# bliunlpr/Robust_e2e_gan

Hardware: AMD Instinct MI355X
Metric: joint_train utterances/sec (higher is better)
Workload: dtype f32; 1 GPU; config4: joint_train.py full GAN+ASR step, B=32 per GPU, T=800, F=257->80, L=40, V=4233, enhancer 2xBLSTM-256, VGG+3xBLSTMP-512, loc-attention decoder 300, D basic ndf64, Adadelta; global_batch=32, per_rank_batch=32, parallelism=dp1, utterance_lengths=560..800 frames (mean 680 of T=800)

## Files before the change

### include/re2e.h

```cpp
#ifndef RE2E_H
#define RE2E_H
#include <stddef.h>
#ifdef __cplusplus
extern "C" {
#endif

typedef struct ihipStream_t* re2e_stream_t;

#define RE2E_OK 0
#define RE2E_EINVAL (-1)
#define RE2E_EUNSUPPORTED (-2)
#define RE2E_EHIP (-3)

#define RE2E_ACT_NONE 0
#define RE2E_ACT_TANH 1
#define RE2E_ACT_RELU 2
#define RE2E_ACT_LRELU 3
#define RE2E_ACT_SIGMOID 4
#define RE2E_ACT_SIGMOID_MASK_MUL 5

#define RE2E_LOSS_L2 0
#define RE2E_LOSS_L1 1
#define RE2E_LOSS_SMOOTH_L1 2
#define RE2E_STREAM_DEFAULT 0
#define RE2E_STREAM_FILLER 1

#define RE2E_LOSS_BCE 3

#define RE2E_ABI_VERSION 322
int re2e_version(void);
const char* re2e_last_error(void);
int re2e_device_ok(void);
int re2e_warmup(void);
int re2e_stream_role(re2e_stream_t stream, int role);

size_t re2e_gemm_workspace_bytes(int transa, int transb, int M, int N, int K);
int re2e_gemm(int transa, int transb, int M, int N, int K, const float* A, long lda, const float* B, long ldb,
              float* C, long ldc, const float* bias, const float* bias2, int act, float beta, const float* mul,
              float* mask_out, const int* lens_dev, int T, void* workspace, size_t workspace_bytes,
              re2e_stream_t stream);
int re2e_gemm_plan(int transa, int transb, int M, int N, int K, int a16, int b16, int c16, int act, int rowmap, int filler, int cus, char* out,
                   size_t out_bytes);
int re2e_gemm_nt_rows(int Mv, int N, int K, const float* A, long lda, const float* B, long ldb, float* C, long ldc, const float* bias,
                      const float* bias2, int act, float beta, const int* rowmap, int ident_rows, int phys_rows, void* workspace,
                      size_t workspace_bytes, re2e_stream_t stream);
int re2e_gemm_tn_rows(int M, int N, int Kv, const float* A, long lda, const float* B, long ldb, float* C, long ldc, float beta,
                      const int* rowmap, int ident_rows, int phys_rows, void* workspace, size_t workspace_bytes, re2e_stream_t stream);
int re2e_fill_rows(float* C, long ldc, int N, const int* rows, int nrows, float value, const float* row_vec, int act, re2e_stream_t stream);

int re2e_conv_igemm(const float* in, int NI, int H, int W, int C, const float* wg, int Cout, int KH, int KW, int PH,
                    int PW, int SY, int SX, int DY, int DX, int OY0, int OX0, float* out, int OHF, int OWF, int osy,
                    int osx, int ooy, int oox, const float* bias, int act, float beta, re2e_stream_t stream);
int re2e_conv_igemm_masked(const float* in, int NI, int H, int W, int C, const float* wg, int Cout, int KH, int KW, int PH,
                           int PW, int SY, int SX, int DY, int DX, int OY0, int OX0, float* out, int OHF, int OWF, int osy,
                           int osx, int ooy, int oox, const float* relu_out, re2e_stream_t stream);
int re2e_conv3x3_relu_pool(const float* in, int NI, int H, int W, int C, const float* wg, int Cout, const float* bias, float* pooled,
                           unsigned char* idx_u8, re2e_stream_t stream);
size_t re2e_conv3x3_wino_workspace_bytes(int C, int Cout);
int re2e_conv3x3_wino(const float* in, int NI, int H, int W, int C, const float* w, int Cout, int dgrad, const float* bias, int relu,
                      const float* mask, float* out, float* pool_out, unsigned char* pool_idx, void* workspace, size_t workspace_bytes,
                      re2e_stream_t stream);

size_t re2e_conv3x3_wino_wgrad_workspace_bytes(int NI, int H, int W, int C, int Cout);
int re2e_conv3x3_wino_wgrad(const float* in, int NI, int H, int W, int C, const float* dout, int Cout, float* gw, float beta,
                            void* workspace, size_t workspace_bytes, re2e_stream_t stream);

int re2e_conv3x3_wino_rows(const float* in, int NI, int H, int W, int C, const float* w, int Cout, int dgrad, const float* bias, int relu,
                           const float* mask, float* out, float* pool_out, unsigned char* pool_idx, const int* row_lim, void* workspace,
                           size_t workspace_bytes, re2e_stream_t stream);
int re2e_conv3x3_wino_wgrad_rows(const float* in, int NI, int H, int W, int C, const float* dout, int Cout, float* gw, float beta,
                                 const int* row_lim, void* workspace, size_t workspace_bytes, re2e_stream_t stream);
int re2e_fill_image_rows(float* t, int N, int H, long row_floats, const int* lim, int div, int max_tail_rows, float value, re2e_stream_t stream);

size_t re2e_conv4x4_wino_workspace_bytes(int NI, int H, int W, int C, int Cout, int pad);
int re2e_conv4x4_wino(const float* in, int NI, int H, int W, int C, const float* w, int Cout, int pad, int dgrad, float* out,
                      void* workspace, size_t workspace_bytes, re2e_stream_t stream);
size_t re2e_conv4x4_wino_wgrad_workspace_bytes(int NI, int H, int W, int C, int Cout, int pad);
int re2e_conv4x4_wino_wgrad(const float* in, int NI, int H, int W, int C, const float* dout, int Cout, int pad, float* gw, float beta,
                            void* workspace, size_t workspace_bytes, re2e_stream_t stream);
size_t re2e_conv_wgrad_workspace_bytes(int NI, int PH, int PW, int C, int Cout, int KH, int KW);
int re2e_conv_wgrad(const float* in, int NI, int H, int W, int C, const float* dout, int Cout, int KH, int KW, int PH,
                    int PW, int SY, int SX, int OY0, int OX0, float* dW, float beta, void* workspace,
                    size_t workspace_bytes, re2e_stream_t stream);
int re2e_conv_dgrad_s2(const float* dz, int N, int OH, int OW, int Cout, const float* W, int Cin, int KH, int KW, int H,
                       int Wd, int pad, float* dx, float* wt_ws, re2e_stream_t stream);
int re2e_conv_weight_gather(const float* W, float* dst, int Cout, int Cin, int KH, int KW, int transpose, int TA,
                            int TB, int kh0, int kw0, int kstep, re2e_stream_t stream);

int re2e_transpose01(const float* in, float* out, int D0, int D1, int W, re2e_stream_t stream);
int re2e_act_fwd(const float* x, float* y, long n, int act, re2e_stream_t stream);
int re2e_act_bwd(const float* dy, const float* y, float* dz, long n, int act, re2e_stream_t stream);
size_t re2e_colsum_workspace_bytes(int M, int N);
int re2e_colsum(const float* A, int M, int N, long lda, float* out, float beta, void* workspace,
                size_t workspace_bytes, re2e_stream_t stream);
int re2e_act_bwd_colsum(const float* dy, const float* y, float* dz, int M, int N, int act, float* out, float beta,
                        void* workspace, size_t workspace_bytes, re2e_stream_t stream);
int re2e_mask_mul_bwd(const float* dout, const float* mix, const float* mask, float* dlin, long n,
                      re2e_stream_t stream);
int re2e_mask_mul_bwd_ld(const float* dout, const float* mix, const float* mask, float* dlin, long rows, int N, int ldd,
                         re2e_stream_t stream);
int re2e_mul(const float* a, const float* b, float* out, long n, re2e_stream_t stream);
int re2e_affine_cols(const float* x, const float* c0, const float* c1, float* out, long rows, int N,
                     re2e_stream_t stream);
int re2e_dropout(const float* x, float* y, long n, float p, unsigned long long seed, unsigned call, re2e_stream_t stream);
int re2e_axpby(float a, const float* x, float b, float* y, long n, re2e_stream_t stream);
int re2e_gather_rows(const float* src, const int* idx_dev, float* dst, int nrows, int W, re2e_stream_t stream);
int re2e_scatter_rows(const float* src, const int* idx_dev, float* dst, int nrows, int W, re2e_stream_t stream);
int re2e_mask_rows(const float* in, float* out, const int* lens_dev, int B, int T, int W, re2e_stream_t stream);

int re2e_pack_pad(const float* src_flat, const int* offsets_dev, const int* lens_dev, int B, int Tmax, int F,
                  float* dst, re2e_stream_t stream);

int re2e_kaldi_decode_pad(const unsigned char* blob, const long* rec_off_dev, const int* kind_dev, const int* lens_dev, int B,
                          int Tmax, int F, float* dst, float* dst_log, const float* cmvn, re2e_stream_t stream);

int re2e_fbank_fwd(const float* x, long rows, int F, int NF, const int* band_off, const int* band_len,
                   const float* band_w, int maxw, float* y_raw, float* y_norm, const float* cmvn, float* pw_out,
                   re2e_stream_t stream);
int re2e_fbank_bwd(const float* x, long rows, int F, int NF, const int* bin_off, const int* bin_len, const float* bin_w, int maxc,
                   const float* pw, const float* dy_raw, const float* dy_norm, const float* cmvn, float* dx, re2e_stream_t stream);
int re2e_logclamp_fwd(const float* z, const float* cmvn, long rows, int N, float* y, re2e_stream_t stream);
int re2e_logclamp_bwd(const float* z, const float* cmvn, long rows, int N, const float* dy, float* dz, re2e_stream_t stream);
int re2e_cmvn_stats(const float* y, const int* lens_dev, int B, int T, int NF, float* sum_out, float* sumsq_out,
                    re2e_stream_t stream);

size_t re2e_reduce_workspace_bytes(long n);
int re2e_loss_fwd(const float* a, const float* b, float target, long n, int kind, float* out, void* workspace,
                  size_t workspace_bytes, re2e_stream_t stream);
int re2e_loss_bwd(const float* a, const float* b, float target, long n, int kind, const float* gscale_dev,
                  float scale, float* da, float beta, re2e_stream_t stream);
int re2e_sumsq(const float* x, long n, float* out, void* workspace, size_t workspace_bytes, re2e_stream_t stream);

int re2e_maxpool2_fwd(const float* in, int NI, int H, int W, int C, float* out, unsigned char* idx_u8, int relu_in,
                      re2e_stream_t stream);
int re2e_maxpool2_bwd(const float* dout, const unsigned char* idx_u8, int NI, int H, int W, int C, float* din,
                      re2e_stream_t stream);
int re2e_vgg_pack_fwd(const float* in, const int* lens_dev, int NI, int T, int Fq, int C, float* out, int NI_total,
                      int n_off, re2e_stream_t stream);
int re2e_vgg_pack_bwd(const float* dout, const int* lens_dev, int NI, int T, int Fq, int C, float* din, int NI_total,
                      int n_off, re2e_stream_t stream);

size_t re2e_bn_workspace_bytes(long P, int C);
int re2e_bn_lrelu_fwd(const float* x, long P, int C, const float* gamma, const float* beta, float* running_mean,
                      float* running_var, float momentum, float eps, int train, float slope, float* y, float* save_mean,
                      float* save_invstd, void* workspace, size_t workspace_bytes, re2e_stream_t stream);
int re2e_bn_lrelu_bwd(const float* dy, const float* x, long P, int C, const float* gamma, const float* beta,
                      const float* save_mean, const float* save_invstd, float slope, float* dx, float* dgamma, float* dbeta,
                      float gbeta, void* workspace, size_t workspace_bytes, re2e_stream_t stream);
int re2e_bn_sync_partial(const float* x, long P, int C, const float* mean, int square, float* out, void* workspace, size_t workspace_bytes,
                         re2e_stream_t stream);
int re2e_bn_sync_finalize(const float* mean, const float* var, long Ptotal, int C, float momentum, float eps, float* running_mean,
                          float* running_var, float* save_mean, float* save_invstd, re2e_stream_t stream);
int re2e_bn_apply(const float* x, long P, int C, const float* save_mean, const float* save_invstd, const float* gamma, const float* beta,
                  float slope, float* y, re2e_stream_t stream);
int re2e_bn_sync_bwd_partial(const float* dy, const float* x, long P, int C, const float* gamma, const float* beta, const float* save_mean,
                             const float* save_invstd, float slope, float* out, void* workspace, size_t workspace_bytes, re2e_stream_t stream);
int re2e_bn_sync_bwd_apply(const float* dy, const float* x, long P, int C, const float* gamma, const float* beta, const float* save_mean,
                           const float* save_invstd, float slope, const float* sums, float* dx, re2e_stream_t stream);

size_t re2e_lstm_workspace_bytes(int B, int H);
int re2e_lstm_abort_count(void);
int re2e_debug_force_abort(int n);
int re2e_debug_occupy(int workgroups, int lds_bytes, int usec, re2e_stream_t stream);
int re2e_step_gate(int* base_dev, int ack, const float* extra_sumsq, float* stats_main, float* stats_d, const float* d_requires, float* hold_next,
                   float* delta_out, re2e_stream_t stream);
int re2e_lstm_seq_fwd(float* xg_f, float* xg_r, const float* whh_f, const float* whh_r, float* ybuf, float* cbuf,
                      const int* lens_dev, int T, int B, int H, void* workspace, size_t workspace_bytes,
                      re2e_stream_t stream);
int re2e_lstm_seq_bwd(float* g_f, float* g_r, const float* whh_f, const float* whh_r, const float* dy,
                      const float* ybuf, const float* cbuf, float* dc_state, const int* lens_dev, int T, int B, int H,
                      float* dbias, void* workspace, size_t workspace_bytes, re2e_stream_t stream);
int re2e_lstm_plan(int T, int B, int H, int backward, int cus, char* out, size_t out_bytes);

int re2e_lstm_cell_fwd(float* gates, const float* c_prev, float* c_out, float* h_out, int B, int H,
                       re2e_stream_t stream);
int re2e_lstm_cell_bwd(float* gates, const float* c_prev, const float* c_cur, const float* dh, const float* dh2,
                       const float* dc_in, float* dc_prev_out, int B, int H, re2e_stream_t stream);
int re2e_dec_gates_cell_fwd(const float* cx, const float* z_prev, const float* w_ctx, long ldw, const float* w_hh, float* gates,
                            const float* c_prev, float* c_out, float* h_out, int B, int E, int D, re2e_stream_t stream);
size_t re2e_dec_loop_workspace_bytes(int L1, int B, int T, int E, int D, int A, int C, int Fh);
int re2e_dec_loop_fwd(const float* pre, const float* enc, const int* hlens_dev, const float* w_decT, const float* w_att, const float* w_conv,
                      const float* gvec, const float* gvec_b, const float* w_ctx, long ldw, const float* w_hh, float* gates, float* z, float* c,
                      float* w, float* cx, float* conv, float* dpj, int L1, int B, int T, int E, int D, int A, int C, int Fh,
                      void* workspace, size_t workspace_bytes, re2e_stream_t stream);
size_t re2e_dec_loop_bwd_workspace_bytes(int L1, int B, int T, int E, int D, int A, int C, int Fh);
int re2e_dec_loop_bwd(const float* pre, const float* enc, const float* cx, const float* z, const float* c, const float* w, const float* conv,
                      const float* dpj, const float* dZ, const int* hlens_dev, const float* w_ctx, long ldw, const float* w_hh, const float* mlp_dec,
                      const float* w_att, const float* w_conv, const float* gvec, float* gates, float* d_cx_all, float* de_all, float* ddp,
                      float* d_pre, int L1, int B, int T, int E, int D, int A, int C, int Fh, void* workspace, size_t workspace_bytes,
                      re2e_stream_t stream);
int re2e_dec_loop_dwconv(const float* w, const int* hlens_dev, const void* workspace, size_t workspace_bytes, float* partials, int partial_floats,
                         int wconv_offset, int L1, int B, int T, int E, int D, int A, int C, int Fh, re2e_stream_t stream);
int re2e_gemm_skinny2(int M, int K, const float* A, long lda, const float* B1, long ldb1, int N1, float* C1, long ldc1,
                      const float* B2, long ldb2, int N2, float* C2, long ldc2, re2e_stream_t stream);
int re2e_embedding_fwd(const float* table, const int* ids_dev, int n, int D, float* out, long ldo,
                       re2e_stream_t stream);
int re2e_embedding_bwd(const float* dout, long ldo, const int* ids_dev, int n, int D, int V, float* dtable,
                       float beta, re2e_stream_t stream);
int re2e_argmax_rows(const float* x, int R, int V, long ldx, int* out_ids, re2e_stream_t stream);
int re2e_log_softmax_rows(const float* x, int R, int V, long ldx, float* out, re2e_stream_t stream);

int re2e_ce_fwd(const float* logits, const int* targets_dev, int R, int V, float scale, float* out, float* lse,
                void* workspace, size_t workspace_bytes, re2e_stream_t stream);
int re2e_ce_bwd(const float* logits, const int* targets_dev, const float* lse, const float* fwd_out, int R, int V,
                float scale, const float* gscale_dev, float* dlogits, re2e_stream_t stream);
int re2e_lsm_fwd(const float* logits, const float* dist, int R, int V, int nutt, float* out, void* workspace,
                 size_t workspace_bytes, re2e_stream_t stream);
int re2e_lsm_bwd(const float* logits, const float* dist, int R, int V, int nutt, const float* gscale, float* dlogits,
                 re2e_stream_t stream);

size_t re2e_ctc_workspace_bytes(int T, int B, int Lmax);
int re2e_ctc_fwd(const float* logits, int T, int B, int V, const int* hlens_dev, const int* labels_dev,
                 const int* label_off_dev, const int* label_len_dev, int Lmax, float* loss_out, float* nll_per_utt,
                 void* workspace, size_t workspace_bytes, re2e_stream_t stream);
int re2e_ctc_bwd(const float* logits, int T, int B, int V, const int* hlens_dev, const int* labels_dev,
                 const int* label_off_dev, const int* label_len_dev, int Lmax, const float* nll_per_utt,
                 const float* gscale_dev, float* dlogits, int ldd, const void* workspace, re2e_stream_t stream);

int re2e_ctc_prefix_score(const float* lpz, int T, int V, const float* att_lsm, int nh, const float* r_prev, const int* last_label_dev,
                          const int* out_len_dev, const float* prev_score_dev, int ctc_beam, float att_weight, float ctc_weight, int blank,
                          int eos, int* cand_out, float* local_out, float* ctc_score_out, float* r_new, re2e_stream_t stream);
int re2e_ctc_prefix_score_cands(const float* lpz, int T, int V, const float* att_lsm, int nh, const float* r_prev, const int* last_label_dev,
                                const int* out_len_dev, const float* prev_score_dev, const int* cand_dev, int ncand, float att_weight,
                                float ctc_weight, int blank, int eos, float* local_out, float* ctc_score_out, float* r_new, re2e_stream_t stream);

int re2e_attloc_fwd(const float* pre, const float* enc, const float* z, const float* att_prev, const int* hlens_dev,
                    const float* w_decT, const float* w_att, const float* w_conv, const float* gvec, const float* gvec_b,
                    int B, int T, int eprojs, int dunits, int adim, int chans, int filts, float* w_out, float* c_out,
                    long ldc_out, float* conv_out, float* dp_out, float* e_scratch, re2e_stream_t stream);
size_t re2e_attloc_partial_floats(int adim, int chans, int filts);
size_t re2e_attloc_workspace_bytes(int B, int T, int adim, int chans);
int re2e_attloc_bwd(const float* pre, const float* enc, const float* att_prev, const float* w_cur, const int* hlens_dev,
                    const float* w_att, const float* w_conv, const float* gvec, const float* conv_in, const float* dp_in,
                    const float* cx_in, const float* dc, long ld_dc, const float* dw_in, int B, int T, int eprojs, int adim,
                    int chans, int filts, float* de_out, float* d_att_prev, float* d_decproj, float* partials,
                    void* workspace, size_t workspace_bytes, re2e_stream_t stream);
int re2e_attloc_dpre(const float* pre, const float* conv_all, const float* dp_all, const float* de_all, const float* w_att,
                     const float* gvec, int L1, int B, int T, int adim, int chans, int filts, float* d_pre, float* partials,
                     void* workspace, size_t workspace_bytes, re2e_stream_t stream);
int re2e_attloc_denc(const float* w_all, const float* dc_all, int L1, int B, int T, int eprojs, float* d_enc, float beta,
                     re2e_stream_t stream);

int re2e_lm_lstm_cell(const float* x, long ldx, const int* ids_dev, int n_embed, int I, const float* w_ih, const float* w_hh,
                      const float* b_ih, const float* b_hh, const float* h_prev, const float* c_prev, int n, int H, float* h_out,
                      float* c_out, re2e_stream_t stream);
int re2e_lm_output(const float* h, const float* w, const float* b, int n, int V, int H, float* logits, re2e_stream_t stream);
int re2e_lm_log_softmax_combine(const float* logits, int n, int V, const float* att, float lm_weight, float* lsm, float* comb,
                                re2e_stream_t stream);
int re2e_lm_add_cands(float* local, const float* lm, const int* cand_dev, int n, int ncand, int V, float lm_weight, re2e_stream_t stream);

int re2e_clip_coef(const float* sumsq_dev, float max_norm, float* stats_dev, re2e_stream_t stream);
int re2e_adadelta_step(float* p, const float* g, float* sq_avg, float* acc_delta, long n, float rho, float eps,
                       float lr, const float* stats_dev, re2e_stream_t stream);
int re2e_adam_step(float* p, const float* g, float* m, float* v, long n, float lr, float beta1, float beta2,
                   float eps, int step, const float* stats_dev, re2e_stream_t stream);

#ifdef __cplusplus
}
#endif
#endif
```

### robust_e2e_gan_amd/csrc/lstm.hip

```cpp
#include <stdlib.h>

#include <atomic>

#include "common.h"

namespace {

#ifdef RE2E_EXPERIMENTS
__device__ unsigned long long* g_lstm_stamps = nullptr;
constexpr int kStampStep0 = 64;
#define LSTM_STAMP_DECL unsigned long long* const stamp_p = g_lstm_stamps
#define LSTM_STAMP(ph)                                                                                                              \
  do {                                                                                                                              \
    if (stamp_p && (threadIdx.x & 63) == 0 && s >= kStampStep0 && s < kStampStep0 + 16)                                             \
      stamp_p[((((long)blockIdx.z * gridDim.y + blockIdx.y) * gridDim.x + blockIdx.x) * 16 + (threadIdx.x >> 6)) * 192 + (s - kStampStep0) * 12 + (ph)] = \
          (ph) >= 10 ? __builtin_amdgcn_s_memrealtime() : __builtin_amdgcn_s_memtime();                                             \
  } while (0)
static void lstm_stamps_arm() {
  const char* v = getenv("RE2E_LSTM_STAMPS");
  unsigned long long* p = v ? (unsigned long long*)strtoull(v, nullptr, 16) : nullptr;
  (void)hipMemcpyToSymbol(HIP_SYMBOL(g_lstm_stamps), &p, sizeof(p));
}
#else
#define LSTM_STAMP_DECL
#define LSTM_STAMP(ph)
static void lstm_stamps_arm() {}
#endif

__device__ __forceinline__ void store_acc(float* red, const f32x16& acc, int lane) {
  int lr = lane & 31, lh = lane >> 5;
#pragma unroll
  for (int r = 0; r < 16; ++r) {
    int row = (r & 3) + 8 * (r >> 2) + 4 * lh;
    red[row * 33 + lr] = acc[r];
  }
}

__device__ __forceinline__ void mfma_chain(const f32x4* __restrict__ ap, const f32x4* __restrict__ bp, int QN, f32x16& acc,
                                           int bstride = 64, bool bvalid = true) {
  constexpr int CH = 8;
  const f32x4 zero = {0.f, 0.f, 0.f, 0.f};
  for (int q0 = 0; q0 < QN; q0 += CH) {
    f32x4 a[CH], b[CH];
#pragma unroll
    for (int u = 0; u < CH; ++u) {
      int q = q0 + u < QN ? q0 + u : QN - 1;
      a[u] = ap[(long)q * 64];
      b[u] = bvalid ? bp[(long)q * bstride] : zero;
    }
#pragma unroll
    for (int u = 0; u < CH; ++u) {
      if (q0 + u < QN) {
#pragma unroll
        for (int j = 0; j < 4; ++j) acc = __builtin_amdgcn_mfma_f32_32x32x2f32(a[u][j], b[u][j], acc, 0, 0, 0);
      }
    }
  }
}

__global__ void pack_w_fwd_kernel(const float* __restrict__ whh, float* __restrict__ wf, int H) {
  long tot = (long)4 * H * H;
  for (long e = (long)blockIdx.x * blockDim.x + threadIdx.x; e < tot; e += (long)gridDim.x * blockDim.x) {
    int i = (int)(e & 3); int lane = (int)((e >> 2) & 63); long r = e >> 8; int Q = (int)(r % (H / 8)); int x = (int)(r / (H / 8));
    int n = lane & 31, h = lane >> 5;
    wf[e] = whh[((long)((n >> 3) * H + 8 * x + (n & 7))) * H + 8 * Q + 4 * h + i];
  }
}
__global__ void pack_w_bwd_kernel(const float* __restrict__ whh, float* __restrict__ wb, int H, int UW) {
  const int njt = (H + 31) / 32, NQ = 4 * UW;
  long tot = (long)(H / (8 * UW)) * njt * NQ * 256;
  for (long e = (long)blockIdx.x * blockDim.x + threadIdx.x; e < tot; e += (long)gridDim.x * blockDim.x) {
    int i = (int)(e & 3); int lane = (int)((e >> 2) & 63); long r = e >> 8; int Q = (int)(r % NQ); r /= NQ; int jt = (int)(r % njt); int x = (int)(r / njt);
    int m = 8 * Q + 4 * (lane >> 5) + i;
    int j = 32 * jt + (lane & 31);
    wb[e] = j < H ? whh[((long)(((m >> 3) & 3) * H + 8 * UW * x + 8 * (m >> 5) + (m & 7))) * H + j] : 0.f;
  }
}

template <int WAVES>
__global__ __launch_bounds__(WAVES * 64) void lstm_fwd_step(float* xg_f, float* xg_r, const float* __restrict__ wfrag, float* ybuf,
                                                            float* cbuf, float* hfrag, const int* __restrict__ lens, int T, int B,
                                                            int H, int s) {
  extern __shared__ __attribute__((aligned(16))) float red[];
  constexpr int NTH = WAVES * 64;
  constexpr int ITER = (256 + NTH - 1) / NTH;
  const int dir = blockIdx.z, mt = blockIdx.y, x = blockIdx.x, MT = gridDim.y;
  const int t = dir ? T - 1 - s : s;
  float* xg = dir ? xg_r : xg_f;
  const int j0 = x * 8, b0 = mt * 32;
  const int tid = threadIdx.x, lane = tid & 63, wid = tid >> 6, lh = lane >> 5;
  const int QN = H / 8 / WAVES;
  const int prev_blk = dir ? t + 2 : t;
  const long H2 = 2L * H;
  const long hf_sz = (long)2 * MT * H * 32;
  const float* hf_rd = hfrag + ((s & 1) ^ 1) * hf_sz + (long)(dir * MT + mt) * H * 32;
  float* hf_wr = hfrag + (s & 1) * hf_sz + (long)(dir * MT + mt) * H * 32;
  float pre[ITER][4], cp[ITER];
  int ln[ITER];
#pragma unroll
  for (int it = 0; it < ITER; ++it) {
    int idx = tid + it * NTH;
    int bm = idx >> 3, jj = idx & 7, b = b0 + bm, j = j0 + jj;
    bool ok = idx < 256 && b < B;
    const float* gp = xg + ((long)t * B + (ok ? b : 0)) * 4 * H + j;
#pragma unroll
    for (int g = 0; g < 4; ++g) pre[it][g] = ok ? gp[g * H] : 0.f;
    cp[it] = ok ? cbuf[((long)prev_blk * B + b) * H2 + dir * H + j] : 0.f;
    ln[it] = ok ? lens[b] : 0;
  }
  const f32x4* wp = reinterpret_cast<const f32x4*>(wfrag) + ((long)(dir * (H / 8) + x) * (H / 8) + wid * QN) * 64 + lane;
  const f32x4* hp = reinterpret_cast<const f32x4*>(hf_rd) + ((long)(2 * wid * QN + lh)) * 32 + (lane & 31);
  f32x16 acc;
#pragma unroll
  for (int r = 0; r < 16; ++r) acc[r] = 0.f;
  if (s > 0) mfma_chain(hp, wp, QN, acc);
  store_acc(red + wid * (32 * 33), acc, lane);
  __syncthreads();
#pragma unroll
  for (int it = 0; it < ITER; ++it) {
    int idx = tid + it * NTH;
    int bm = idx >> 3, jj = idx & 7, b = b0 + bm, j = j0 + jj;
    if (idx >= 256 || b >= B) continue;
    float v[4];
#pragma unroll
    for (int g = 0; g < 4; ++g) {
      float a = 0.f;
      for (int w = 0; w < WAVES; ++w) a += red[w * (32 * 33) + bm * 33 + g * 8 + jj];
      v[g] = a + pre[it][g];
    }
    float gi = sigmoidf_(v[0]), gf = sigmoidf_(v[1]), gg = tanhf_(v[2]), go = sigmoidf_(v[3]);
    float c = gf * cp[it] + gi * gg;
    float h = go * tanhf_(c);
    if (t >= ln[it]) { c = 0.f; h = 0.f; }
    float* go_ = xg + ((long)t * B + b) * 4 * H + j;
    go_[0] = gi; go_[H] = gf; go_[2 * H] = gg; go_[3 * H] = go;
    cbuf[((long)(t + 1) * B + b) * H2 + dir * H + j] = c;
    ybuf[((long)(t + 1) * B + b) * H2 + dir * H + j] = h;
    hf_wr[((long)(j >> 2) * 32 + bm) * 4 + (j & 3)] = h;
  }
}

typedef unsigned long long u64;
typedef unsigned u32x4 __attribute__((ext_vector_type(4)));
typedef __attribute__((address_space(1))) u64 gu64;
__device__ unsigned g_persist_aborts = 0;
constexpr unsigned kSpinLimit = 1u << 24;

template <int WAVES, int QN, int UW>
__global__ __launch_bounds__(WAVES * 64) void lstm_fwd_persist(float* xg_f, float* xg_r, const float* __restrict__ wfrag, float* ybuf,
                                                               float* cbuf, u64* hx_, unsigned* err, const int* __restrict__ lens,
                                                               int T, int B, int H) {
  extern __shared__ __attribute__((aligned(16))) float red[];
  static_assert(WAVES >= 4 * UW, "256 threads per 8 units own the 32 x 8 cell updates");
  const int dir = blockIdx.z, mt = blockIdx.y, MT = gridDim.y, NX = gridDim.x * UW;
  const int tid = threadIdx.x, lane = tid & 63, wid = tid >> 6, lr = lane & 31, lh = lane >> 5;
  const int usub = (tid >> 8) < UW ? (tid >> 8) : 0;
  const int x = blockIdx.x * UW + usub;
  float* xg = dir ? xg_r : xg_f;
  const int j0 = x * 8, b0 = mt * 32;
  constexpr int kAbort = UW * WAVES * 32 * 33;
  if (tid == 0) red[kAbort] = 0.f;
  const long H2 = 2L * H;
  f32x4 w[UW][QN];
#pragma unroll
  for (int u = 0; u < UW; ++u) {
    const f32x4* wp = reinterpret_cast<const f32x4*>(wfrag) + ((long)(dir * NX + blockIdx.x * UW + u) * NX + wid * QN) * 64 + lane;
#pragma unroll
    for (int q = 0; q < QN; ++q) w[u][q] = wp[q * 64];
  }
  gu64* hx = (gu64*)hx_;
  const int par_sz = 2 * MT * NX * 256;
  const __amdgpu_buffer_rsrc_t hx_rs = __builtin_amdgcn_make_buffer_rsrc(hx_, 0, (int)(2 * par_sz * 8), 0x00020000);
  const int grp = (dir * MT + mt) * NX * 256;
  const int rd_off = grp + (wid * QN) * 256 + (lh * 32 + lr) * 4;
  const bool pw = tid < 256 * UW;
  const int bm = (tid >> 3) & 31, jj = tid & 7, b = b0 + bm, j = j0 + jj;
  const bool ok = pw && b < B;
  const int ln = ok ? lens[b] : 0;
  const int wr_off = grp + x * 256 + ((jj >> 2) * 32 + bm) * 4 + (jj & 3);
  float c = 0.f, pre[4] = {0.f, 0.f, 0.f, 0.f};
  if (ok) {
    const float* gp = xg + ((long)(dir ? T - 1 : 0) * B + b) * 4 * H + j;
#pragma unroll
    for (int g = 0; g < 4; ++g) pre[g] = gp[g * H];
  }
  LSTM_STAMP_DECL;
  __syncthreads();
  for (int s = 0; s < T; ++s) {
    const int t = dir ? T - 1 - s : s;
    LSTM_STAMP(0); LSTM_STAMP(10);
    f32x16 acc[UW];
#pragma unroll
    for (int u = 0; u < UW; ++u)
#pragma unroll
      for (int r = 0; r < 16; ++r) acc[u][r] = 0.f;
    if (s > 0) {
      const gu64* src = hx + ((s & 1) ^ 1) * par_sz + rd_off;
      float hv[QN][4];
      const unsigned rd_b = (unsigned)((((s & 1) ^ 1) * par_sz + rd_off) * 8);
      for (unsigned spins = 0;; ++spins) {
        asm volatile("" ::: "memory");
        bool good = true;
#pragma unroll
        for (int q = 0; q < QN; ++q) {
          const u32x4 lo = __builtin_amdgcn_raw_buffer_load_b128(hx_rs, rd_b + (unsigned)q * 2048u, 0, 16);
          const u32x4 hi = __builtin_amdgcn_raw_buffer_load_b128(hx_rs, rd_b + (unsigned)q * 2048u + 16u, 0, 16);
          hv[q][0] = __uint_as_float(lo[0]); hv[q][1] = __uint_as_float(lo[2]);
          hv[q][2] = __uint_as_float(hi[0]); hv[q][3] = __uint_as_float(hi[2]);
          good &= (lo[1] == (unsigned)s) & (lo[3] == (unsigned)s) & (hi[1] == (unsigned)s) & (hi[3] == (unsigned)s);
        }
        if (__all(good)) break;
        if (spins > kSpinLimit) { if (lane == 0) { red[kAbort] = 1.f; if (atomicExch(err, 1u) == 0u) atomicAdd(&g_persist_aborts, 1u); } break; }
        __builtin_amdgcn_s_sleep(1);
      }
      LSTM_STAMP(1);
#pragma unroll
      for (int q = 0; q < QN; ++q)
#pragma unroll
        for (int i = 0; i < 4; ++i)
#pragma unroll
          for (int u = 0; u < UW; ++u) acc[u] = __builtin_amdgcn_mfma_f32_32x32x2f32(hv[q][i], w[u][q][i], acc[u], 0, 0, 0);
    }
#pragma unroll
    for (int u = 0; u < UW; ++u) store_acc(red + (u * WAVES + wid) * (32 * 33), acc[u], lane);
    LSTM_STAMP(2);
    __syncthreads();
    LSTM_STAMP(3);
    if (red[kAbort] != 0.f) break;
    if (pw) {
      float v[4];
#pragma unroll
      for (int g = 0; g < 4; ++g) {
        float a = 0.f;
#pragma unroll
        for (int wv = 0; wv < WAVES; ++wv) a += red[(usub * WAVES + wv) * (32 * 33) + bm * 33 + g * 8 + jj];
        v[g] = a + pre[g];
      }
      float gi = sigmoidf_(v[0]), gf = sigmoidf_(v[1]), gg = tanhf_(v[2]), go = sigmoidf_(v[3]);
      float cn = gf * c + gi * gg;
      float h = go * tanhf_(cn);
      if (t >= ln) { cn = 0.f; h = 0.f; }
      c = cn;
      if (ok && s + 1 < T) {
        const float* gp = xg + ((long)(dir ? t - 1 : t + 1) * B + b) * 4 * H + j;
#pragma unroll
        for (int g = 0; g < 4; ++g) pre[g] = gp[g * H];
      }
      if (s + 1 < T)
        __hip_atomic_store(hx + (s & 1) * par_sz + wr_off, ((u64)(unsigned)(s + 1) << 32) | (u64)__float_as_uint(h), __ATOMIC_RELAXED,
                           __HIP_MEMORY_SCOPE_AGENT);
      LSTM_STAMP(4); LSTM_STAMP(11);
      if (ok) {
        float* go_ = xg + ((long)t * B + b) * 4 * H + j;
        go_[0] = gi; go_[H] = gf; go_[2 * H] = gg; go_[3 * H] = go;
        cbuf[((long)(t + 1) * B + b) * H2 + dir * H + j] = cn;
        ybuf[((long)(t + 1) * B + b) * H2 + dir * H + j] = h;
      }
    }
    LSTM_STAMP(5);
    __syncthreads();
    LSTM_STAMP(6);
  }
  if (red[kAbort] != 0.f && ok) {
    for (int t = 0; t < T; ++t) ybuf[((long)(t + 1) * B + b) * H2 + dir * H + j] = __uint_as_float(0x7fc00000u);
  }
}

__device__ __forceinline__ void store16u_sc1(unsigned* p, const u32x4& v) {
  asm volatile("global_store_dwordx4 %0, %1, off sc1\n\ts_nop 1" ::"v"(p), "v"(v) : "memory");
}
constexpr unsigned kTagBit = 0x40000000u, kNanPub = 0x3FC00000u;
__device__ __forceinline__ bool tags_are(const u32x4& v, unsigned want) {
  return (((v[0] & v[1] & v[2] & v[3]) ^ want) & kTagBit) == 0u && (((v[0] | v[1] | v[2] | v[3]) ^ want) & kTagBit) == 0u;
}

template <int TILES, int NJ, bool PERSIST>
__global__ __launch_bounds__(256) void lstm_fwd2(float* xg_f, float* xg_r, const float* __restrict__ whh_f, const float* __restrict__ whh_r,
                                                 float* ybuf, float* cbuf, unsigned* hx_, unsigned* err, const int* __restrict__ lens, int T,
                                                 int B, int H, int s_arg) {
  constexpr int KS = 4;
  extern __shared__ __attribute__((aligned(16))) float lds2[];
  f32x4* part = reinterpret_cast<f32x4*>(lds2);
  int* abortw = reinterpret_cast<int*>(lds2 + 2 * TILES * KS * 64 * 4);
  const int dir = blockIdx.z, mt = blockIdx.y, MT = gridDim.y, x = blockIdx.x;
  const int tid = threadIdx.x, lane = tid & 63, ks = tid >> 6, n = lane & 15, kk = lane >> 4;
  const int ft = ks < TILES ? ks : -1;
  float* xg = dir ? xg_r : xg_f;
  const float* whh = dir ? whh_r : whh_f;
  const long H2 = 2L * H;
  if (PERSIST && tid == 0) *abortw = 0;
  f32x4 w[TILES][NJ];
#pragma unroll
  for (int t = 0; t < TILES; ++t) {
    const long row = (long)(n & 3) * H + 4 * TILES * x + 4 * t + (n >> 2);
#pragma unroll
    for (int jj = 0; jj < NJ; ++jj) w[t][jj] = *reinterpret_cast<const f32x4*>(whh + row * H + 16 * (ks * NJ + jj) + 4 * kk);
  }
  const int par_w = 2 * MT * H * 16;
  const __amdgpu_buffer_rsrc_t hx_rs = __builtin_amdgcn_make_buffer_rsrc(hx_, 0, (int)(2 * par_w * 4), 0x00020000);
  const bool fin = ft >= 0;
  const int j = 4 * TILES * x + 4 * (fin ? ft : 0) + kk;
  const int s0 = PERSIST ? 0 : s_arg, s1 = PERSIST ? T : s_arg + 1;
  const int grp = (dir * MT + mt) * H * 16;
  const int b = 16 * mt + n;
  const unsigned rd_w = (unsigned)(grp + ((4 * ks * NJ + kk) * 16 + n) * 4);
  const unsigned poll_w = (unsigned)(grp + ((4 * ks * NJ + (lane < 4 * NJ ? lane : 0)) * 16) * 4);
  const bool ok = fin && b < B;
  const int ln = ok ? lens[b] : 0;
  const unsigned wr_w = (unsigned)(grp + ((TILES * x + (fin ? ft : 0)) * 16 + n) * 4);
  float c = 0.f, pre[4] = {0.f, 0.f, 0.f, 0.f};
  if (ok) {
    const int t0 = dir ? T - 1 - s0 : s0;
    const float* gp = xg + ((long)t0 * B + b) * 4 * H + j;
#pragma unroll
    for (int g = 0; g < 4; ++g) pre[g] = gp[g * H];
    if (!PERSIST) c = cbuf[((long)(dir ? t0 + 2 : t0) * B + b) * H2 + dir * H + j];
  }
  u32x4 ld[NJ];
#pragma unroll
  for (int jj = 0; jj < NJ; ++jj) ld[jj] = u32x4{0u, 0u, 0u, 0u};
  if (!PERSIST && s0 > 0) {
    const u32x4* src = reinterpret_cast<const u32x4*>(hx_ + ((s0 & 1) ^ 1) * par_w) + rd_w / 4;
#pragma unroll
    for (int jj = 0; jj < NJ; ++jj) ld[jj] = src[jj * 64];
  }
  LSTM_STAMP_DECL;
  if (PERSIST) __syncthreads();
  for (int s = s0; s < s1; ++s) {
    const int t = dir ? T - 1 - s : s;
    LSTM_STAMP(0); LSTM_STAMP(10);
    constexpr int NACC = TILES == 1 ? 2 : TILES;
    f32x4 acc[NACC];
#pragma unroll
    for (int tt = 0; tt < NACC; ++tt) acc[tt] = f32x4{0.f, 0.f, 0.f, 0.f};
    if (s > 0) {
      const unsigned want = PERSIST ? (unsigned)((((s - 1) >> 1) + 1) & 1) << 30 : 0u;
      const unsigned rd_b = (unsigned)((((s & 1) ^ 1) * par_w) * 4) + rd_w * 4u;
      const unsigned pl_b = (unsigned)((((s & 1) ^ 1) * par_w) * 4) + poll_w * 4u;
      auto wait_producers = [&]() {
        for (unsigned spins = 0;; ++spins) {
          asm volatile("" ::: "memory");
          const u32x4 pv = __builtin_amdgcn_raw_buffer_load_b128(hx_rs, pl_b, 0, 16);
          if (__all(tags_are(pv, want))) break;
          if (spins > kSpinLimit) { if (lane == 0) { *abortw = 1; if (atomicExch(err, 1u) == 0u) atomicAdd(&g_persist_aborts, 1u); } break; }
        }
        asm volatile("" ::: "memory");
      };
      if (PERSIST) {
        wait_producers();
#pragma unroll
        for (int jj = 0; jj < NJ; ++jj) ld[jj] = __builtin_amdgcn_raw_buffer_load_b128(hx_rs, rd_b + (unsigned)jj * 1024u, 0, 16);
        LSTM_STAMP(7);
      }
#pragma unroll
      for (int jj = 0; jj < NJ; ++jj) {
        u32x4 v = ld[jj];
        if (PERSIST) {
          if (!__all(tags_are(v, want))) {
            wait_producers();
#pragma unroll
            for (int j2 = jj; j2 < NJ; ++j2) ld[j2] = __builtin_amdgcn_raw_buffer_load_b128(hx_rs, rd_b + (unsigned)j2 * 1024u, 0, 16);
            v = ld[jj];
            for (unsigned spins = 0; !__all(tags_are(v, want)); ++spins) {
              asm volatile("" ::: "memory");
              v = __builtin_amdgcn_raw_buffer_load_b128(hx_rs, rd_b + (unsigned)jj * 1024u, 0, 16);
              if (spins > kSpinLimit) { if (lane == 0) { *abortw = 1; if (atomicExch(err, 1u) == 0u) atomicAdd(&g_persist_aborts, 1u); } break; }
            }
          }
        }
        float hv[4];
#pragma unroll
        for (int i = 0; i < 4; ++i) {
          unsigned uu = PERSIST ? (v[i] & ~kTagBit) : v[i];
          if (PERSIST) uu = uu == kNanPub ? 0x7fc00000u : uu;
          hv[i] = __uint_as_float(uu);
        }
#pragma unroll
        for (int i = 0; i < 4; ++i)
#pragma unroll
          for (int tt = 0; tt < TILES; ++tt) {
            const int a = TILES == 1 ? (i & 1) : tt;
            acc[a] = __builtin_amdgcn_mfma_f32_16x16x4f32(w[tt][jj][i], hv[i], acc[a], 0, 0, 0);
          }
      }
      if (TILES == 1) acc[0] += acc[1];
    }
    LSTM_STAMP(1);
    f32x4* pp = part + (s & 1) * (TILES * KS * 64);
#pragma unroll
    for (int tt = 0; tt < TILES; ++tt)
      if (tt != ft) pp[(tt * KS + ks) * 64 + lane] = acc[tt];
    LSTM_STAMP(2);
    __syncthreads();
    LSTM_STAMP(3);
    if (PERSIST && *abortw) break;
    float og[6] = {0.f, 0.f, 0.f, 0.f, 0.f, 0.f};
    if (fin) {
      f32x4 v = {0.f, 0.f, 0.f, 0.f};
      f32x4 mine = acc[0];
#pragma unroll
      for (int tt = 1; tt < TILES; ++tt) mine = ft == tt ? acc[tt] : mine;
#pragma unroll
      for (int k2 = 0; k2 < KS; ++k2) v += k2 == ks ? mine : pp[(ft * KS + k2) * 64 + lane];
      const float gi = sigmoidf_(v[0] + pre[0]), gf = sigmoidf_(v[1] + pre[1]), gg = tanhf_(v[2] + pre[2]), go = sigmoidf_(v[3] + pre[3]);
      float cn = __builtin_fmaf(gf, c, gi * gg);
      float h = go * tanhf_(cn);
      if (t >= ln) { cn = 0.f; h = 0.f; }
      c = cn;
      if (PERSIST && ok && s + 1 < T) {
        const float* gp = xg + ((long)(dir ? t - 1 : t + 1) * B + b) * 4 * H + j;
#pragma unroll
        for (int g = 0; g < 4; ++g) pre[g] = gp[g * H];
      }
      if (!PERSIST || s + 1 < T) {
        unsigned hb = __float_as_uint(h);
        if (PERSIST) hb = (h != h ? kNanPub : hb) | ((unsigned)(((s >> 1) + 1) & 1) << 30);
        u32x4 pv;
        pv[0] = hb;
        pv[1] = (unsigned)__builtin_amdgcn_ds_bpermute(((lane + 16) & 63) * 4, (int)hb);
        pv[2] = (unsigned)__builtin_amdgcn_ds_bpermute(((lane + 32) & 63) * 4, (int)hb);
        pv[3] = (unsigned)__builtin_amdgcn_ds_bpermute(((lane + 48) & 63) * 4, (int)hb);
        if (kk == 0) {
          if (PERSIST) store16u_sc1(hx_ + (s & 1) * par_w + wr_w, pv);
          else *reinterpret_cast<u32x4*>(hx_ + (s & 1) * par_w + wr_w) = pv;
        }
      }
      LSTM_STAMP(4); LSTM_STAMP(11);
      og[0] = gi; og[1] = gf; og[2] = gg; og[3] = go; og[4] = cn; og[5] = h;
    }
    LSTM_STAMP(5);
    if (ok) {
      float* go_ = xg + ((long)t * B + b) * 4 * H + j;
      go_[0] = og[0]; go_[H] = og[1]; go_[2 * H] = og[2]; go_[3 * H] = og[3];
      cbuf[((long)(t + 1) * B + b) * H2 + dir * H + j] = og[4];
      ybuf[((long)(t + 1) * B + b) * H2 + dir * H + j] = og[5];
    }
    LSTM_STAMP(6);
  }
  if (PERSIST && *abortw && ok) {
    for (int t = 0; t < T; ++t) ybuf[((long)(t + 1) * B + b) * H2 + dir * H + j] = __uint_as_float(0x7fc00000u);
  }
}

template <int JT>
__global__ __launch_bounds__(256) void lstm_bwd_step(float* g_f, float* g_r, const float* __restrict__ wb, const float* __restrict__ dy,
                                                     const float* __restrict__ cbuf, float* dc_state, float* slabs,
                                                     const int* __restrict__ lens, int T, int B, int H, int s) {
  __shared__ __attribute__((aligned(16))) float dgs[32 * 36];
  const int dir = blockIdx.z, mt = blockIdx.y, x = blockIdx.x, MT = gridDim.y, NX = gridDim.x;
  const int t = dir ? s : T - 1 - s;
  float* G = dir ? g_r : g_f;
  const int j0 = x * 8, b0 = mt * 32;
  const int tid = threadIdx.x, lane = tid & 63, wid = tid >> 6, lr = lane & 31, lh = lane >> 5;
  const int K4 = 4 * H;
  const long H2 = 2L * H;
  const int prev_blk = dir ? t + 2 : t;
  const long sl_sz = (long)2 * MT * NX * NX * 256;
  const float* sl_rd = slabs + ((s & 1) ^ 1) * sl_sz + (long)(dir * MT + mt) * NX * NX * 256;
  float* sl_wr = slabs + (s & 1) * sl_sz + (long)(dir * MT + mt) * NX * NX * 256;
  {
    const int bm = tid >> 3, jj = tid & 7, b = b0 + bm, j = j0 + jj;
    const bool ok = b < B;
    const long bb = ok ? b : 0;
    float dh = dy[((long)t * B + bb) * H2 + dir * H + j];
    const float* gp0 = G + ((long)t * B + bb) * K4 + j;
    const float gi = gp0[0], gf = gp0[H], gg = gp0[2 * H], go = gp0[3 * H];
    const float c = cbuf[((long)(t + 1) * B + bb) * H2 + dir * H + j];
    const float cp = cbuf[((long)prev_blk * B + bb) * H2 + dir * H + j];
    const float dc = dc_state[bb * H2 + dir * H + j];
    const int ln = lens[bb];
    if (s > 0) {
      const float* q = sl_rd + (long)x * NX * 256 + tid;
      float a0 = 0.f, a1 = 0.f, a2 = 0.f, a3 = 0.f;
      int xx = 0;
      for (; xx + 8 <= NX; xx += 8) {
        float v0 = q[(long)(xx + 0) * 256], v1 = q[(long)(xx + 1) * 256], v2 = q[(long)(xx + 2) * 256], v3 = q[(long)(xx + 3) * 256];
        float v4 = q[(long)(xx + 4) * 256], v5 = q[(long)(xx + 5) * 256], v6 = q[(long)(xx + 6) * 256], v7 = q[(long)(xx + 7) * 256];
        a0 += v0 + v4; a1 += v1 + v5; a2 += v2 + v6; a3 += v3 + v7;
      }
      for (; xx < NX; ++xx) a0 += q[(long)xx * 256];
      dh += (a0 + a1) + (a2 + a3);
    }
    float di = 0.f, df = 0.f, dg = 0.f, dout = 0.f, dcp = dc;
    if (ok && t < ln) {
      float tc = tanhf_(c);
      float dct = dh * go * (1.f - tc * tc) + dc;
      dout = dh * tc * go * (1.f - go);
      di = dct * gg * gi * (1.f - gi);
      df = dct * cp * gf * (1.f - gf);
      dg = dct * gi * (1.f - gg * gg);
      dcp = dct * gf;
    }
    if (ok) {
      float* gp = G + ((long)t * B + b) * K4 + j;
      gp[0] = di; gp[H] = df; gp[2 * H] = dg; gp[3 * H] = dout;
      dc_state[(long)b * H2 + dir * H + j] = dcp;
    }
    dgs[bm * 36 + jj] = di; dgs[bm * 36 + 8 + jj] = df; dgs[bm * 36 + 16 + jj] = dg; dgs[bm * 36 + 24 + jj] = dout;
  }
  __syncthreads();
  if (s == T - 1) return;
  f32x4 a4[4];
#pragma unroll
  for (int Q = 0; Q < 4; ++Q) a4[Q] = *reinterpret_cast<const f32x4*>(dgs + lr * 36 + 8 * Q + 4 * lh);
  const int njt = (H + 31) / 32;
  const f32x4* wp = reinterpret_cast<const f32x4*>(wb) + ((long)(dir * NX + x) * njt) * 256 + lane;
  for (int jt0 = wid * JT; jt0 < njt; jt0 += 4 * JT) {
    f32x4 b4[JT][4];
    f32x16 acc[JT];
#pragma unroll
    for (int u = 0; u < JT; ++u) {
      const int jt = jt0 + u < njt ? jt0 + u : njt - 1;
#pragma unroll
      for (int Q = 0; Q < 4; ++Q) b4[u][Q] = wp[(long)(jt * 4 + Q) * 64];
#pragma unroll
      for (int r = 0; r < 16; ++r) acc[u][r] = 0.f;
    }
#pragma unroll
    for (int Q = 0; Q < 4; ++Q)
#pragma unroll
      for (int i = 0; i < 4; ++i)
#pragma unroll
        for (int u = 0; u < JT; ++u) acc[u] = __builtin_amdgcn_mfma_f32_32x32x2f32(a4[Q][i], b4[u][Q][i], acc[u], 0, 0, 0);
#pragma unroll
    for (int u = 0; u < JT; ++u) {
      const int jt = jt0 + u;
      if (jt < njt && 32 * jt + lr < H) {
        float* dst = sl_wr + ((long)(4 * jt + (lr >> 3)) * NX + x) * 256 + (lr & 7);
#pragma unroll
        for (int r = 0; r < 16; ++r) {
          int row = (r & 3) + 8 * (r >> 2) + 4 * lh;
          dst[row * 8] = acc[u][r];
        }
      }
    }
  }
}

typedef __attribute__((address_space(1))) unsigned gu32;

__device__ __forceinline__ void store16_sc1(float* p, const f32x4& v) {
  asm volatile("global_store_dwordx4 %0, %1, off sc1\n\ts_nop 1" ::"v"(p), "v"(v) : "memory");
}

template <int TPW, int UW>
__global__ __launch_bounds__(256) void lstm_bwd_persist(float* g_f, float* g_r, const float* __restrict__ wb, const float* __restrict__ dy,
                                                        const float* __restrict__ cbuf, float* dc_state, float* xbuf, unsigned* flags_,
                                                        unsigned* err, const int* __restrict__ lens, int T, int B, int H) {
  constexpr int UN = 8 * UW;
  constexpr int KG = 32 * UW;
  constexpr int LDG = KG + 4;
  constexpr int BLK = 256 * UW;
  __shared__ __attribute__((aligned(16))) float dgs[32 * LDG];
  __shared__ __attribute__((aligned(16))) float psum[4 * 256];
  __shared__ int aborted;
  const int dir = blockIdx.z, mt = blockIdx.y, x = blockIdx.x, MT = gridDim.y, NX = gridDim.x;
  float* G = dir ? g_r : g_f;
  const int j0 = x * UN, b0 = mt * 32;
  const int tid = threadIdx.x, lane = tid & 63, wid = tid >> 6, lr = lane & 31, lh = lane >> 5;
  const int K4 = 4 * H;
  const long H2 = 2L * H;
  const int njt = (H + 31) / 32;
// ... 394 lines not shown
  float v = 0.f;
  if (c < H4)
    for (long r = rl; r < M; r += 4) v += G[r * H4 + c];
  red[rl][threadIdx.x & 63] = v;
  __syncthreads();
  if (rl == 0 && c < H4) out[(long)dir * H4 + c] = (red[0][threadIdx.x] + red[1][threadIdx.x]) + (red[2][threadIdx.x] + red[3][threadIdx.x]);
}

__global__ void zero_kernel(float* p, long n) {
  for (long i = (long)blockIdx.x * blockDim.x + threadIdx.x; i < n; i += (long)gridDim.x * blockDim.x) p[i] = 0.f;
}

int fwd_step_waves(int H) {
  if (const char* v = exp_env("RE2E_LSTM_WAVES_FWD")) {
    const int w = atoi(v);
    if (w >= 1 && w <= 16 && (w & (w - 1)) == 0 && H % (8 * w) == 0) return w;
  }
  for (int w = 16; w > 1; w >>= 1)
    if (H % (8 * w) == 0 && H / w >= 32) return w;
  return 1;
}

size_t fwd_ws_floats(int B, int H) { long MT = (B + 31) / 32; return (size_t)2 * 4 * H * H + (size_t)2 * 2 * MT * H * 32; }
size_t fwd_hx_bytes(int B, int H) { long MT = (B + 31) / 32; return 16 + (size_t)2 * 2 * MT * (H / 8) * 256 * 8; }
size_t bwd_ws_floats(int B, int H) {
  long MT = (B + 31) / 32, NX = H / 8, njt = (H + 31) / 32;
  return (size_t)2 * NX * njt * 1024 + (size_t)2 * 2 * MT * NX * NX * 256;
}
size_t bwd_flag_bytes(int B, int H) { long MT = (B + 15) / 16, NX = H / 8; return 16 + (size_t)2 * 2 * MT * NX * 128; }

int cu_count() {
  static const int n = [] { int dev = 0; hipDeviceProp_t p; return (hipGetDevice(&dev) == hipSuccess && hipGetDeviceProperties(&p, dev) == hipSuccess) ? p.multiProcessorCount : 1; }();
  return n;
}

enum SeqFamily { kFwd2Persist, kFwd2Step, kFwdPersist, kFwdStep, kBwd3, kBwdPersist, kBwdStep };
struct SeqPlan {
  SeqFamily family;
  int a, b;
  dim3 grid;
  size_t lds;
};
const struct { const char *name, *a, *b; } kFamilyText[] = {{"fwd2_persist", "tiles", "nj"}, {"fwd2_step", "tiles", "nj"}, {"fwd_persist", "waves", "qn"},
                                                            {"fwd_step", "waves", nullptr}, {"bwd3", "un", "tpw"},          {"bwd_persist", "tpw", "uw"},
                                                            {"bwd_step", "jt", nullptr}};

#define RE2E_FWD2_NJ(M, TL) M(TL, 1) M(TL, 2) M(TL, 4) M(TL, 5) M(TL, 8)
#define RE2E_FWD2_ALL(M) RE2E_FWD2_NJ(M, 1) RE2E_FWD2_NJ(M, 2) RE2E_FWD2_NJ(M, 4)
#define RE2E_FWD_PERSIST_ALL(M) M(8, 8) M(8, 5) M(8, 4) M(8, 3) M(4, 4) M(4, 2) M(4, 1)
#define RE2E_FWD_STEP_ALL(M) M(16, 0) M(8, 0) M(4, 0) M(2, 0) M(1, 0)
#define RE2E_BWD3_UN(M, U) M(U, 1) M(U, 2) M(U, 3) M(U, 4) M(U, 5) M(U, 6) M(U, 7) M(U, 8)
#define RE2E_BWD3_ALL(M) RE2E_BWD3_UN(M, 8) RE2E_BWD3_UN(M, 16)
#define RE2E_BWD_PERSIST_ALL(M) M(1, 1) M(1, 2) M(2, 1) M(2, 2) M(3, 1) M(3, 2) M(4, 1) M(4, 2)
#define RE2E_BWD_STEP_ALL(M) M(1, 0) M(2, 0)

bool is_built(SeqFamily family, int a, int b) {
#define RE2E_HAS(A, B) if (a == A && b == B) return true;
  switch (family) {
    case kFwd2Persist: case kFwd2Step: RE2E_FWD2_ALL(RE2E_HAS) break;
    case kFwdPersist: RE2E_FWD_PERSIST_ALL(RE2E_HAS) break;
    case kFwdStep: RE2E_FWD_STEP_ALL(RE2E_HAS) break;
    case kBwd3: RE2E_BWD3_ALL(RE2E_HAS) break;
    case kBwdPersist: RE2E_BWD_PERSIST_ALL(RE2E_HAS) break;
    case kBwdStep: RE2E_BWD_STEP_ALL(RE2E_HAS) break;
  }
#undef RE2E_HAS
  return false;
}

constexpr size_t kCuLds = 160 * 1024;
constexpr size_t kBwdStaticLds = 16 * 1024;
size_t own_cu_lds(long workgroups, int cus, size_t static_lds, size_t needed) {
  return workgroups <= cus / 2 ? kCuLds - static_lds : needed;
}

bool env_off(const char* name) {
  const char* v = getenv(name);
  return v && atoi(v) == 0;
}

bool plan_fwd(int T, int B, int H, bool weights_16B_aligned, int cus, SeqPlan& p) {
  if (H % 8 != 0) return false;
  const bool persist = !env_off("RE2E_LSTM_PERSIST") && T >= 2;
  if (!env_off("RE2E_LSTM_FWD2") && weights_16B_aligned && H % 64 == 0 && (B <= 16 || H >= 384)) {
    const long per = (long)cdiv(B, 16) * 2;
    int tiles = 0;
    for (int lim : {cus / 2, cus})
      for (int tl = 1; tl <= 4 && !tiles; tl *= 2)
        if ((long)(H / (4 * tl)) * per <= lim) tiles = tl;
    const bool resident = persist && tiles;
    if (!tiles) tiles = 4;
    if (is_built(kFwd2Persist, tiles, H / 64)) {
      p = {resident ? kFwd2Persist : kFwd2Step, tiles, H / 64, dim3(H / (4 * tiles), cdiv(B, 16), 2), (size_t)tiles * 8192 + 16};
      if (resident) p.lds = own_cu_lds((long)p.grid.x * p.grid.y * 2, cus, 0, p.lds);
      return true;
    }
  }
  const dim3 grid(H / 8, cdiv(B, 32), 2);
  if (persist && (long)grid.x * grid.y * 2 <= cus) {
#define RE2E_FIT(W, Q) if ((int)grid.x == W * Q) { p = {kFwdPersist, W, Q, grid, own_cu_lds((long)grid.x * grid.y * 2, cus, 0, (size_t)W * 32 * 33 * sizeof(float) + 16)}; return true; }
    RE2E_FWD_PERSIST_ALL(RE2E_FIT)
#undef RE2E_FIT
  }
  const int w = fwd_step_waves(H);
  p = {kFwdStep, w, 0, grid, (size_t)w * 32 * 33 * sizeof(float)};
  return is_built(kFwdStep, w, 0);
}

bool plan_bwd(int T, int B, int H, int cus, SeqPlan& p) {
  if (H % 8 != 0) return false;
  const bool persist = !env_off("RE2E_LSTM_PERSIST_BWD") && T >= 2;
  if (persist && !env_off("RE2E_LSTM_BWD3") && H % 64 == 0) {
    const long per = (long)cdiv(B, 16) * 2;
    const int ue = exp_env("RE2E_LSTM_BWD3_UN") ? atoi(exp_env("RE2E_LSTM_BWD3_UN")) : 0;
    int un = 0;
    if (ue == 8 || ue == 16) un = (long)(H / ue) * per <= cus ? ue : 0;
    else if ((long)(H / 8) * per <= cus / 4) un = 8;
    else if ((long)(H / 16) * per <= cus) un = 16;
    if (un && is_built(kBwd3, un, H / 64)) {
      p = {kBwd3, un, H / 64, dim3(H / un, cdiv(B, 16), 2), 0};
      p.lds = own_cu_lds((long)p.grid.x * p.grid.y * 2, cus, kBwdStaticLds, 0);
      return true;
    }
  }
  if (persist) {
    const char* wv = getenv("RE2E_LSTM_BWD_UW");
    const int uw = (wv ? atoi(wv) : (H >= 512 ? 2 : 1)) == 2 && H % 16 == 0 ? 2 : 1;
    const int tpw = ((H + 31) / 32 + 3) / 4;
    const dim3 grid(H / (8 * uw), cdiv(B, 32), 2);
    if ((long)grid.x * grid.y * 2 <= cus && grid.x <= 128 && is_built(kBwdPersist, tpw, uw)) {
      p = {kBwdPersist, tpw, uw, grid, own_cu_lds((long)grid.x * grid.y * 2, cus, kBwdStaticLds, 0)};
      return true;
    }
  }
  p = {kBwdStep, H / 32 >= 8 ? 2 : 1, 0, dim3(H / 8, cdiv(B, 32), 2), 0};
  return true;
}

template <auto Kernel>
void ensure_lds(size_t bytes) {
  static LdsLimit lim;
  lim.ensure(reinterpret_cast<const void*>(Kernel), bytes);
}

struct FwdArgs {
  float *xg_f, *xg_r;
  const float *whh_f, *whh_r;
  float *ybuf, *cbuf;
  const int* lens;
  int T, B, H;
  float *wfrag, *hfrag;
  void* hxmem;
  size_t hxbytes;
};
struct BwdArgs {
  float *g_f, *g_r;
  const float *wb, *dy, *cbuf;
  float *dc, *slabs;
  const int* lens;
  int T, B, H;
  void* flagmem;
  size_t flagbytes;
  float* dbp;
};

template <int W>
void launch_fwd_step(const SeqPlan& p, const FwdArgs& a, hipStream_t st) {
  ensure_lds<&lstm_fwd_step<W>>(p.lds);
  const long hn = (long)2 * 2 * p.grid.y * a.H * 32;
  hipLaunchKernelGGL(zero_kernel, dim3(cdiv(hn, 256) > 1024 ? 1024 : cdiv(hn, 256)), dim3(256), 0, st, a.hfrag, hn);
  for (int s = 0; s < a.T; ++s)
    hipLaunchKernelGGL((lstm_fwd_step<W>), p.grid, dim3(W * 64), p.lds, st, a.xg_f, a.xg_r, a.wfrag, a.ybuf, a.cbuf, a.hfrag, a.lens, a.T, a.B, a.H, s);
}
template <int W, int QN>
void launch_fwd_persist(const SeqPlan& p, const FwdArgs& a, hipStream_t st) {
  ensure_lds<&lstm_fwd_persist<W, QN, 1>>(p.lds);
  lstm_stamps_arm();
  (void)hipMemsetAsync(a.hxmem, 0, a.hxbytes, st);
  hipLaunchKernelGGL((lstm_fwd_persist<W, QN, 1>), p.grid, dim3(W * 64), p.lds, st, a.xg_f, a.xg_r, a.wfrag, a.ybuf, a.cbuf, (u64*)((char*)a.hxmem + 16),
                     (unsigned*)a.hxmem, a.lens, a.T, a.B, a.H);
}
template <int TILES, int NJ>
void launch_fwd2_persist(const SeqPlan& p, const FwdArgs& a, hipStream_t st) {
  ensure_lds<&lstm_fwd2<TILES, NJ, true>>(p.lds);
  lstm_stamps_arm();
  (void)hipMemsetAsync(a.hxmem, 0, a.hxbytes, st);
  hipLaunchKernelGGL((lstm_fwd2<TILES, NJ, true>), p.grid, dim3(256), p.lds, st, a.xg_f, a.xg_r, a.whh_f, a.whh_r, a.ybuf, a.cbuf,
                     (unsigned*)((char*)a.hxmem + 16), (unsigned*)a.hxmem, a.lens, a.T, a.B, a.H, 0);
}
template <int TILES, int NJ>
void launch_fwd2_step(const SeqPlan& p, const FwdArgs& a, hipStream_t st) {
  ensure_lds<&lstm_fwd2<TILES, NJ, false>>(p.lds);
  for (int s = 0; s < a.T; ++s)
    hipLaunchKernelGGL((lstm_fwd2<TILES, NJ, false>), p.grid, dim3(256), p.lds, st, a.xg_f, a.xg_r, a.whh_f, a.whh_r, a.ybuf, a.cbuf,
                       (unsigned*)((char*)a.hxmem + 16), (unsigned*)a.hxmem, a.lens, a.T, a.B, a.H, s);
}
template <int JT>
void launch_bwd_step(const SeqPlan& p, const BwdArgs& a, hipStream_t st) {
  for (int s = 0; s < a.T; ++s)
    hipLaunchKernelGGL((lstm_bwd_step<JT>), p.grid, dim3(256), 0, st, a.g_f, a.g_r, a.wb, a.dy, a.cbuf, a.dc, a.slabs, a.lens, a.T, a.B, a.H, s);
}
template <int TPW, int UW>
void launch_bwd_persist(const SeqPlan& p, const BwdArgs& a, hipStream_t st) {
  lstm_stamps_arm();
  (void)hipMemsetAsync(a.flagmem, 0, a.flagbytes, st);
  ensure_lds<&lstm_bwd_persist<TPW, UW>>(p.lds);
  hipLaunchKernelGGL((lstm_bwd_persist<TPW, UW>), p.grid, dim3(256), p.lds, st, a.g_f, a.g_r, a.wb, a.dy, a.cbuf, a.dc, a.slabs,
                     (unsigned*)((char*)a.flagmem + 16), (unsigned*)a.flagmem, a.lens, a.T, a.B, a.H);
}
template <int UN, int TPW>
void launch_bwd3(const SeqPlan& p, const BwdArgs& a, hipStream_t st) {
  lstm_stamps_arm();
  (void)hipMemsetAsync(a.flagmem, 0, a.flagbytes, st);
  ensure_lds<&lstm_bwd3<UN, TPW>>(p.lds);
  hipLaunchKernelGGL((lstm_bwd3<UN, TPW>), p.grid, dim3(256), p.lds, st, a.g_f, a.g_r, a.wb, a.dy, a.cbuf, a.dc, a.slabs,
                     (unsigned*)((char*)a.flagmem + 16), (unsigned*)a.flagmem, a.lens, a.T, a.B, a.H, a.dbp);
}

int run_fwd(const SeqPlan& p, const FwdArgs& args, hipStream_t st) {
  switch (p.family) {
#define RE2E_F2P(A, B) if (p.a == A && p.b == B) return launch_fwd2_persist<A, B>(p, args, st), RE2E_OK;
#define RE2E_F2S(A, B) if (p.a == A && p.b == B) return launch_fwd2_step<A, B>(p, args, st), RE2E_OK;
#define RE2E_FP(A, B) if (p.a == A && p.b == B) return launch_fwd_persist<A, B>(p, args, st), RE2E_OK;
#define RE2E_FS(A, B) if (p.a == A) return launch_fwd_step<A>(p, args, st), RE2E_OK;
    case kFwd2Persist: RE2E_FWD2_ALL(RE2E_F2P) break;
    case kFwd2Step: RE2E_FWD2_ALL(RE2E_F2S) break;
    case kFwdPersist: RE2E_FWD_PERSIST_ALL(RE2E_FP) break;
    case kFwdStep: RE2E_FWD_STEP_ALL(RE2E_FS) break;
    default: break;
#undef RE2E_F2P
#undef RE2E_F2S
#undef RE2E_FP
#undef RE2E_FS
  }
  re2e_set_error("re2e_lstm_seq_fwd: plan %s(%d, %d) is not in the instantiation tables", kFamilyText[p.family].name, p.a, p.b);
  return RE2E_EUNSUPPORTED;
}
int run_bwd(const SeqPlan& p, const BwdArgs& args, hipStream_t st) {
  switch (p.family) {
#define RE2E_B3(A, B) if (p.a == A && p.b == B) return launch_bwd3<A, B>(p, args, st), RE2E_OK;
#define RE2E_BP(A, B) if (p.a == A && p.b == B) return launch_bwd_persist<A, B>(p, args, st), RE2E_OK;
#define RE2E_BS(A, B) if (p.a == A) return launch_bwd_step<A>(p, args, st), RE2E_OK;
    case kBwd3: RE2E_BWD3_ALL(RE2E_B3) break;
    case kBwdPersist: RE2E_BWD_PERSIST_ALL(RE2E_BP) break;
    case kBwdStep: RE2E_BWD_STEP_ALL(RE2E_BS) break;
    default: break;
#undef RE2E_B3
#undef RE2E_BP
#undef RE2E_BS
  }
  re2e_set_error("re2e_lstm_seq_bwd: plan %s(%d, %d) is not in the instantiation tables", kFamilyText[p.family].name, p.a, p.b);
  return RE2E_EUNSUPPORTED;
}

}

namespace {
std::atomic<int> g_force_abort{0};
bool debug_hooks_enabled() {
  static const bool on = [] { const char* e = getenv("RE2E_DEBUG_HOOKS"); return e && atoi(e) == 1; }();
  return on;
}
__global__ void forced_abort_kernel(float* ybuf, long n) {
  for (long i = (long)blockIdx.x * blockDim.x + threadIdx.x; i < n; i += (long)gridDim.x * blockDim.x) ybuf[i] = __uint_as_float(0x7fc00000u);
  if (blockIdx.x == 0 && threadIdx.x == 0) atomicAdd(&g_persist_aborts, 1u);
}
bool forced_abort(hipStream_t st, float* ybuf, int T, int B, int H) {
  int left = g_force_abort.load(std::memory_order_relaxed);
  do {
    if (left <= 0) return false;
  } while (!g_force_abort.compare_exchange_weak(left, left - 1, std::memory_order_relaxed));
  const long n = (long)T * B * 2 * H;
  hipLaunchKernelGGL(forced_abort_kernel, dim3(1024), dim3(256), 0, st, ybuf + (long)B * 2 * H, n);
  return true;
}
__global__ __launch_bounds__(256) void occupy_kernel(unsigned long long ticks, float* sink) {
  extern __shared__ float occ_lds[];
  const unsigned long long t0 = __builtin_amdgcn_s_memrealtime();
  float x = 0.f;
  while (__builtin_amdgcn_s_memrealtime() - t0 < ticks) { occ_lds[threadIdx.x] = x; x += 1.f; __builtin_amdgcn_s_sleep(8); }
  if (x < 0.f) sink[0] = occ_lds[0];
}
}

extern "C" int re2e_debug_force_abort(int n) {
  RE2E_CHECK_ARG(n >= 0, "n must be >= 0");
  if (!debug_hooks_enabled()) { re2e_set_error("re2e_debug_force_abort: test hook, needs RE2E_DEBUG_HOOKS=1 in the environment"); return RE2E_EUNSUPPORTED; }
  g_force_abort.store(n, std::memory_order_relaxed);
  return RE2E_OK;
}

extern "C" int re2e_debug_occupy(int workgroups, int lds_bytes, int usec, hipStream_t stream) {
  RE2E_CHECK_ARG(workgroups > 0 && workgroups <= 4096 && lds_bytes >= 1024 && lds_bytes <= 160 * 1024 && usec > 0 && usec <= 1000000, "bad argument");
  if (!debug_hooks_enabled()) { re2e_set_error("re2e_debug_occupy: test hook, needs RE2E_DEBUG_HOOKS=1 in the environment"); return RE2E_EUNSUPPORTED; }
  static LdsLimit lim;
  lim.ensure(reinterpret_cast<const void*>(&occupy_kernel), (size_t)lds_bytes);
  hipLaunchKernelGGL(occupy_kernel, dim3(workgroups), dim3(256), (size_t)lds_bytes, stream, (unsigned long long)usec * 100ull, (float*)nullptr);
  RE2E_LAUNCH_CHECK();
  return RE2E_OK;
}

extern "C" int re2e_warmup(void) {
  const size_t fwd_own = kCuLds, bwd_own = kCuLds - kBwdStaticLds;
#define RE2E_WFP(W, Q) ensure_lds<&lstm_fwd_persist<W, Q, 1>>(fwd_own);
#define RE2E_WF2(TL, NJV) ensure_lds<&lstm_fwd2<TL, NJV, true>>(fwd_own);
#define RE2E_WBP(TP, U) ensure_lds<&lstm_bwd_persist<TP, U>>(bwd_own);
#define RE2E_WB3(U, TP) ensure_lds<&lstm_bwd3<U, TP>>(bwd_own);
  RE2E_FWD_PERSIST_ALL(RE2E_WFP) RE2E_FWD2_ALL(RE2E_WF2) RE2E_BWD_PERSIST_ALL(RE2E_WBP) RE2E_BWD3_ALL(RE2E_WB3)
#undef RE2E_WFP
#undef RE2E_WF2
#undef RE2E_WBP
#undef RE2E_WB3
  hipError_t e = hipGetLastError();
  if (e != hipSuccess) { re2e_set_error("re2e_warmup: %s", hipGetErrorString(e)); return RE2E_EHIP; }
  return RE2E_OK;
}

size_t bwd_dbp_bytes(int B, int H) { return (size_t)2 * ((B + 15) / 16) * 4 * H * sizeof(float); }
extern "C" size_t re2e_lstm_workspace_bytes(int B, int H) {
  size_t a = fwd_ws_floats(B, H) * sizeof(float) + fwd_hx_bytes(B, H), b = bwd_ws_floats(B, H) * sizeof(float) + bwd_flag_bytes(B, H) + bwd_dbp_bytes(B, H);
  return a > b ? a : b;
}

int re2e_dec_abort_count_();

const unsigned* re2e_dec_abort_counter_ptr_();
namespace {
__global__ void step_gate_kernel(const unsigned* dec_cnt, int* base, int ack, const float* extra_sumsq, float* stats_main, float* stats_d,
                                 const float* d_requires, float* hold_next, float* delta_out) {
  const int c = (int)(__hip_atomic_load(&g_persist_aborts, __ATOMIC_RELAXED, __HIP_MEMORY_SCOPE_AGENT) +
                      (dec_cnt ? __hip_atomic_load(dec_cnt, __ATOMIC_RELAXED, __HIP_MEMORY_SCOPE_AGENT) : 0u));
  if (ack) *base = c;
  const int delta = c - *base;
  if (delta_out) *delta_out = (float)delta;
  if (hold_next) *hold_next = delta == 0 ? 1.f : __uint_as_float(0x7fc00000u);
  bool ok = delta == 0;
  if (extra_sumsq) { const float e = *extra_sumsq; ok = ok && e == e && fabsf(e) < 3.0e38f; }
  if (stats_main && !ok) { stats_main[2] = 0.f; stats_main[5] = 0.f; stats_main[0] = __uint_as_float(0x7fc00000u); stats_main[3] = stats_main[0]; }
  if (stats_d && (delta != 0 || (d_requires && *d_requires == 0.f))) stats_d[2] = 0.f;
}
}

extern "C" int re2e_step_gate(int* base_dev, int ack, const float* extra_sumsq, float* stats_main, float* stats_d, const float* d_requires,
                              float* hold_next, float* delta_out, hipStream_t stream) {
  RE2E_CHECK_ARG(base_dev, "null base");
  hipLaunchKernelGGL(step_gate_kernel, dim3(1), dim3(1), 0, stream, re2e_dec_abort_counter_ptr_(), base_dev, ack, extra_sumsq, stats_main, stats_d,
                     d_requires, hold_next, delta_out);
  RE2E_LAUNCH_CHECK();
  return RE2E_OK;
}

extern "C" int re2e_lstm_abort_count(void) {
  unsigned n = 0;
  if (hipMemcpyFromSymbol(&n, HIP_SYMBOL(g_persist_aborts), sizeof(n)) != hipSuccess) return -1;
  const int d = re2e_dec_abort_count_();
  return d < 0 ? -1 : (int)n + d;
}

extern "C" int re2e_lstm_plan(int T, int B, int H, int backward, int cus, char* out, size_t out_bytes) {
  RE2E_CHECK_ARG(T > 0 && B > 0 && H > 0 && cus >= 0 && out && out_bytes > 0, "bad argument");
  if (cus == 0) cus = cu_count();
  SeqPlan p;
  if (!(backward ? plan_bwd(T, B, H, cus, p) : plan_fwd(T, B, H, true, cus, p))) {
    re2e_set_error("re2e_lstm_plan: no recurrence kernel is built for hidden size %d", H);
    return RE2E_EUNSUPPORTED;
  }
  const auto& f = kFamilyText[p.family];
  int n = snprintf(out, out_bytes, "family=%s %s=%d", f.name, f.a, p.a);
  if (f.b && n > 0 && (size_t)n < out_bytes) n += snprintf(out + n, out_bytes - n, " %s=%d", f.b, p.b);
  if (n > 0 && (size_t)n < out_bytes) n += snprintf(out + n, out_bytes - n, " grid=%ux%ux%u lds=%zu", p.grid.x, p.grid.y, p.grid.z, p.lds);
  RE2E_CHECK_ARG(n > 0 && (size_t)n < out_bytes, "out_bytes too small");
  return RE2E_OK;
}

extern "C" int re2e_lstm_seq_fwd(float* xg_f, float* xg_r, const float* whh_f, const float* whh_r, float* ybuf, float* cbuf,
                                 const int* lens_dev, int T, int B, int H, void* workspace, size_t workspace_bytes,
                                 hipStream_t stream) {
  RE2E_CHECK_ARG(xg_f && xg_r && whh_f && whh_r && ybuf && cbuf && lens_dev && workspace, "null arg");
  RE2E_CHECK_ARG(T > 0 && B > 0 && H > 0, "bad shape");
  if (H % 8 != 0) { re2e_set_error("re2e_lstm_seq_fwd: hidden size must be a multiple of 8 (got %d)", H); return RE2E_EUNSUPPORTED; }
  RE2E_CHECK_ARG(workspace_bytes >= fwd_ws_floats(B, H) * sizeof(float) + fwd_hx_bytes(B, H), "workspace too small");
  SeqPlan p;
  const bool aligned = ((reinterpret_cast<uintptr_t>(whh_f) | reinterpret_cast<uintptr_t>(whh_r)) & 15) == 0;
  if (!plan_fwd(T, B, H, aligned, cu_count(), p)) { re2e_set_error("re2e_lstm_seq_fwd: no kernel is built for hidden size %d", H); return RE2E_EUNSUPPORTED; }
  if (!env_off("RE2E_LSTM_PERSIST") && T >= 2 && forced_abort(stream, ybuf, T, B, H)) { RE2E_LAUNCH_CHECK(); return RE2E_OK; }
  const long wn = (long)4 * H * H;
  float* wfrag = (float*)workspace;
  const FwdArgs args = {xg_f, xg_r, whh_f, whh_r, ybuf, cbuf, lens_dev, T, B, H, wfrag, wfrag + 2 * wn,
                        (char*)workspace + fwd_ws_floats(B, H) * sizeof(float), fwd_hx_bytes(B, H)};
  if (p.family == kFwdPersist || p.family == kFwdStep) {
    hipLaunchKernelGGL(pack_w_fwd_kernel, dim3(cdiv(wn, 256) > 2048 ? 2048 : cdiv(wn, 256)), dim3(256), 0, stream, whh_f, wfrag, H);
    hipLaunchKernelGGL(pack_w_fwd_kernel, dim3(cdiv(wn, 256) > 2048 ? 2048 : cdiv(wn, 256)), dim3(256), 0, stream, whh_r, wfrag + wn, H);
  }
  if (const int rc = run_fwd(p, args, stream)) return rc;
  RE2E_LAUNCH_CHECK();
  return RE2E_OK;
}

extern "C" int re2e_lstm_seq_bwd(float* g_f, float* g_r, const float* whh_f, const float* whh_r, const float* dy, const float* ybuf,
                                 const float* cbuf, float* dc_state, const int* lens_dev, int T, int B, int H, float* dbias, void* workspace,
                                 size_t workspace_bytes, hipStream_t stream) {
  (void)ybuf;
  RE2E_CHECK_ARG(g_f && g_r && whh_f && whh_r && dy && cbuf && dc_state && lens_dev && workspace, "null arg");
  RE2E_CHECK_ARG(T > 0 && B > 0 && H > 0, "bad shape");
  if (H % 8 != 0) { re2e_set_error("re2e_lstm_seq_bwd: hidden size must be a multiple of 8 (got %d)", H); return RE2E_EUNSUPPORTED; }
  RE2E_CHECK_ARG(workspace_bytes >= bwd_ws_floats(B, H) * sizeof(float) + bwd_flag_bytes(B, H) + (dbias ? bwd_dbp_bytes(B, H) : 0), "workspace too small");
  SeqPlan p;
  if (!plan_bwd(T, B, H, cu_count(), p)) { re2e_set_error("re2e_lstm_seq_bwd: no kernel is built for hidden size %d", H); return RE2E_EUNSUPPORTED; }
  const long wn = (long)(H / 8) * ((H + 31) / 32) * 1024;
  float* wb = (float*)workspace;
  char* flagmem = (char*)workspace + bwd_ws_floats(B, H) * sizeof(float);
  const BwdArgs args = {g_f, g_r, wb, dy, cbuf, dc_state, wb + 2 * wn, lens_dev, T, B, H, flagmem, bwd_flag_bytes(B, H),
                        dbias && p.family == kBwd3 ? (float*)(flagmem + bwd_flag_bytes(B, H)) : nullptr};
  const dim3 pack_grid(cdiv(wn, 256) > 2048 ? 2048 : cdiv(wn, 256));
  if (p.family == kBwd3) {
    const int un = p.a;
    hipLaunchKernelGGL(pack_w_bwd3_kernel, pack_grid, dim3(256), 0, stream, whh_f, wb, H, un);
    hipLaunchKernelGGL(pack_w_bwd3_kernel, pack_grid, dim3(256), 0, stream, whh_r, wb + wn, H, un);
  } else {
    const int uw = p.family == kBwdPersist ? p.b : 1;
    hipLaunchKernelGGL(pack_w_bwd_kernel, pack_grid, dim3(256), 0, stream, whh_f, wb, H, uw);
    hipLaunchKernelGGL(pack_w_bwd_kernel, pack_grid, dim3(256), 0, stream, whh_r, wb + wn, H, uw);
  }
  const long nz = (long)B * 2 * H;
  hipLaunchKernelGGL(zero_kernel, dim3(cdiv(nz, 256)), dim3(256), 0, stream, dc_state, nz);
  if (const int rc = run_bwd(p, args, stream)) return rc;
  if (dbias && p.family == kBwd3)
    hipLaunchKernelGGL(lstm_dbias_reduce_kernel, dim3(cdiv(4 * H, 256), 2), dim3(256), 0, stream, args.dbp, cdiv(B, 16), 4 * H, dbias);
  else if (dbias)
    hipLaunchKernelGGL(gates_colsum_kernel, dim3(cdiv(4 * H, 64), 2), dim3(256), 0, stream, g_f, g_r, (long)T * B, 4 * H, dbias);
  RE2E_LAUNCH_CHECK();
  return RE2E_OK;
}

__global__ void lstm_cell_fwd_kernel(float* gates, const float* __restrict__ c_prev, float* c_out, float* h_out, int B, int H) {
  int i = blockIdx.x * blockDim.x + threadIdx.x;
  if (i >= B * H) return;
  int b = i / H, j = i % H;
  float* g = gates + (long)b * 4 * H + j;
  float gi = sigmoidf_(g[0]), gf = sigmoidf_(g[H]), gg = tanhf_(g[2 * H]), go = sigmoidf_(g[3 * H]);
  float c = gf * c_prev[i] + gi * gg;
  g[0] = gi; g[H] = gf; g[2 * H] = gg; g[3 * H] = go;
  c_out[i] = c;
  h_out[i] = go * tanhf_(c);
}
__global__ __launch_bounds__(512) void dec_gates_cell_kernel(const float* __restrict__ cx, const float* __restrict__ zp, const float* __restrict__ w_ctx,
                                                             long ldw, const float* __restrict__ w_hh, float* gates,
                                                             const float* __restrict__ c_prev, float* c_out, float* h_out, int B, int E, int D) {
  __shared__ float red[8][32][33];
  const int tid = threadIdx.x, lane = tid & 63, wid = tid >> 6, lr = lane & 31, lh = lane >> 5;
  const int u0 = blockIdx.x * 8, b0 = blockIdx.y * 32;
  const int g = lr >> 3, u = u0 + (lr & 7);
  const bool cok = u < D, rok = b0 + lr < B;
  const long wrow = (long)g * D + (cok ? u : 0);
  const int brow = rok ? b0 + lr : 0;
  f32x16 acc;
#pragma unroll
  for (int r = 0; r < 16; ++r) acc[r] = 0.f;
  const f32x4 zero = {0.f, 0.f, 0.f, 0.f};
#pragma unroll
  for (int seg = 0; seg < 2; ++seg) {
    const int K = seg ? D : E;
    const float* ap = (seg ? zp + (long)brow * D : cx + (long)brow * E);
    const float* bp = (seg ? w_hh + wrow * D : w_ctx + wrow * ldw);
    const int kq = (K + 7) / 8;
    for (int qb = wid * 4; qb < kq; qb += 32) {
      f32x4 av[4], bv[4];
#pragma unroll
      for (int t = 0; t < 4; ++t) {
        const int k = 8 * (qb + t) + 4 * lh;
        const bool kok = qb + t < kq && k + 3 < K;
        av[t] = (kok && rok) ? *reinterpret_cast<const f32x4*>(ap + k) : zero;
        bv[t] = (kok && cok) ? *reinterpret_cast<const f32x4*>(bp + k) : zero;
      }
#pragma unroll
      for (int t = 0; t < 4; ++t)
#pragma unroll
        for (int j = 0; j < 4; ++j) acc = __builtin_amdgcn_mfma_f32_32x32x2f32(av[t][j], bv[t][j], acc, 0, 0, 0);
    }
  }
#pragma unroll
  for (int r = 0; r < 16; ++r) red[wid][(r & 3) + 8 * (r >> 2) + 4 * lh][lr] = acc[r];
  __syncthreads();
  if (tid < 256) {
    const int bm = tid >> 3, jj = tid & 7, b = b0 + bm, uu = u0 + jj;
    if (b < B && uu < D) {
      float* gp = gates + (long)b * 4 * D + uu;
      float v[4];
#pragma unroll
      for (int q = 0; q < 4; ++q) {
        float a = 0.f;
#pragma unroll
        for (int w = 0; w < 8; ++w) a += red[w][bm][q * 8 + jj];
        v[q] = a + gp[(long)q * D];
      }
      const float gi = sigmoidf_(v[0]), gf = sigmoidf_(v[1]), gg = tanhf_(v[2]), go = sigmoidf_(v[3]);
      const float c = gf * c_prev[(long)b * D + uu] + gi * gg;
      gp[0] = gi; gp[D] = gf; gp[2L * D] = gg; gp[3L * D] = go;
      c_out[(long)b * D + uu] = c;
      h_out[(long)b * D + uu] = go * tanhf_(c);
    }
  }
}
extern "C" int re2e_dec_gates_cell_fwd(const float* cx, const float* z_prev, const float* w_ctx, long ldw, const float* w_hh, float* gates,
                                       const float* c_prev, float* c_out, float* h_out, int B, int E, int D, hipStream_t stream) {
  RE2E_CHECK_ARG(cx && z_prev && w_ctx && w_hh && gates && c_prev && c_out && h_out, "null operand");
  RE2E_CHECK_ARG(B > 0 && E > 0 && D > 0, "bad shape");
  if (E % 4 || D % 4 || ldw % 4 || ((reinterpret_cast<uintptr_t>(cx) | reinterpret_cast<uintptr_t>(z_prev) | reinterpret_cast<uintptr_t>(w_ctx) |
                                      reinterpret_cast<uintptr_t>(w_hh)) & 15)) {
    re2e_set_error("re2e_dec_gates_cell_fwd: E, D, ldw must be multiples of 4 and the operands 16-byte aligned");
    return RE2E_EUNSUPPORTED;
  }
  hipLaunchKernelGGL(dec_gates_cell_kernel, dim3(cdiv(D, 8), cdiv(B, 32)), dim3(512), 0, stream, cx, z_prev, w_ctx, ldw, w_hh, gates, c_prev, c_out,
                     h_out, B, E, D);
  RE2E_LAUNCH_CHECK();
  return RE2E_OK;
}

extern "C" int re2e_lstm_cell_fwd(float* gates, const float* c_prev, float* c_out, float* h_out, int B, int H, hipStream_t stream) {
  RE2E_CHECK_ARG(gates && c_prev && c_out && h_out && B > 0 && H > 0, "bad args");
  hipLaunchKernelGGL(lstm_cell_fwd_kernel, dim3(cdiv((long)B * H, 256)), dim3(256), 0, stream, gates, c_prev, c_out, h_out, B, H);
  RE2E_LAUNCH_CHECK();
  return RE2E_OK;
}
__global__ void lstm_cell_bwd_kernel(float* gates, const float* __restrict__ c_prev, const float* __restrict__ c_cur,
                                     const float* __restrict__ dh, const float* __restrict__ dh2, const float* __restrict__ dc_in,
                                     float* dc_prev_out, int B, int H) {
  int i = blockIdx.x * blockDim.x + threadIdx.x;
  if (i >= B * H) return;
  int b = i / H, j = i % H;
  float* g = gates + (long)b * 4 * H + j;
  float gi = g[0], gf = g[H], gg = g[2 * H], go = g[3 * H];
  float tc = tanhf_(c_cur[i]);
  float d = dh[i] + (dh2 ? dh2[i] : 0.f);
  float dct = d * go * (1.f - tc * tc) + (dc_in ? dc_in[i] : 0.f);
  g[0] = dct * gg * gi * (1.f - gi);
  g[H] = dct * c_prev[i] * gf * (1.f - gf);
  g[2 * H] = dct * gi * (1.f - gg * gg);
  g[3 * H] = d * tc * go * (1.f - go);
  dc_prev_out[i] = dct * gf;
}
extern "C" int re2e_lstm_cell_bwd(float* gates, const float* c_prev, const float* c_cur, const float* dh, const float* dh2,
                                  const float* dc_in, float* dc_prev_out, int B, int H, hipStream_t stream) {
  RE2E_CHECK_ARG(gates && c_prev && c_cur && dh && dc_prev_out && B > 0 && H > 0, "bad args");
  hipLaunchKernelGGL(lstm_cell_bwd_kernel, dim3(cdiv((long)B * H, 256)), dim3(256), 0, stream, gates, c_prev, c_cur, dh, dh2, dc_in,
                     dc_prev_out, B, H);
  RE2E_LAUNCH_CHECK();
  return RE2E_OK;
}
// ... 1 lines not shown
```

### robust_e2e_gan_amd/flops.py

```python
import contextlib

from . import lib

ROW_HINTS = {}


def note_rows(ptr, values):
    if lib.FLOP_METER is not None:
        ROW_HINTS[int(ptr)] = tuple(int(v) for v in values)


def _rows(ptr, n, H, patch=8):
    lim = ROW_HINTS.get(int(ptr)) if ptr is not None else None
    if lim is None:
        return n * H
    return sum(min(H, (min(l, H) + patch - 1) // patch * patch) for l in lim[:n])


def _ptr(p):
    return getattr(p, 'value', p)


def _wino33(a, rows=None):
    NI, H, W, C, Cout = a[1], a[2], a[3], a[4], a[6]
    return 2.0 * 4 * C * Cout * (NI * H if rows is None else rows) * W


def _wino44(NI, H, W, C, Cout, pad):
    OH, OW = H + 2 * pad - 3, W + 2 * pad - 3
    return 2.0 * 25 * C * Cout * NI * ((OH + 1) // 2) * ((OW + 1) // 2)


EXECUTED = {
    're2e_gemm': lambda *a: 2.0 * a[2] * a[3] * a[4],
    're2e_gemm_nt_rows': lambda *a: 2.0 * a[0] * a[1] * a[2],
    're2e_gemm_tn_rows': lambda *a: 2.0 * a[0] * a[1] * a[2],
    're2e_gemm_skinny2': lambda *a: 2.0 * a[0] * a[1] * (a[6] + a[11]),
    're2e_conv_igemm': lambda *a: 2.0 * a[1] * a[9] * a[10] * a[6] * a[7] * a[8] * a[4],
    're2e_conv_igemm_masked': lambda *a: 2.0 * a[1] * a[9] * a[10] * a[6] * a[7] * a[8] * a[4],
    're2e_conv3x3_relu_pool': lambda *a: 2.0 * 9 * a[1] * a[2] * a[3] * a[4] * a[6],
    're2e_conv3x3_wino': lambda *a: _wino33(a),
    're2e_conv3x3_wino_wgrad': lambda *a: _wino33(a),
    're2e_conv3x3_wino_rows': lambda *a: _wino33(a, _rows(_ptr(a[14]), a[1], a[2])),
    're2e_conv3x3_wino_wgrad_rows': lambda *a: _wino33(a, _rows(_ptr(a[9]), a[1], a[2])),
    're2e_conv4x4_wino': lambda *a: _wino44(a[1], a[2], a[3], a[4], a[6], a[7]),
    're2e_conv4x4_wino_wgrad': lambda *a: _wino44(a[1], a[2], a[3], a[4], a[6], a[7]),
    're2e_conv_wgrad': lambda *a: 2.0 * a[1] * a[9] * a[10] * a[6] * a[7] * a[8] * a[4],
    're2e_conv_dgrad_s2': lambda *a: 2.0 * a[1] * a[9] * a[10] * a[6] * a[4] * (a[7] * a[8] / 4.0),
    're2e_lstm_seq_fwd': lambda *a: 2.0 * 2 * a[7] * a[8] * a[9] * 4 * a[9],
    're2e_lstm_seq_bwd': lambda *a: 2.0 * 2 * a[9] * a[10] * a[11] * 4 * a[11],
    're2e_fbank_fwd': lambda *a: 2.0 * a[1] * a[2] * a[3],
    're2e_fbank_bwd': lambda *a: 2.0 * a[1] * a[2] * a[3],
}


@contextlib.contextmanager
def meter():
    prev, lib.FLOP_METER = lib.FLOP_METER, {}
    try:
        yield lib.FLOP_METER
    finally:
        lib.FLOP_METER = prev
        ROW_HINTS.clear()


DIRECT_OVER_EXECUTED = {'re2e_conv3x3_wino': 2.25, 're2e_conv3x3_wino_rows': 2.25, 're2e_conv3x3_wino_wgrad': 2.25, 're2e_conv3x3_wino_wgrad_rows': 2.25,
                        're2e_conv4x4_wino': 64.0 / 25.0, 're2e_conv4x4_wino_wgrad': 64.0 / 25.0}
DIRECT = '(direct-form equivalent of all of the above)'


def count(name, args):
    fn = EXECUTED.get(name)
    if fn is not None:
        m = lib.FLOP_METER
        f = float(fn(*args))
        m[name] = m.get(name, 0.0) + f
        m[DIRECT] = m.get(DIRECT, 0.0) + f * DIRECT_OVER_EXECUTED.get(name, 1.0)


def totals(m):
    return sum(v for k, v in m.items() if k != DIRECT), m.get(DIRECT, 0.0)
```

### robust_e2e_gan_amd/joint_train.py

```python
import collections
import copy
import logging
import math
import os
import time

import numpy as np
import torch

from . import lib, ops
from . import dist as rdist
from .dist import GradSync
from .model.e2e_common import set_requires_grad
from .model.gan_model import CORAL, GANLoss, replay_running_stats
from .optim import FlatOptimizer

_LOSS_KIND = {'L2': lib.LOSS_L2, 'L1': lib.LOSS_L1, 'smooth_L1': lib.LOSS_SMOOTH_L1}

_Forward = collections.namedtuple('_Forward', 'enhance_out enhance_feat clean_feat clean_branch d_real')
_DFake = collections.namedtuple('_DFake', 'd_fake gan_loss stats bn_layers')


class stepwise_kernels(object):
    _KEYS = ('RE2E_LSTM_PERSIST', 'RE2E_LSTM_PERSIST_BWD')

    def __enter__(self):
        self.saved = {k: os.environ.get(k) for k in self._KEYS}
        for k in self._KEYS:
            os.environ[k] = '0'
        self.dec, ops.DECODER_PERSIST = ops.DECODER_PERSIST, False
        return self

    def __exit__(self, *exc):
        ops.DECODER_PERSIST = self.dec
        for k, v in self.saved.items():
            if v is None:
                os.environ.pop(k, None)
            else:
                os.environ[k] = v
        return False


def compute_cmvn_epoch(opt, train_loader, enhance_model, feat_model):
    enhance_model.eval()
    feat_model.eval()
    enhance_cmvn = None
    with torch.no_grad():
        for data in train_loader:
            mix_inputs, mix_log_inputs, input_sizes = data[4], data[5], data[8]
            enhance_out = enhance_model(mix_inputs, mix_log_inputs, input_sizes)
            enhance_cmvn = feat_model.compute_cmvn(enhance_out, input_sizes)
            if enhance_cmvn is not None:
                if getattr(opt, 'exp_path', None) and rdist.rank() == 0:
                    os.makedirs(opt.exp_path, exist_ok=True)
                    np.save(os.path.join(opt.exp_path, 'enhance_cmvn.npy'), enhance_cmvn)
                break
    enhance_model.train()
    feat_model.train()
    if rdist.any_rank(1 if enhance_cmvn is None else 0):
        raise RuntimeError('train_loader exhausted before cmvn_num utterances were accumulated'
                           + ('' if enhance_cmvn is None else ' (on another rank)'))
    return rdist.broadcast_(torch.FloatTensor(enhance_cmvn), 0)


def build_optimizers(opt, enhance_model, asr_model, gan_model=None):
    def mk(m):
        ps = [p for p in m.parameters() if p.requires_grad]
        if opt.opt_type == 'adadelta':
            return FlatOptimizer(ps, 'adadelta', rho=0.95, eps=opt.eps)
        return FlatOptimizer(ps, 'adam', lr=opt.lr, betas=(opt.beta1, 0.999), eps=1e-8)
    return mk(enhance_model), mk(asr_model), (mk(gan_model) if gan_model is not None else None)


class JointTrainer(object):
    def __init__(self, opt, enhance_model, feat_model, asr_model, gan_model=None):
        self.opt = opt
        self.enhance_model, self.feat_model, self.asr_model, self.gan_model = enhance_model, feat_model, asr_model, gan_model
        self.isGAN = bool(getattr(opt, 'isGAN', False)) and gan_model is not None
        if self.isGAN and getattr(opt, 'netD_type', 'basic') == 'pixel':
            raise lib.Re2eError('the joint loop cannot drive netD_type pixel: upstream reads an undefined mix_feat for it '
                                '(joint_train.py:178) and applies the 80-wide CMVN to the 160-wide concatenation')
        self.enhance_optimizer, self.asr_optimizer, self.gan_optimizer = build_optimizers(opt, enhance_model, asr_model,
                                                                                          gan_model if self.isGAN else None)
        self.criterionGAN = GANLoss(use_lsgan=not opt.no_lsgan) if self.isGAN else None
        self.asr_model.dec.return_acc_tensor = True
        self._gate = None
        self._step_no = 0
        if any(float(getattr(opt, k, 0.0) or 0.0) > 0.0 for k in ('dropout_rate', 'enhance_dropout_rate')):
            ops.dropout_seed(self._dropout_stream_seed(int(getattr(opt, 'seed', 1234))))
        self.overlap_dstep = os.environ.get('RE2E_NO_OVERLAP', '0') != '1'
        self.marks = [] if os.environ.get('RE2E_TIMELINE') else None
        self.main_stream = self.side_stream = self.wgrad_stream = None
        if torch.cuda.is_available():
            self.main_stream, self.side_stream, self.wgrad_stream = lib.step_streams(next(enhance_model.parameters()).device)

    def step(self, data, sche_samp_rate, enhance_cmvn):
        overlap = self.overlap_dstep
        with ops.routing(wgrad=self.wgrad_stream if overlap else None, aux=self.side_stream if overlap else None, marks=self.marks, multi=overlap,
                         sync_bn=bool(getattr(self.opt, 'sync_bn', False)) and rdist.world_size() > 1):
            if not (overlap and self.main_stream is not None):
                return self._step(data, sche_samp_rate, enhance_cmvn)
            caller = torch.cuda.current_stream()
            self.main_stream.wait_stream(caller)
            with torch.cuda.stream(self.main_stream):
                out = self._step(data, sche_samp_rate, enhance_cmvn)
            caller.wait_stream(self.main_stream)
            return out

    def _mark(self, label):
        if self.marks is not None:
            ev = torch.cuda.Event(enable_timing=True)
            ev.record()
            self.marks.append((label, time.perf_counter(), ev))

    def _mark_on(self, stream, label):
        if self.marks is not None:
            with torch.cuda.stream(stream):
                self._mark(label)

    def timeline(self):
        torch.cuda.synchronize()
        (l0, h0, e0), rows = self.marks[0], []
        for label, h, e in self.marks:
            rows.append((label, (h - h0) * 1e3, e0.elapsed_time(e)))
        self.marks = []
        return rows

    def _step(self, data, sche_samp_rate, enhance_cmvn):
        opt = self.opt
        self._mark('start')
        clean_inputs, mix_inputs, mix_log_inputs, targets, input_sizes, target_sizes = data[2], data[4], data[5], data[7], data[8], data[9]
        hold = self._hold_factor()
        fwd = self._enhancer_forward(clean_inputs, mix_inputs, mix_log_inputs, input_sizes, enhance_cmvn, hold)
        enhance_loss = opt.enhance_loss_lambda * ops.mean_loss(fwd.enhance_feat, fwd.clean_feat, 0.0, _LOSS_KIND[opt.enhance_loss_type])
        d_fwd = self._gstep_d_forward(fwd.enhance_feat, enhance_cmvn) if self.isGAN else None
        self._mark('fbank + G-step D fwd enqueued (side)')
        loss, out, asr_meters = self._asr_forward_and_loss(fwd, d_fwd, enhance_loss, targets, input_sizes, target_sizes, sche_samp_rate,
                                                           enhance_cmvn, hold)
        self.enhance_optimizer.zero_grad()
        self.asr_optimizer.zero_grad()
        sync = GradSync()
        armed = fwd.clean_branch is None
        if armed:
            sync.arm(fwd.enhance_feat, self.asr_optimizer, issue_stream=ops.WGRAD_STREAM, also_wait=[ops.AUX_STREAM])
        if self.isGAN and self.overlap_dstep:
            loss_D, armed = self._backward_two_phase(loss, fwd, d_fwd, enhance_cmvn, hold, sync, armed)
        else:
            loss_D = self._backward_single(loss, fwd)
        grad_norm, loss_D, aborts = self._update(fwd, d_fwd, loss_D, enhance_cmvn, hold, sync, armed)
        if self.isGAN:
            out['train/loss_D'] = loss_D.detach()
        out.update(asr_meters)
        out.update({'grad_norm': grad_norm.clone(),
                    'aborts': aborts.clone()})
        self.last = dict(enhance_out=fwd.enhance_out, enhance_feat=fwd.enhance_feat)
        self._mark('optimizers')
        return out

    def _enhancer_forward(self, clean_inputs, mix_inputs, mix_log_inputs, input_sizes, enhance_cmvn, hold):
        if not (self.overlap_dstep and getattr(self.asr_model, 'etype', '').startswith('vgg')):
            enhance_out = self.enhance_model(mix_inputs, mix_log_inputs, input_sizes)
            enhance_feat = self.feat_model(enhance_out)
            with torch.no_grad():
                clean_feat = self.feat_model(clean_inputs)
            return _Forward(enhance_out, enhance_feat, clean_feat, None, None)
        main, side = torch.cuda.current_stream(), self.side_stream
        side.wait_stream(main)
        with torch.cuda.stream(side):
            with torch.no_grad():
                clean_feat = self.feat_model(clean_inputs)
            ev_cf = torch.cuda.Event()
            ev_cf.record()
            clean_branch = self.asr_model.encode_clean(clean_feat, enhance_cmvn, input_sizes)
        self._mark('clean branch enqueued (side)')
        enhance_out = self.enhance_model(mix_inputs, mix_log_inputs, input_sizes)
        self._mark('enhancer fwd')
        d_real = None
        if self.isGAN:
            with torch.cuda.stream(side):
                d_real = self._d_real(clean_feat, enhance_cmvn, hold)
        ops.mark_grad(enhance_out, 'enhance_out (fbank bwd done)')
        enhance_feat = self.feat_model(enhance_out)
        ops.mark_grad(enhance_feat, 'enhance_feat (VGG, D, L1 bwd done)')
        main.wait_event(ev_cf)
        clean_feat.record_stream(main)
        return _Forward(enhance_out, enhance_feat, clean_feat, clean_branch, d_real)

    def _gstep_d_forward(self, enhance_feat, enhance_cmvn):
        set_requires_grad([self.gan_model], True)
        stats = []

        def forward():
            with ops.bn_stats(stats):
                d = self.gan_model(enhance_feat, enhance_cmvn)
            return d, self.opt.gan_loss_lambda * self.criterionGAN(d, True)
        if self.overlap_dstep:
            self.side_stream.wait_stream(torch.cuda.current_stream())
            with torch.cuda.stream(self.side_stream):
                enhance_feat.record_stream(self.side_stream)
                d_fake, gan_loss = forward()
                ops.mark_grad(d_fake, 'd_fake (side: G-step D bwd starts)')
        else:
            d_fake, gan_loss = forward()
        return _DFake(d_fake, gan_loss, stats, list(self.gan_model._bn_layers_last))

    def _asr_forward_and_loss(self, fwd, d_fwd, enhance_loss, targets, input_sizes, target_sizes, sche_samp_rate, enhance_cmvn, hold):
        opt = self.opt
        loss_ctc, loss_att, acc, _, _ = self.asr_model(
            fwd.clean_feat, fwd.enhance_feat, targets, input_sizes, target_sizes, sche_samp_rate, enhance_cmvn, clean_branch=fwd.clean_branch,
            context_loss=lambda cc, mc: opt.coral_loss_lambda * CORAL(cc, mc))
        self._mark('ASR fwd')
        coral_loss = self.asr_model.last_context_loss
        asr_loss = opt.mtlalpha * loss_ctc.view(()) + (1 - opt.mtlalpha) * loss_att
        loss = asr_loss + enhance_loss + coral_loss
        out = {}
        if d_fwd is not None:
            if self.overlap_dstep:
                torch.cuda.current_stream().wait_stream(self.side_stream)
            loss = loss + d_fwd.gan_loss
            out['train/gan_loss'] = opt.gan_loss_lambda * d_fwd.gan_loss.detach()
        out['train/loss'] = loss.detach()
        asr_meters = {'train/loss_ctc': loss_ctc.detach().view(()), 'train/acc': acc, 'train/loss_att': loss_att.detach(),
                      'train/enhance_loss': enhance_loss.detach(), 'train/coral_loss': coral_loss.detach()}
        return loss * hold, out, asr_meters

    def _take_clean_cut(self, clean_branch):
        cut = getattr(self.asr_model, 'clean_cut', None) if clean_branch is not None else None
        self.asr_model.clean_cut = None
        return cut

    def _clean_conv_backward(self, cut, grad, after):
        side = self.side_stream
        side.wait_event(after)
        with torch.cuda.stream(side):
            grad.record_stream(side)
            torch.autograd.backward([cut[0]], [grad])

    def _backward_single(self, loss, fwd):
        cut = self._take_clean_cut(fwd.clean_branch)
        with ops.frozen_params(self.gan_model if self.isGAN else ()):
            loss.backward(retain_graph=self.isGAN)
        if cut is not None and cut[1].grad is not None:
            self._clean_conv_backward(cut, cut[1].grad, torch.cuda.current_stream().record_event())
            cut[1].grad = None
        if self.overlap_dstep:
            torch.cuda.current_stream().wait_stream(self.side_stream)
        return None

    def _backward_two_phase(self, loss, fwd, d_fwd, enhance_cmvn, hold, sync, armed):
        main, side = torch.cuda.current_stream(), self.side_stream
        ev_fwd = torch.cuda.Event()
# ... 437 lines not shown
```

### robust_e2e_gan_amd/lib.py

```python
import atexit
import ctypes
import os
from ctypes import c_char_p, c_float, c_int, c_long, c_size_t, c_uint, c_ulonglong, c_void_p

import torch

_HERE = os.path.dirname(os.path.abspath(__file__))
LIB_PATH = os.environ.get('RE2E_LIB') or os.path.join(_HERE, 'libre2e_hip.so')
ABI_VERSION = 322

ACT_NONE, ACT_TANH, ACT_RELU, ACT_LRELU, ACT_SIGMOID, ACT_SIGMOID_MASK_MUL = range(6)
LOSS_L2, LOSS_L1, LOSS_SMOOTH_L1, LOSS_BCE = range(4)
EUNSUPPORTED = -2
STREAM_DEFAULT, STREAM_FILLER = 0, 1

P, I, L, F, Z = c_void_p, c_int, c_long, c_float, c_size_t

SIGNATURES = {
    're2e_version': (I, []),
    're2e_warmup': (I, []),
    're2e_last_error': (c_char_p, []),
    're2e_device_ok': (I, []),
    're2e_stream_role': (I, [P, I]),
    're2e_gemm_workspace_bytes': (Z, [I, I, I, I, I]),
    're2e_gemm': (I, [I, I, I, I, I, P, L, P, L, P, L, P, P, I, F, P, P, P, I, P, Z, P]),
    're2e_gemm_plan': (I, [I, I, I, I, I, I, I, I, I, I, I, I, P, Z]),
    're2e_gemm_nt_rows': (I, [I, I, I, P, L, P, L, P, L, P, P, I, F, P, I, I, P, Z, P]),
    're2e_gemm_tn_rows': (I, [I, I, I, P, L, P, L, P, L, F, P, I, I, P, Z, P]),
    're2e_fill_rows': (I, [P, L, I, P, I, F, P, I, P]),
    're2e_conv_igemm': (I, [P, I, I, I, I, P, I, I, I, I, I, I, I, I, I, I, I, P, I, I, I, I, I, I, P, I, F, P]),
    're2e_conv3x3_relu_pool': (I, [P, I, I, I, I, P, I, P, P, P, P]),
    're2e_conv_igemm_masked': (I, [P, I, I, I, I, P, I, I, I, I, I, I, I, I, I, I, I, P, I, I, I, I, I, I, P, P]),
    're2e_conv3x3_wino_workspace_bytes': (Z, [I, I]),
    're2e_conv3x3_wino': (I, [P, I, I, I, I, P, I, I, P, I, P, P, P, P, P, Z, P]),
    're2e_conv3x3_wino_wgrad_workspace_bytes': (Z, [I, I, I, I, I]),
    're2e_conv3x3_wino_wgrad': (I, [P, I, I, I, I, P, I, P, F, P, Z, P]),
    're2e_conv3x3_wino_rows': (I, [P, I, I, I, I, P, I, I, P, I, P, P, P, P, P, P, Z, P]),
    're2e_conv3x3_wino_wgrad_rows': (I, [P, I, I, I, I, P, I, P, F, P, P, Z, P]),
    're2e_fill_image_rows': (I, [P, I, I, L, P, I, I, F, P]),
    're2e_conv4x4_wino_workspace_bytes': (Z, [I, I, I, I, I, I]),
    're2e_conv4x4_wino': (I, [P, I, I, I, I, P, I, I, I, P, P, Z, P]),
    're2e_conv4x4_wino_wgrad_workspace_bytes': (Z, [I, I, I, I, I, I]),
    're2e_conv4x4_wino_wgrad': (I, [P, I, I, I, I, P, I, I, P, F, P, Z, P]),
    're2e_conv_wgrad_workspace_bytes': (Z, [I, I, I, I, I, I, I]),
    're2e_conv_wgrad': (I, [P, I, I, I, I, P, I, I, I, I, I, I, I, I, I, P, F, P, Z, P]),
    're2e_conv_dgrad_s2': (I, [P, I, I, I, I, P, I, I, I, I, I, I, P, P, P]),
    're2e_conv_weight_gather': (I, [P, P, I, I, I, I, I, I, I, I, I, I, P]),
    're2e_transpose01': (I, [P, P, I, I, I, P]),
    're2e_act_fwd': (I, [P, P, L, I, P]),
    're2e_act_bwd': (I, [P, P, P, L, I, P]),
    're2e_act_bwd_colsum': (I, [P, P, P, I, I, I, P, F, P, Z, P]),
    're2e_colsum_workspace_bytes': (Z, [I, I]),
    're2e_colsum': (I, [P, I, I, L, P, F, P, Z, P]),
    're2e_mask_mul_bwd': (I, [P, P, P, P, L, P]),
    're2e_mask_mul_bwd_ld': (I, [P, P, P, P, L, I, I, P]),
    're2e_mul': (I, [P, P, P, L, P]),
    're2e_affine_cols': (I, [P, P, P, P, L, I, P]),
    're2e_dropout': (I, [P, P, L, F, c_ulonglong, c_uint, P]),
    're2e_axpby': (I, [F, P, F, P, L, P]),
    're2e_gather_rows': (I, [P, P, P, I, I, P]),
    're2e_scatter_rows': (I, [P, P, P, I, I, P]),
    're2e_mask_rows': (I, [P, P, P, I, I, I, P]),
    're2e_pack_pad': (I, [P, P, P, I, I, I, P, P]),
    're2e_kaldi_decode_pad': (I, [P, P, P, P, I, I, I, P, P, P, P]),
    're2e_fbank_fwd': (I, [P, L, I, I, P, P, P, I, P, P, P, P, P]),
    're2e_fbank_bwd': (I, [P, L, I, I, P, P, P, I, P, P, P, P, P, P]),
    're2e_logclamp_fwd': (I, [P, P, L, I, P, P]),
    're2e_logclamp_bwd': (I, [P, P, L, I, P, P, P]),
    're2e_cmvn_stats': (I, [P, P, I, I, I, P, P, P]),
    're2e_reduce_workspace_bytes': (Z, [L]),
    're2e_loss_fwd': (I, [P, P, F, L, I, P, P, Z, P]),
    're2e_loss_bwd': (I, [P, P, F, L, I, P, F, P, F, P]),
    're2e_sumsq': (I, [P, L, P, P, Z, P]),
    're2e_maxpool2_fwd': (I, [P, I, I, I, I, P, P, I, P]),
    're2e_maxpool2_bwd': (I, [P, P, I, I, I, I, P, P]),
    're2e_vgg_pack_fwd': (I, [P, P, I, I, I, I, P, I, I, P]),
    're2e_vgg_pack_bwd': (I, [P, P, I, I, I, I, P, I, I, P]),
    're2e_bn_workspace_bytes': (Z, [L, I]),
    're2e_bn_lrelu_fwd': (I, [P, L, I, P, P, P, P, F, F, I, F, P, P, P, P, Z, P]),
    're2e_bn_lrelu_bwd': (I, [P, P, L, I, P, P, P, P, F, P, P, P, F, P, Z, P]),
    're2e_bn_sync_partial': (I, [P, L, I, P, I, P, P, Z, P]),
    're2e_bn_sync_finalize': (I, [P, P, L, I, F, F, P, P, P, P, P]),
    're2e_bn_apply': (I, [P, L, I, P, P, P, P, F, P, P]),
    're2e_bn_sync_bwd_partial': (I, [P, P, L, I, P, P, P, P, F, P, P, Z, P]),
    're2e_bn_sync_bwd_apply': (I, [P, P, L, I, P, P, P, P, F, P, P, P]),
    're2e_lstm_workspace_bytes': (Z, [I, I]),
    're2e_lstm_abort_count': (I, []),
    're2e_debug_force_abort': (I, [I]),
    're2e_debug_occupy': (I, [I, I, I, P]),
    're2e_step_gate': (I, [P, I, P, P, P, P, P, P, P]),
    're2e_lstm_seq_fwd': (I, [P, P, P, P, P, P, P, I, I, I, P, Z, P]),
    're2e_lstm_seq_bwd': (I, [P, P, P, P, P, P, P, P, P, I, I, I, P, P, Z, P]),
    're2e_lstm_plan': (I, [I, I, I, I, I, P, Z]),
    're2e_lstm_cell_fwd': (I, [P, P, P, P, I, I, P]),
    're2e_lstm_cell_bwd': (I, [P, P, P, P, P, P, P, I, I, P]),
    're2e_dec_gates_cell_fwd': (I, [P, P, P, L, P, P, P, P, P, I, I, I, P]),
    're2e_gemm_skinny2': (I, [I, I, P, L, P, L, I, P, L, P, L, I, P, L, P]),
    're2e_dec_loop_workspace_bytes': (Z, [I, I, I, I, I, I, I, I]),
    're2e_dec_loop_bwd_workspace_bytes': (Z, [I, I, I, I, I, I, I, I]),
    're2e_dec_loop_bwd': (I, [P, P, P, P, P, P, P, P, P, P, P, L, P, P, P, P, P, P, P, P, P, P, I, I, I, I, I, I, I, I, P, Z, P]),
    're2e_dec_loop_dwconv': (I, [P, P, P, Z, P, I, I, I, I, I, I, I, I, I, I, P]),
    're2e_dec_loop_fwd': (I, [P, P, P, P, P, P, P, P, P, L, P, P, P, P, P, P, P, P, I, I, I, I, I, I, I, I, P, Z, P]),
    're2e_embedding_fwd': (I, [P, P, I, I, P, L, P]),
    're2e_embedding_bwd': (I, [P, L, P, I, I, I, P, F, P]),
    're2e_lsm_fwd': (I, [P, P, I, I, I, P, P, Z, P]),
    're2e_lsm_bwd': (I, [P, P, I, I, I, P, P, P]),
    're2e_log_softmax_rows': (I, [P, I, I, L, P, P]),
    're2e_argmax_rows': (I, [P, I, I, L, P, P]),
    're2e_ce_fwd': (I, [P, P, I, I, F, P, P, P, Z, P]),
    're2e_ce_bwd': (I, [P, P, P, P, I, I, F, P, P, P]),
    're2e_ctc_workspace_bytes': (Z, [I, I, I]),
    're2e_ctc_fwd': (I, [P, I, I, I, P, P, P, P, I, P, P, P, Z, P]),
    're2e_ctc_bwd': (I, [P, I, I, I, P, P, P, P, I, P, P, P, I, P, P]),
    're2e_ctc_prefix_score': (I, [P, I, I, P, I, P, P, P, P, I, F, F, I, I, P, P, P, P, P]),
    're2e_ctc_prefix_score_cands': (I, [P, I, I, P, I, P, P, P, P, P, I, F, F, I, I, P, P, P, P]),
    're2e_attloc_fwd': (I, [P, P, P, P, P, P, P, P, P, P, I, I, I, I, I, I, I, P, P, L, P, P, P, P]),
    're2e_attloc_partial_floats': (Z, [I, I, I]),
    're2e_attloc_workspace_bytes': (Z, [I, I, I, I]),
    're2e_attloc_bwd': (I, [P, P, P, P, P, P, P, P, P, P, P, P, L, P, I, I, I, I, I, I, P, P, P, P, P, Z, P]),
    're2e_attloc_dpre': (I, [P, P, P, P, P, P, I, I, I, I, I, I, P, P, P, Z, P]),
    're2e_attloc_denc': (I, [P, P, I, I, I, I, P, F, P]),
    're2e_lm_lstm_cell': (I, [P, L, P, I, I, P, P, P, P, P, P, I, I, P, P, P]),
    're2e_lm_output': (I, [P, P, P, I, I, I, P, P]),
    're2e_lm_log_softmax_combine': (I, [P, I, I, P, F, P, P, P]),
    're2e_lm_add_cands': (I, [P, P, P, I, I, I, F, P]),
    're2e_clip_coef': (I, [P, F, P, P]),
    're2e_adadelta_step': (I, [P, P, P, P, L, F, F, F, P, P]),
    're2e_adam_step': (I, [P, P, P, P, L, F, F, F, F, I, P, P]),
}

def exp_env(name, default=None):
    return os.environ.get(name, default) if os.environ.get('RE2E_EXPERIMENTS') == '1' else default


_lib = None


class Re2eError(RuntimeError):
    pass


def load():
    global _lib
    if _lib is not None:
        return _lib
    if not os.path.exists(LIB_PATH):
        raise Re2eError('%s not found: build it with `python -c "import __graft_entry__ as g; g.build()"` '
                        '(hipcc --offload-arch=gfx950); there is no CPU fallback' % LIB_PATH)
    lib = ctypes.CDLL(LIB_PATH)
    lib.re2e_version.restype = ctypes.c_int
    got = lib.re2e_version()
    if got != ABI_VERSION:
        raise Re2eError('%s was built for ABI version %d, this binding is written for %d (include/re2e.h RE2E_ABI_VERSION): rebuild it '
                        'with `python -c "import __graft_entry__ as g; g.build()"`' % (LIB_PATH, got, ABI_VERSION))
    for name, (res, args) in SIGNATURES.items():
        fn = getattr(lib, name)
        fn.restype = res
        fn.argtypes = args
    _lib = lib
    try:
        if torch.cuda.is_available():
            lib.re2e_warmup()
    except Exception:
        pass
    return lib


def ptr(t):
    if t is None:
        return None
    if not t.is_cuda:
        raise Re2eError('expected a CUDA tensor, got device %s' % t.device)
    if not t.is_contiguous():
        raise Re2eError('expected a contiguous tensor')
    return t.data_ptr()


_raw_stream = getattr(torch._C, '_cuda_getCurrentRawStream', None)
_cur_device = getattr(torch._C, '_cuda_getDevice', None)


def stream():
    if _raw_stream is not None and _cur_device is not None:
        return _raw_stream(_cur_device())
    return torch.cuda.current_stream().cuda_stream


FLOP_METER = None


def call(name, *args):
    lib = load()
    rc = getattr(lib, name)(*args, stream())
    if rc != 0:
        raise Re2eError('%s failed (%d): %s' % (name, rc, lib.re2e_last_error().decode()))
    if FLOP_METER is not None:
        from . import flops
        flops.count(name, args)


def call_supported(name, *args):
    lib = load()
    rc = getattr(lib, name)(*args, stream())
    if rc == EUNSUPPORTED:
        return False
    if rc != 0:
        raise Re2eError('%s failed (%d): %s' % (name, rc, lib.re2e_last_error().decode()))
    if FLOP_METER is not None:
        from . import flops
        flops.count(name, args)
    return True


def set_stream_role(torch_stream, filler=True):
    lib = load()
    rc = lib.re2e_stream_role(c_void_p(torch_stream.cuda_stream), STREAM_FILLER if filler else STREAM_DEFAULT)
    if rc != 0:
        raise Re2eError('re2e_stream_role failed (%d): %s' % (rc, lib.re2e_last_error().decode()))


def query(name, *args):
    return getattr(load(), name)(*args)


def lstm_plan(T, B, H, backward=False, cus=0):
    buf = ctypes.create_string_buffer(160)
    lib = load()
    rc = lib.re2e_lstm_plan(T, B, H, int(backward), cus, buf, len(buf))
    if rc != 0:
        raise Re2eError('re2e_lstm_plan failed (%d): %s' % (rc, lib.re2e_last_error().decode()))
    return dict(kv.split('=') for kv in buf.value.decode().split())


def gemm_plan(transa, transb, M, N, K, act=ACT_NONE, aligned=(True, True, True), rowmap=False, filler=False, cus=0):
    buf = ctypes.create_string_buffer(256)
    lib = load()
    rc = lib.re2e_gemm_plan(int(transa), int(transb), M, N, K, int(aligned[0]), int(aligned[1]), int(aligned[2]), act, int(rowmap), int(filler), cus,
                            buf, len(buf))
    if rc != 0:
        raise Re2eError('re2e_gemm_plan failed (%d): %s' % (rc, lib.re2e_last_error().decode()))
    return dict(kv.split('=') for kv in buf.value.decode().split())


_STEP_STREAMS = {}


def step_streams(device=None, main_priority=-1):
    idx = torch.cuda.current_device() if device is None else (torch.device(device).index if torch.device(device).index is not None else torch.cuda.current_device())
    key = (idx, int(main_priority))
    got = _STEP_STREAMS.get(key)
    if got is None:
        with torch.cuda.device(idx):
            main = torch.cuda.Stream(priority=int(main_priority))
            side, wgrad = torch.cuda.Stream(), torch.cuda.Stream()
        set_stream_role(side, True)
        set_stream_role(wgrad, True)
        got = _STEP_STREAMS[key] = (main, side, wgrad)
    return got


_ws_cache = {}


def workspace(nbytes, device, tag='ws'):
    nbytes = max(int(nbytes), 16)
    key = (str(device), stream() if torch.cuda.is_available() else 0, tag)
    buf = _ws_cache.get(key)
    if buf is None or buf.numel() * 4 < nbytes:
        buf = torch.empty((nbytes + 3) // 4 + 1024, dtype=torch.float32, device=device)
        _ws_cache[key] = buf
    return buf


_hip = None


_masked_streams = []


def _destroy_masked_streams():
    try:
        _hip.hipStreamSynchronize.argtypes = [c_void_p]
        _hip.hipStreamDestroy.argtypes = [c_void_p]
        for h in _masked_streams:
            _hip.hipStreamSynchronize(c_void_p(h))
            _hip.hipStreamDestroy(c_void_p(h))
    except Exception:
        pass
    del _masked_streams[:]


def cu_masked_stream(enabled_cus, total_cus=256, device=None, first=0):
    global _hip
    try:
        if _hip is None:
            _hip = ctypes.CDLL('libamdhip64.so')
            _hip.hipExtStreamCreateWithCUMask.restype = c_int
            _hip.hipExtStreamCreateWithCUMask.argtypes = [ctypes.POINTER(c_void_p), ctypes.c_uint32, ctypes.POINTER(ctypes.c_uint32)]
        words = (total_cus + 31) // 32
        mask = (ctypes.c_uint32 * words)()
        for i in range(first, min(first + enabled_cus, total_cus)):
            mask[i // 32] |= (1 << (i % 32))
        st = c_void_p()
        rc = _hip.hipExtStreamCreateWithCUMask(ctypes.byref(st), words, mask)
        if rc != 0 or not st.value:
            return None
        if not _masked_streams and 'rocprof' in os.environ.get('LD_PRELOAD', ''):
            atexit.register(_destroy_masked_streams)
        _masked_streams.append(st.value)
        return torch.cuda.ExternalStream(st.value, device=device)
    except Exception:
        return None
```

### robust_e2e_gan_amd/ops.py

```python
import contextlib
import os
import time
import torch

from . import lib
from .lib import call, ptr, query, workspace

ACT = {None: lib.ACT_NONE, 'tanh': lib.ACT_TANH, 'relu': lib.ACT_RELU, 'lrelu': lib.ACT_LRELU, 'sigmoid': lib.ACT_SIGMOID}


def _f32(t):
    if t.dtype != torch.float32:
        t = t.float()
    return t if t.is_contiguous() else t.contiguous()


def _need_gpu(t):
    if not t.is_cuda:
        raise lib.Re2eError('robust_e2e_gan_amd ops run on the GPU only (no CPU fallback); got a %s tensor' % t.device)


def empty(shape, like):
    return torch.empty(shape, dtype=torch.float32, device=like.device)


def zeros(shape, like):
    return torch.zeros(shape, dtype=torch.float32, device=like.device)


def gemm(A, B, C, M, N, K, transa=False, transb=False, lda=None, ldb=None, ldc=None, bias=None, bias2=None,
         act=lib.ACT_NONE, beta=0.0, mul=None, mask_out=None, lens=None, T=0, dev=None):
    lda = lda if lda is not None else (M if transa else K)
    ldb = ldb if ldb is not None else (K if transb else N)
    ldc = ldc if ldc is not None else N
    wsb = query('re2e_gemm_workspace_bytes', int(transa), int(transb), M, N, K)
    ws = workspace(wsb, dev if dev is not None else A.device, 'gemm') if wsb else None
    _p = lambda t: t if isinstance(t, int) else t.data_ptr()
    call('re2e_gemm', int(transa), int(transb), M, N, K, _p(A), lda, _p(B), ldb, _p(C), ldc,
         ptr(bias), ptr(bias2), act, float(beta), ptr(mul), ptr(mask_out), ptr(lens), T, ptr(ws), wsb)
    return C


NT_INPUT_GRAD = lib.exp_env('RE2E_NO_NT_INPUT_GRAD') is None
INLINE_LAST_WGRAD = lib.exp_env('RE2E_NO_INLINE_LAST_WGRAD') is None
FUSED_DBIAS = lib.exp_env('RE2E_NO_FUSED_DBIAS') is None


def gemm_input_grad(dz, W, dx, M, K, N, beta=0.0):
    if NT_INPUT_GRAD and M >= 2048 and K % 4 == 0 and N % 4 == 0 and W.is_contiguous():
        wt = empty((K, N), dz)
        call('re2e_conv_weight_gather', W.data_ptr(), wt.data_ptr(), N, K, 1, 1, 1, 1, 1, 0, 0, 1)
        return gemm(dz, wt, dx, M, K, N, transb=True, beta=beta)
    return gemm(dz, W, dx, M, K, N, beta=beta)


ROW_MAPS = lib.exp_env('RE2E_NO_ROW_MAPS') is None
TN_ROW_MAPS = lib.exp_env('RE2E_NO_TN_ROW_MAPS') is None
ROW_IDENT = lib.exp_env('RE2E_NO_ROW_IDENT') is None
ROW_MAPS_MIN_K = 384
ROW_MAPS_MIN_PAD = 0.04


class RowMaps(object):
    __slots__ = ('valid', 'invalid', 'nv', 'ni', 'rows', 'ident')

    def __init__(self, valid, invalid, nv, ni, rows, ident):
        self.valid, self.invalid, self.nv, self.ni, self.rows, self.ident = valid, invalid, nv, ni, rows, ident


_ROW_MAPS = {}


def row_maps(lens_d, T, B):
    if not ROW_MAPS or lens_d is None:
        return None
    from .model import e2e_common as ec
    lens = ec.host_lens_of(lens_d)
    if lens is None or len(lens) != B:
        return None
    key = (lens, T, B, str(lens_d.device))
    hit = _ROW_MAPS.get(key)
    if hit is None:
        import numpy as np
        ln = np.minimum(np.asarray(lens, np.int64), T)
        ok = (np.arange(T, dtype=np.int64)[:, None] < ln[None, :]).reshape(-1)
        idx = np.arange(T * B, dtype=np.int32)
        v_ = idx[ok]
        neq = np.nonzero(v_ != idx[:v_.size])[0]
        hit = (v_, idx[~ok], int(neq[0]) if neq.size else int(v_.size))
        while len(_ROW_MAPS) >= 64:
            _ROW_MAPS.pop(next(iter(_ROW_MAPS)))
        _ROW_MAPS[key] = hit
    v, iv, ident = hit
    if v.size < 256 or iv.size < ROW_MAPS_MIN_PAD * T * B:
        return None
    dev = lens_d.device
    return RowMaps(ec.dev_cached(('rows_v',) + key, lambda: v, dev), ec.dev_cached(('rows_i',) + key, lambda: iv, dev), int(v.size), int(iv.size), T * B,
                   ident if ROW_IDENT else 0)


def gemm_rows(A, B, C, N, K, maps, lda=None, ldb=None, ldc=None, bias=None, bias2=None, act=lib.ACT_NONE, beta=0.0, fill=False):
    if fill and bias2 is not None:
        raise lib.Re2eError('gemm_rows(fill=True) takes one bias')
    lda = lda if lda is not None else K
    ldb = ldb if ldb is not None else K
    ldc = ldc if ldc is not None else N
    if K < ROW_MAPS_MIN_K and not fill:
        return gemm(A, B, C, maps.rows, N, K, transb=True, lda=lda, ldb=ldb, ldc=ldc, bias=bias, bias2=bias2, act=act, beta=beta)
    wsb = query('re2e_gemm_workspace_bytes', 0, 1, maps.nv, N, K)
    ws = workspace(wsb, A.device, 'gemm') if wsb else None
    _p = lambda t: t if isinstance(t, int) else t.data_ptr()
    if lib.call_supported('re2e_gemm_nt_rows', maps.nv, N, K, _p(A), lda, _p(B), ldb, _p(C), ldc, ptr(bias), ptr(bias2), act, float(beta),
                          maps.valid.data_ptr(), maps.ident, maps.rows, ptr(ws), wsb):
        if fill and N % 4 == 0 and ldc % 4 == 0:
            call('re2e_fill_rows', _p(C), ldc, N, maps.invalid.data_ptr(), maps.ni, 0.0, ptr(bias), act if bias is not None else lib.ACT_NONE)
        return C
    return gemm(A, B, C, maps.rows, N, K, transb=True, lda=lda, ldb=ldb, ldc=ldc, bias=bias, bias2=bias2, act=act, beta=beta)


def gemm_input_grad_rows(dz, W, dx, K, N, maps, beta=0.0, fill=False):
    if K % 4 == 0 and N % 4 == 0 and W.is_contiguous():
        wt = empty((K, N), dz)
        call('re2e_conv_weight_gather', W.data_ptr(), wt.data_ptr(), N, K, 1, 1, 1, 1, 1, 0, 0, 1)
        return gemm_rows(dz, wt, dx, K, N, maps, beta=beta, fill=fill)
    return gemm_input_grad(dz, W, dx, maps.rows, K, N, beta=beta)


def gemm_tn_rows(A, B, C, M, N, maps, beta=0.0, lda=None, ldb=None, ldc=None):
    lda = lda if lda is not None else M
    ldb = ldb if ldb is not None else N
    ldc = ldc if ldc is not None else N
    wsb = query('re2e_gemm_workspace_bytes', 1, 0, M, N, maps.nv)
    ws = workspace(wsb, A.device if not isinstance(A, int) else C.device, 'gemm') if wsb else None
    _p = lambda t: t if isinstance(t, int) else t.data_ptr()
    if TN_ROW_MAPS and lib.call_supported('re2e_gemm_tn_rows', M, N, maps.nv, _p(A), lda, _p(B), ldb, _p(C), ldc, float(beta), maps.valid.data_ptr(), maps.ident,
                          maps.rows, ptr(ws), wsb):
        return C
    wsb = query('re2e_gemm_workspace_bytes', 1, 0, M, N, maps.rows)
    ws = workspace(wsb, C.device, 'gemm') if wsb else None
    call('re2e_gemm', 1, 0, M, N, maps.rows, _p(A), lda, _p(B), ldb, _p(C), ldc, None, None, lib.ACT_NONE, float(beta), None, None, None, 0, ptr(ws), wsb)
    return C


def colsum_into(A2d, M, N, out, beta, lda=None):
    wsb = query('re2e_colsum_workspace_bytes', M, N)
    ws = workspace(wsb, A2d.device, 'colsum')
    call('re2e_colsum', A2d.data_ptr(), M, N, lda if lda is not None else N, out.data_ptr(), float(beta), ws.data_ptr(), wsb)


MULTI_STREAM = False
WGRAD_STREAM = None
AUX_STREAM = None
FROZEN_PARAMS = frozenset()
MARKS = None
SYNC_BN = False
BN_DEFER_RUNNING = False
BN_STATS_SINK = None


@contextlib.contextmanager
def _ambient(**values):
    g = globals()
    prev = {k: g[k] for k in values}
    g.update(values)
    try:
        yield
    finally:
        g.update(prev)


def routing(wgrad=None, aux=None, marks=None, sync_bn=False, multi=None):
    multi = (wgrad is not None or aux is not None) if multi is None else bool(multi)
    return _ambient(MULTI_STREAM=multi, WGRAD_STREAM=wgrad, AUX_STREAM=aux, MARKS=marks, SYNC_BN=bool(sync_bn))


def inline_weight_grads():
    return _ambient(WGRAD_STREAM=None)


def frozen_params(module_or_params):
    ps = module_or_params.parameters() if hasattr(module_or_params, 'parameters') else module_or_params
    return _ambient(FROZEN_PARAMS=frozenset(id(p) for p in ps))


def bn_stats(sink, defer=False):
    return _ambient(BN_STATS_SINK=sink, BN_DEFER_RUNNING=bool(defer))


def mark_grad(t, label):
    if MARKS is not None and isinstance(t, torch.Tensor) and t.requires_grad:
        marks = MARKS

        def hook(g):
            ev = torch.cuda.Event(enable_timing=True)
            ev.record()
            marks.append(('  grad of ' + label, time.perf_counter(), ev))
        t.register_hook(hook)
    return t


def mark(label):
    if MARKS is not None:
        ev = torch.cuda.Event(enable_timing=True)
        ev.record()
        MARKS.append(('  ' + label, time.perf_counter(), ev))


def _wants(ctx, i, p):
    return ctx.needs_input_grad[i] and (p is None or id(p) not in FROZEN_PARAMS)


class param_grads(object):
    __slots__ = ('ts', 'ctx', 'inline')

    def __init__(self, *tensors, inline=False):
        self.ts = tensors
        self.ctx = None
        self.inline = inline

    def __enter__(self):
        ws = WGRAD_STREAM
        if not MULTI_STREAM or ws is None or self.inline:
            return self
        cur = torch.cuda.current_stream()
        if cur == ws:
            return self
        ev = torch.cuda.Event()
        ev.record(cur)
        ws.wait_event(ev)
        for t in self.ts:
            if isinstance(t, torch.Tensor):
                t.record_stream(ws)
            elif t is not None:
                for name in t.__slots__:
                    v = getattr(t, name)
                    if isinstance(v, torch.Tensor):
                        v.record_stream(ws)
        self.ctx = torch.cuda.stream(ws)
        self.ctx.__enter__()
        return self

    def __exit__(self, *exc):
        if self.ctx is not None:
            self.ctx.__exit__(*exc)
            self.ctx = None
        return False


class accumulate(object):
    __slots__ = ('p',)

    def __init__(self, p):
        self.p = p

    def __enter__(self):
        p = self.p
        if MULTI_STREAM:
            ev = getattr(p, '_re2e_ev', None)
            if ev is not None:
                torch.cuda.current_stream().wait_event(ev)
        if p.grad is None:
            p.grad = torch.empty_like(p)
            return p.grad, 0.0
        return p.grad, 1.0

    def __exit__(self, *exc):
        if MULTI_STREAM:
            ev = torch.cuda.Event()
            ev.record()
            self.p._re2e_ev = ev
        return False


def act_bwd(dy, y, act):
    if act == lib.ACT_NONE:
        return dy
    dz = torch.empty_like(dy)
    call('re2e_act_bwd', dy.data_ptr(), y.data_ptr(), dz.data_ptr(), dy.numel(), act)
    return dz


def act_bwd_bias(dy2, y, act, b, b_needs_grad=None):
    if b_needs_grad is None:
        b_needs_grad = b is not None and b.requires_grad
    if act == lib.ACT_NONE or b is None or not b_needs_grad:
        return act_bwd(dy2, y, act), False
    M, N = dy2.shape
    dz = torch.empty_like(dy2)
    wsb = query('re2e_colsum_workspace_bytes', M, N)
    ws = workspace(wsb, dy2.device, 'colsum')
    with accumulate(b) as (gb, beta):
        call('re2e_act_bwd_colsum', dy2.data_ptr(), y.data_ptr(), dz.data_ptr(), M, N, act, gb.data_ptr(), float(beta), ws.data_ptr(), wsb)
    return dz, True


_PADDED_GRADS = {}


def _linear_backward_padded(ctx, dy, x2, W, b, M, K, N, Np, need_w, need_b):
    dzp = dy.as_strided((M, Np), (Np, 1))
    dx = None
    if ctx.needs_input_grad[0]:
        wt = zeros((K, Np), dzp)
        wt[:, :N].copy_(W.t())
        dx = empty((M, K), x2)
        gemm(dzp, wt, dx, M, K, Np, transb=True)
        dx = dx.view(ctx.xshape)
    with param_grads(dzp, x2):
        if need_w:
            tmp = empty((Np, K), x2)
            gemm(dzp, x2, tmp, Np, K, M, transa=True)
            with accumulate(W) as (gw, beta):
                if beta:
                    gw.add_(tmp[:N])
                else:
                    gw.copy_(tmp[:N])
        if b is not None and need_b:
            with accumulate(b) as (gb, beta):
                colsum_into(dzp, M, N, gb, beta, lda=Np)
    return dx, None, None, None, None


class LinearFn(torch.autograd.Function):
    @staticmethod
    def forward(ctx, x, W, b, act, maps=None):
        _need_gpu(x)
# ... 687 lines not shown
def sync_bn_flags():
    return list(_SYNC_BN_RAGGED.values())


def check_sync_bn(counts=None):
    if counts is None:
        counts = [float(c.item()) for c in _SYNC_BN_RAGGED.values()]
    n = int(sum(counts))
    if n:
        for c in _SYNC_BN_RAGGED.values():
            c.zero_()
        raise lib.Re2eError('synchronised BatchNorm needs the same number of rows on every rank (%d BatchNorm calls saw ranks with different '
                            'row counts; their statistics were poisoned with NaN and no update was applied): shard equal utterance '
                            'counts of equal padded length, or leave opt.sync_bn off' % n)


class BnLreluFn(torch.autograd.Function):

    @staticmethod
    def forward(ctx, x, gamma, beta, rm, rv, train, momentum, eps, slope=0.2):
        _need_gpu(x)
        x = _f32(x)
        C = x.shape[-1]
        Pn = x.numel() // C
        y = empty(x.shape, x)
        sm, si = empty((C,), x), empty((C,), x)
        wsb = query('re2e_bn_workspace_bytes', Pn, C)
        ws = workspace(wsb, x.device, 'bn')
        defer = BN_DEFER_RUNNING and BN_STATS_SINK is not None and train
        world = _sync_world() if train else 1
        ctx.ptot = Pn
        if world > 1:
            from . import dist as rdist
            acc = empty((C,), x)
            call('re2e_bn_sync_partial', x.data_ptr(), Pn, C, None, 0, acc.data_ptr(), ws.data_ptr(), wsb)
            rdist.allreduce_sum_(acc)
            ptot = Pn * world
            mean = (acc / float(ptot) + _sync_rows_poison(Pn, x.device)).contiguous()
            var = empty((C,), x)
            call('re2e_bn_sync_partial', x.data_ptr(), Pn, C, mean.data_ptr(), 1, var.data_ptr(), ws.data_ptr(), wsb)
            rdist.allreduce_sum_(var)
            var = (var / float(ptot)).contiguous()
            call('re2e_bn_sync_finalize', mean.data_ptr(), var.data_ptr(), ptot, C, 0.0 if defer else float(momentum), float(eps), rm.data_ptr(),
                 rv.data_ptr(), sm.data_ptr(), si.data_ptr())
            call('re2e_bn_apply', x.data_ptr(), Pn, C, sm.data_ptr(), si.data_ptr(), gamma.data_ptr(), beta.data_ptr(), float(slope), y.data_ptr())
            ctx.ptot = ptot
        else:
            call('re2e_bn_lrelu_fwd', x.data_ptr(), Pn, C, gamma.data_ptr(), beta.data_ptr(), rm.data_ptr(), rv.data_ptr(),
                 0.0 if defer else float(momentum), float(eps), int(train), float(slope), y.data_ptr(), sm.data_ptr(), si.data_ptr(), ws.data_ptr(), wsb)
        ctx.gamma, ctx.beta, ctx.train, ctx.slope = gamma, beta, train, float(slope)
        ctx.save_for_backward(x, sm, si)
        if BN_STATS_SINK is not None and train:
            BN_STATS_SINK.append((rm, rv, sm, si, ctx.ptot, float(momentum), float(eps)))
        return y

    @staticmethod
    def backward(ctx, dy):
        x, sm, si = ctx.saved_tensors
        if not ctx.train:
            raise lib.Re2eError('BatchNorm backward is implemented for train mode only')
        gamma, beta = ctx.gamma, ctx.beta
        C = x.shape[-1]
        Pn = x.numel() // C
        dy = _f32(dy)
        dx = empty(x.shape, x)
        wsb = query('re2e_bn_workspace_bytes', Pn, C)
        ws = workspace(wsb, x.device, 'bn')
        if ctx.ptot != Pn:
            from . import dist as rdist
            sums = empty((2 * C,), x)
            call('re2e_bn_sync_bwd_partial', dy.data_ptr(), x.data_ptr(), Pn, C, gamma.data_ptr(), beta.data_ptr(), sm.data_ptr(), si.data_ptr(),
                 ctx.slope, sums.data_ptr(), ws.data_ptr(), wsb)
            if _wants(ctx, 1, gamma):
                with accumulate(gamma) as (dg, gbeta), accumulate(beta) as (db, _):
                    if gbeta:
                        dg.add_(sums[C:]); db.add_(sums[:C])
                    else:
                        dg.copy_(sums[C:]); db.copy_(sums[:C])
            tot = sums.clone()
            rdist.allreduce_sum_(tot)
            tot.mul_(float(Pn) / float(ctx.ptot))
            call('re2e_bn_sync_bwd_apply', dy.data_ptr(), x.data_ptr(), Pn, C, gamma.data_ptr(), beta.data_ptr(), sm.data_ptr(), si.data_ptr(),
                 ctx.slope, tot.data_ptr(), dx.data_ptr())
            return dx, None, None, None, None, None, None, None, None
        if _wants(ctx, 1, gamma):
            with accumulate(gamma) as (dg, gbeta), accumulate(beta) as (db, _):
                call('re2e_bn_lrelu_bwd', dy.data_ptr(), x.data_ptr(), Pn, C, gamma.data_ptr(), beta.data_ptr(), sm.data_ptr(), si.data_ptr(),
                     ctx.slope, dx.data_ptr(), dg.data_ptr(), db.data_ptr(), gbeta, ws.data_ptr(), wsb)
        else:
            call('re2e_bn_lrelu_bwd', dy.data_ptr(), x.data_ptr(), Pn, C, gamma.data_ptr(), beta.data_ptr(), sm.data_ptr(), si.data_ptr(),
                 ctx.slope, dx.data_ptr(), None, None, 0.0, ws.data_ptr(), wsb)
        return dx, None, None, None, None, None, None, None, None


class InstanceNormLreluFn(torch.autograd.Function):

    @staticmethod
    def forward(ctx, x, eps, slope):
        _need_gpu(x)
        x = _f32(x).contiguous()
        N, C = x.shape[0], x.shape[-1]
        Pn = x.numel() // (N * C)
        y = empty(x.shape, x)
        sm, si = empty((N, C), x), empty((N, C), x)
        ones, zero = torch.ones(C, device=x.device), torch.zeros(C, device=x.device)
        rm, rv = torch.zeros(C, device=x.device), torch.ones(C, device=x.device)
        wsb = query('re2e_bn_workspace_bytes', Pn, C)
        ws = workspace(wsb, x.device, 'bn')
        st = Pn * C * 4
        for n in range(N):
            call('re2e_bn_lrelu_fwd', x.data_ptr() + n * st, Pn, C, ones.data_ptr(), zero.data_ptr(), rm.data_ptr(), rv.data_ptr(), 0.0, float(eps), 1,
                 float(slope), y.data_ptr() + n * st, sm[n].data_ptr(), si[n].data_ptr(), ws.data_ptr(), wsb)
        ctx.save_for_backward(x, sm, si, ones, zero)
        ctx.slope = float(slope)
        return y

    @staticmethod
    def backward(ctx, dy):
        x, sm, si, ones, zero = ctx.saved_tensors
        N, C = x.shape[0], x.shape[-1]
        Pn = x.numel() // (N * C)
        dy = _f32(dy).contiguous()
        dx = empty(x.shape, x)
        wsb = query('re2e_bn_workspace_bytes', Pn, C)
        ws = workspace(wsb, x.device, 'bn')
        st = Pn * C * 4
        for n in range(N):
            call('re2e_bn_lrelu_bwd', dy.data_ptr() + n * st, x.data_ptr() + n * st, Pn, C, ones.data_ptr(), zero.data_ptr(), sm[n].data_ptr(),
                 si[n].data_ptr(), ctx.slope, dx.data_ptr() + n * st, None, None, 0.0, ws.data_ptr(), wsb)
        return dx, None, None


def instance_norm_lrelu(x, eps=1e-5, slope=0.2):
    return InstanceNormLreluFn.apply(x, eps, slope)


def bn_lrelu(x, gamma, beta, rm, rv, train=True, momentum=0.1, eps=1e-5, slope=0.2):
    return BnLreluFn.apply(x, gamma, beta, rm, rv, train, momentum, eps, slope)


class BiLstmFn(torch.autograd.Function):

    @staticmethod
    def forward(ctx, x, lens_dev, *w):
        _need_gpu(x)
        x = _f32(x)
        T, B, I = x.shape
        H = w[1].shape[1]
        x2 = x.view(T * B, I)
        maps = row_maps(lens_dev, T, B)
        ctx.maps = maps
        xg = [empty((T * B, 4 * H), x), empty((T * B, 4 * H), x)]
        Ip = (I + 3) & ~3
        if Ip != I and T * B >= 1024 and lib.exp_env('RE2E_NO_PAD_INPUT') != '1':
            x2p = zeros((T * B, Ip), x)
            x2p[:, :I].copy_(x2)
            for d in range(2):
                wp = zeros((4 * H, Ip), x)
                wp[:, :I].copy_(w[4 * d].detach())
                if maps is not None:
                    gemm_rows(x2p, wp, xg[d], 4 * H, Ip, maps, bias=w[4 * d + 2], bias2=w[4 * d + 3])
                else:
                    gemm(x2p, wp, xg[d], T * B, 4 * H, Ip, transb=True, bias=w[4 * d + 2], bias2=w[4 * d + 3])
            x2 = x2p
        else:
            for d in range(2):
                if maps is not None and w[4 * d].is_contiguous():
                    gemm_rows(x2, w[4 * d], xg[d], 4 * H, I, maps, bias=w[4 * d + 2], bias2=w[4 * d + 3])
                else:
                    gemm(x2, w[4 * d], xg[d], T * B, 4 * H, I, transb=True, bias=w[4 * d + 2], bias2=w[4 * d + 3])
        ybuf = empty((T + 2, B, 2 * H), x)
        cbuf = empty((T + 2, B, 2 * H), x)
        for buf in (ybuf, cbuf):
            buf[0].zero_()
            buf[T + 1].zero_()
        wsb = query('re2e_lstm_workspace_bytes', B, H)
        ws = workspace(wsb, x.device, 'lstm')
        call('re2e_lstm_seq_fwd', xg[0].data_ptr(), xg[1].data_ptr(), w[1].data_ptr(), w[5].data_ptr(), ybuf.data_ptr(), cbuf.data_ptr(),
             lens_dev.data_ptr(), T, B, H, ws.data_ptr(), wsb)
        ctx.w, ctx.lens = w, lens_dev
        ctx.save_for_backward(x2, xg[0], xg[1], ybuf, cbuf)
        ctx.dims = (T, B, I, H)
        return ybuf[1:T + 1]

    @staticmethod
    def backward(ctx, dy):
        x2, g_f, g_r, ybuf, cbuf = ctx.saved_tensors
        w = ctx.w
        T, B, I, H = ctx.dims
        dy = _f32(dy)
        dc = empty((B, 2 * H), dy)
        wsb = query('re2e_lstm_workspace_bytes', B, H)
        ws = workspace(wsb, dy.device, 'lstm')
        dbias = empty((2, 4 * H), dy) if any(ctx.needs_input_grad[4 + 4 * d] or ctx.needs_input_grad[5 + 4 * d] for d in range(2)) else None
        if dbias is not None and not FUSED_DBIAS:
            dbias = None
        call('re2e_lstm_seq_bwd', g_f.data_ptr(), g_r.data_ptr(), w[1].data_ptr(), w[5].data_ptr(), dy.data_ptr(), ybuf.data_ptr(),
             cbuf.data_ptr(), dc.data_ptr(), ctx.lens.data_ptr(), T, B, H, ptr(dbias), ws.data_ptr(), wsb)
        dG = (g_f, g_r)
        M = T * B
        dx = None
        if ctx.needs_input_grad[0]:
            dx = empty((M, I), dy)
            if ctx.maps is not None and I % 4 == 0:
                gemm_input_grad_rows(dG[0], w[0], dx, I, 4 * H, ctx.maps, fill=True)
                gemm_input_grad_rows(dG[1], w[4], dx, I, 4 * H, ctx.maps, beta=1.0)
            else:
                gemm_input_grad(dG[0], w[0], dx, M, I, 4 * H)
                gemm_input_grad(dG[1], w[4], dx, M, I, 4 * H, beta=1.0)
            dx = dx.view(T, B, I)
        yflat = ybuf.view((T + 2) * B, 2 * H)
        last = INLINE_LAST_WGRAD and not ctx.needs_input_grad[0]
        needs = ctx.needs_input_grad

        def weight_grads(inline):
            with param_grads(g_f, g_r, x2, ybuf, dbias, ctx.maps, inline=inline):
                for d in range(2):
                    w_ih, w_hh, b_ih, b_hh = w[4 * d:4 * d + 4]
                    n_ih, n_hh, n_bi, n_bh = needs[2 + 4 * d:6 + 4 * d]
                    mp = ctx.maps
                    if n_ih and x2.shape[1] != I:
                        tmp = empty((4 * H, x2.shape[1]), dy)
                        if mp is not None:
                            gemm_tn_rows(dG[d], x2, tmp, 4 * H, x2.shape[1], mp)
                        else:
                            gemm(dG[d], x2, tmp, 4 * H, x2.shape[1], M, transa=True)
                        with accumulate(w_ih) as (gw, beta):
                            if beta == 0.0:
                                gw.copy_(tmp[:, :I])
                            else:
                                gw.add_(tmp[:, :I])
                    elif n_ih:
                        with accumulate(w_ih) as (gw, beta):
                            if mp is not None:
                                gemm_tn_rows(dG[d], x2, gw, 4 * H, I, mp, beta=beta)
                            else:
                                gemm(dG[d], x2, gw, 4 * H, I, M, transa=True, beta=beta)
                    if n_hh:
                        hprev = yflat[(0 if d == 0 else 2 * B):, d * H:]
                        with accumulate(w_hh) as (gw, beta):
                            if mp is not None:
                                gemm_tn_rows(dG[d], hprev.data_ptr(), gw, 4 * H, H, mp, beta=beta, lda=4 * H, ldb=2 * H)
                            else:
                                call_gemm_strided(dG[d], hprev, gw, 4 * H, H, M, lda=4 * H, ldb=2 * H, beta=beta)
                    csum = dbias[d] if dbias is not None else None
                    if csum is None and (n_bi or n_bh):
                        csum = empty((4 * H,), dy)
                        colsum_into(dG[d], M, 4 * H, csum, 0.0)
                    for b_, need in ((b_ih, n_bi), (b_hh, n_bh)):
                        if need:
                            with accumulate(b_) as (gb, beta):
                                if beta == 0.0:
                                    gb.copy_(csum)
                                else:
                                    gb.add_(csum)

        weight_grads(last)
        return (dx, None) + (None,) * len(w)


def call_gemm_strided(A, Bview, C, M, N, K, lda, ldb, beta):
    wsb = query('re2e_gemm_workspace_bytes', 1, 0, M, N, K)
    ws = workspace(wsb, A.device, 'gemm') if wsb else None
    call('re2e_gemm', 1, 0, M, N, K, A.data_ptr(), lda, Bview.data_ptr(), ldb, C.data_ptr(), N, None, None, lib.ACT_NONE, float(beta),
         None, None, None, 0, ptr(ws), wsb)


def bilstm(x_tm, lens_dev, weights):
    return BiLstmFn.apply(x_tm, lens_dev, *weights)


class CtcFn(torch.autograd.Function):

    @staticmethod
    def forward(ctx, logits, hlens_dev, labels_dev, loff_dev, llen_dev, Lmax):
        _need_gpu(logits)
        logits = _f32(logits)
        T, B, V = logits.shape
        wsb = query('re2e_ctc_workspace_bytes', T, B, Lmax)
        ws = torch.empty(wsb // 4 + 4, dtype=torch.float32, device=logits.device)
        loss = empty((1,), logits)
        nll = empty((B,), logits)
        call('re2e_ctc_fwd', logits.data_ptr(), T, B, V, hlens_dev.data_ptr(), labels_dev.data_ptr(), loff_dev.data_ptr(), llen_dev.data_ptr(),
             Lmax, loss.data_ptr(), nll.data_ptr(), ws.data_ptr(), wsb)
        ctx.save_for_backward(logits, ws, nll)
        ctx.meta = (hlens_dev, labels_dev, loff_dev, llen_dev, Lmax)
        return loss

    @staticmethod
    def backward(ctx, g):
        logits, ws, nll = ctx.saved_tensors
        hlens_dev, labels_dev, loff_dev, llen_dev, Lmax = ctx.meta
        T, B, V = logits.shape
        g = _f32(g).reshape(1)
        Vp = (V + 15) // 16 * 16 if (V % 4 and T * B >= 2048) else V
        d = empty((T, B, Vp), logits)
        call('re2e_ctc_bwd', logits.data_ptr(), T, B, V, hlens_dev.data_ptr(), labels_dev.data_ptr(), loff_dev.data_ptr(), llen_dev.data_ptr(),
             Lmax, nll.data_ptr(), g.data_ptr(), d.data_ptr(), Vp, ws.data_ptr())
        if Vp != V:
            if len(_PADDED_GRADS) > 8:
                _PADDED_GRADS.clear()
            _PADDED_GRADS[d.data_ptr()] = (T * B, V, Vp)
            d = d[..., :V]
        return d, None, None, None, None, None


ctc_loss = CtcFn.apply


class GatherRowsFn(torch.autograd.Function):
    @staticmethod
    def forward(ctx, src2d, idx_dev):
        src2d = _f32(src2d)
        n, W = idx_dev.numel(), src2d.shape[1]
        out = empty((n, W), src2d)
        call('re2e_gather_rows', src2d.data_ptr(), idx_dev.data_ptr(), out.data_ptr(), n, W)
        ctx.idx, ctx.shape = idx_dev, src2d.shape
        return out

    @staticmethod
    def backward(ctx, dy):
        dy = _f32(dy)
        dx = zeros(ctx.shape, dy)
        call('re2e_scatter_rows', dy.data_ptr(), ctx.idx.data_ptr(), dx.data_ptr(), ctx.idx.numel(), ctx.shape[1])
        return dx, None


gather_rows = GatherRowsFn.apply


class CoralFn(torch.autograd.Function):

# ... 404 lines not shown
```

### robust_e2e_gan_amd/trainers.py

```python
import contextlib
import os

import torch

from . import lib, ops
from .dist import GradSync
from .joint_train import _LOSS_KIND
from .model.e2e_common import set_requires_grad
from .model.gan_model import GANLoss
from .optim import FlatOptimizer


def make_optimizer(opt, module):
    ps = [p for p in module.parameters() if p.requires_grad]
    if opt.opt_type == 'adadelta':
        return FlatOptimizer(ps, 'adadelta', rho=0.95, eps=opt.eps)
    return FlatOptimizer(ps, 'adam', lr=opt.lr, betas=(opt.beta1, 0.999), eps=1e-8)


def _update(optimizer, max_norm):
    GradSync().finish([optimizer])
    gn = optimizer.clip_grad_norm(max_norm)
    optimizer.step()
    return gn


class StepStreams(object):

    def __init__(self):
        self.on = torch.cuda.is_available() and os.environ.get('RE2E_NO_OVERLAP', '0') != '1'
        self.main = self.side = self.wgrad = None
        if self.on:
            self.main, self.side, self.wgrad = lib.step_streams()

    @contextlib.contextmanager
    def step(self):
        if not self.on:
            yield None
            return
        caller = torch.cuda.current_stream()
        self.main.wait_stream(caller)
        try:
            with ops.routing(wgrad=self.wgrad, aux=self.side, multi=True), torch.cuda.stream(self.main):
                yield self
                torch.cuda.current_stream().wait_stream(self.wgrad)
                torch.cuda.current_stream().wait_stream(self.side)
        finally:
            caller.wait_stream(self.main)

    def join(self):
        torch.cuda.current_stream().wait_stream(self.wgrad)


class EnhanceBaseTrainer(object):

    def __init__(self, opt, enhance_model):
        self.opt, self.enhance_model = opt, enhance_model
        self.enhance_optimizer = make_optimizer(opt, enhance_model)
        self.streams = StepStreams()

    def step(self, data):
        clean_inputs, mix_inputs, mix_log_inputs, cos_angles, input_sizes = data[2], data[4], data[5], data[6], data[8]
        with self.streams.step() as st:
            loss, enhance_out = self.enhance_model(mix_inputs, mix_log_inputs, input_sizes, clean_inputs, cos_angles)
            self.enhance_optimizer.zero_grad()
            loss.backward()
            if st is not None:
                st.join()
            gn = _update(self.enhance_optimizer, self.opt.grad_clip)
        self.last = dict(enhance_out=enhance_out)
        return {'train/loss': loss.detach(), 'grad_norm': gn}


class EnhanceFbankTrainer(object):

    def __init__(self, opt, enhance_model, feat_model):
        self.opt, self.enhance_model, self.feat_model = opt, enhance_model, feat_model
        self.enhance_optimizer = make_optimizer(opt, enhance_model)
        self.streams = StepStreams()

    def step(self, data):
        clean_inputs, mix_inputs, mix_log_inputs, input_sizes = data[2], data[4], data[5], data[8]
        with self.streams.step() as st:
            enhance_out = self.enhance_model(mix_inputs, mix_log_inputs, input_sizes)
            enhance_feat = self.feat_model(enhance_out)
            with torch.no_grad():
                clean_feat = self.feat_model(clean_inputs)
            loss = ops.mean_loss(enhance_feat, clean_feat, 0.0, _LOSS_KIND[self.opt.enhance_loss_type])
            self.enhance_optimizer.zero_grad()
            loss.backward()
            if st is not None:
                st.join()
            gn = _update(self.enhance_optimizer, self.opt.grad_clip)
        self.last = dict(enhance_out=enhance_out, enhance_feat=enhance_feat)
        return {'train/loss': loss.detach(), 'grad_norm': gn}


class EnhanceGanTrainer(object):

    def __init__(self, opt, enhance_model, feat_model, gan_model):
        self.opt, self.enhance_model, self.feat_model, self.gan_model = opt, enhance_model, feat_model, gan_model
        self.enhance_optimizer = make_optimizer(opt, enhance_model)
        self.gan_optimizer = make_optimizer(opt, gan_model)
        self.criterionGAN = GANLoss(use_lsgan=not opt.no_lsgan)
        self.streams = StepStreams()

    def step(self, data, enhance_cmvn):
        with self.streams.step() as st:
            return self._step_streams(data, enhance_cmvn, st) if st is not None else self._step_plain(data, enhance_cmvn)

    def _step_plain(self, data, enhance_cmvn):
        opt = self.opt
        clean_inputs, mix_inputs, mix_log_inputs, cos_angles, input_sizes = data[2], data[4], data[5], data[6], data[8]
        enhance_loss, enhance_out = self.enhance_model(mix_inputs, mix_log_inputs, input_sizes, clean_inputs, cos_angles)
        enhance_feat = self.feat_model(enhance_out, enhance_cmvn)
        with torch.no_grad():
            clean_feat = self.feat_model(clean_inputs, enhance_cmvn)
        set_requires_grad([self.gan_model], False)
        gan_loss = self.criterionGAN(self.gan_model(enhance_feat), True)
        self.enhance_optimizer.zero_grad()
        loss = enhance_loss + opt.gan_loss_lambda * gan_loss
        loss.backward()
        gn = _update(self.enhance_optimizer, opt.grad_clip)
        set_requires_grad([self.gan_model], True)
        self.gan_optimizer.zero_grad()
        loss_D = (self.criterionGAN(self.gan_model(clean_feat.detach()), True)
                  + self.criterionGAN(self.gan_model(enhance_feat.detach()), False)) * 0.5
        loss_D.backward()
        gnD = _update(self.gan_optimizer, opt.grad_clip)
        self.last = dict(enhance_out=enhance_out, enhance_feat=enhance_feat)
        return {'train/loss': loss.detach(), 'train/gan_loss': gan_loss.detach(), 'train/enhance_loss': enhance_loss.detach(),
                'train/loss_D': loss_D.detach(), 'grad_norm': gn, 'grad_norm_D': gnD}

    def _step_streams(self, data, enhance_cmvn, st):
        opt = self.opt
        clean_inputs, mix_inputs, mix_log_inputs, cos_angles, input_sizes = data[2], data[4], data[5], data[6], data[8]
        main, side = torch.cuda.current_stream(), st.side
        enhance_loss, enhance_out = self.enhance_model(mix_inputs, mix_log_inputs, input_sizes, clean_inputs, cos_angles)
        enhance_feat = self.feat_model(enhance_out, enhance_cmvn)
        with torch.no_grad():
            clean_feat = self.feat_model(clean_inputs, enhance_cmvn)
        set_requires_grad([self.gan_model], False)
        gan_loss = self.criterionGAN(self.gan_model(enhance_feat), True)
        self.enhance_optimizer.zero_grad()
        loss = enhance_loss + opt.gan_loss_lambda * gan_loss
        (g_eo,) = torch.autograd.grad(loss, [enhance_out])
        set_requires_grad([self.gan_model], True)
        ev = torch.cuda.Event()
        ev.record(main)
        side.wait_event(ev)
        with torch.cuda.stream(side):
            fake, real = enhance_feat.detach(), clean_feat.detach()
            fake.record_stream(side)
            real.record_stream(side)
            self.gan_optimizer.zero_grad()
            loss_D = (self.criterionGAN(self.gan_model(real), True) + self.criterionGAN(self.gan_model(fake), False)) * 0.5
            loss_D.backward()
            st.join()
            gnD = _update(self.gan_optimizer, opt.grad_clip)
            for t_ in (loss_D, gnD):
                t_.record_stream(main)
        enhance_out.backward(g_eo)
        st.join()
        gn = _update(self.enhance_optimizer, opt.grad_clip)
        main.wait_stream(side)
        self.last = dict(enhance_out=enhance_out, enhance_feat=enhance_feat)
        return {'train/loss': loss.detach(), 'train/gan_loss': gan_loss.detach(), 'train/enhance_loss': enhance_loss.detach(),
                'train/loss_D': loss_D.detach(), 'grad_norm': gn, 'grad_norm_D': gnD}


class AsrTrainer(object):

    def __init__(self, opt, asr_model):
        self.opt, self.asr_model = opt, asr_model
        self.optimizer = make_optimizer(opt, asr_model)
        self.asr_model.dec.return_acc_tensor = True
        self.streams = StepStreams()

    def step(self, data, sche_samp_rate=0.0):
        fbank_features, targets, input_sizes, target_sizes = data[2], data[3], data[4], data[5]
        with self.streams.step() as st:
            loss_ctc, loss_att, acc = self.asr_model(fbank_features, targets, input_sizes, target_sizes, sche_samp_rate)[:3]
            loss = self.opt.mtlalpha * loss_ctc.view(()) + (1 - self.opt.mtlalpha) * loss_att
            self.optimizer.zero_grad()
            loss.backward()
            if st is not None:
                st.join()
            gn = _update(self.optimizer, self.opt.grad_clip)
        return {'train/loss': loss.detach(), 'train/loss_ctc': loss_ctc.detach().view(()), 'train/acc': acc, 'train/loss_att': loss_att.detach(),
                'grad_norm': gn}
```

Measured before the change: 687.4 utterances/s.

## Pipeline BiLSTM input projection with recurrent scan across time segments on feed stream

Adds a bilstm_fwd_pipe entry point that splits the time axis into segments. It computes each segment's input-projection GEMM on a separate high-priority feed stream while the persistent recurrent LSTM kernel processes earlier segments. To support this, the LSTM kernels gain a step range and can resume mid-sequence from h and c already written to ybuf and cbuf. The segment count comes from a cost model that is gated behind an experiment env flag, so by default the plan is a single segment and no overlap happens. The trade-off is extra kernel launches and event syncs when it is enabled, plus a reworked projection path when it is not.

Result: no change. 682.1 utterances/s (-0.8%).

```diff
diff --git a/include/re2e.h b/include/re2e.h
--- a/include/re2e.h
+++ b/include/re2e.h
@@ -27,7 +27,7 @@
 
 #define RE2E_LOSS_BCE 3
 
-#define RE2E_ABI_VERSION 322
+#define RE2E_ABI_VERSION 323
 int re2e_version(void);
 const char* re2e_last_error(void);
 int re2e_device_ok(void);
@@ -167,6 +167,16 @@
 int re2e_lstm_seq_fwd(float* xg_f, float* xg_r, const float* whh_f, const float* whh_r, float* ybuf, float* cbuf,
                       const int* lens_dev, int T, int B, int H, void* workspace, size_t workspace_bytes,
                       re2e_stream_t stream);
+int re2e_lstm_seq_fwd_range(float* xg_f, float* xg_r, const float* whh_f, const float* whh_r, float* ybuf, float* cbuf,
+                            const int* lens_dev, int T, int B, int H, int s_begin, int s_end, void* workspace, size_t workspace_bytes,
+                            re2e_stream_t stream);
+int re2e_bilstm_fwd_pipe(const float* x, long ldx, int K, const float* wih_f, const float* wih_r, long ldw, const float* bih_f, const float* bhh_f,
+                         const float* bih_r, const float* bhh_r, float* xg_f, float* xg_r, const float* whh_f, const float* whh_r, float* ybuf,
+                         float* cbuf, const int* lens_dev, int T, int B, int H, const int* valid_dev, int nvalid, int ident,
+                         const int* t_off_host, int segments, void* lstm_ws, size_t lstm_ws_bytes, void* gemm_ws, size_t gemm_ws_bytes,
+                         re2e_stream_t feed, re2e_stream_t stream);
+size_t re2e_bilstm_pipe_workspace_bytes(int T, int B, int H, int K, const int* t_off_host, int segments, int have_feed);
+int re2e_bilstm_pipe_plan(int T, int B, int H, long rows, int N, int K, int cus, int segments, int have_feed, char* out, size_t out_bytes);
 int re2e_lstm_seq_bwd(float* g_f, float* g_r, const float* whh_f, const float* whh_r, const float* dy,
                       const float* ybuf, const float* cbuf, float* dc_state, const int* lens_dev, int T, int B, int H,
                       float* dbias, void* workspace, size_t workspace_bytes, re2e_stream_t stream);
diff --git a/robust_e2e_gan_amd/csrc/bilstm_pipe.hip b/robust_e2e_gan_amd/csrc/bilstm_pipe.hip
--- /dev/null
+++ b/robust_e2e_gan_amd/csrc/bilstm_pipe.hip
@@ -0,0 +1,182 @@
+#include <mutex>
+
+#include "common.h"
+
+int re2e_lstm_fwd_resident_(int T, int B, int H, int cus);
+
+namespace {
+
+constexpr int kMaxSeg = 64;
+constexpr int kRowMapsMinK = 384;
+
+hipEvent_t next_event() {
+  constexpr int kPool = 256;
+  static std::mutex mu;
+  static hipEvent_t pool[16][kPool];
+  static unsigned made[16] = {0}, next[16] = {0};
+  int dev = 0;
+  if (hipGetDevice(&dev) != hipSuccess || dev < 0 || dev >= 16) return nullptr;
+  std::lock_guard<std::mutex> g(mu);
+  const unsigned i = next[dev]++ % kPool;
+  if (i >= made[dev]) {
+    if (hipEventCreateWithFlags(&pool[dev][i], hipEventDisableTiming) != hipSuccess) { --next[dev]; return nullptr; }
+    made[dev] = i + 1;
+  }
+  return pool[dev][i];
+}
+
+bool order_after(hipStream_t waiter, hipStream_t from) {
+  hipEvent_t e = next_event();
+  return e && hipEventRecord(e, from) == hipSuccess && hipStreamWaitEvent(waiter, e, 0) == hipSuccess;
+}
+
+constexpr double kSegUs = 6.0;
+constexpr double kMinGainUs = 30.0;
+double chain_step_us(int H) { return H >= 384 ? 5.2 : 3.2; }
+int min_segment_steps(int H) { return (int)(kSegUs / (0.02 * chain_step_us(H)) + 0.999); }
+
+struct PipePlan { int K; int s[kMaxSeg + 1]; int min_len; };
+
+bool rule_on() { const char* v = exp_env("RE2E_LSTM_PIPE_RULE"); return v && atoi(v) == 1; }
+bool pipe_off() { const char* v = getenv("RE2E_LSTM_PIPE"); return v && atoi(v) == 0; }
+
+PipePlan plan_pipe(int T, int B, int H, long rows, int N, int Kd, int cus, int segments, bool have_feed) {
+  PipePlan p;
+  p.min_len = min_segment_steps(H);
+  int K = 1;
+  const bool resident = re2e_lstm_fwd_resident_(T, B, H, cus) != 0;
+  if (segments > 0) K = segments;
+  else if (resident && have_feed && !pipe_off() && rule_on()) {
+    const double prod_us = 2.0 * 2.0 * (double)rows * N * Kd / 100e6;
+    const int kmax = T / p.min_len < kMaxSeg ? T / p.min_len : kMaxSeg;
+    double best = 0.0;
+    for (int k = 2; k <= kmax; ++k) {
+      const double gain = prod_us * (1.0 - 1.0 / k) - (k - 1) * kSegUs;
+      if (gain > best + 1e-9 && gain >= kMinGainUs) { best = gain; K = k; }
+    }
+  }
+  if (!have_feed || K > T) K = have_feed ? T : 1;
+  if (K > kMaxSeg) K = kMaxSeg;
+  if (K < 1) K = 1;
+  p.K = K;
+  for (int k = 0; k <= K; ++k) p.s[k] = (int)((long)k * T / K);
+  return p;
+}
+
+struct Layer {
+  const float* x; long ldx; int Kd;
+  const float* wih[2]; long ldw;
+  const float* bih[2]; const float* bhh[2];
+  float* xg[2];
+  int T, B, H;
+  const int* valid; int nvalid, ident; const int* t_off;
+};
+
+size_t project_ws(const Layer& L, int t0, int t1) {
+  const int N = 4 * L.H;
+  size_t need = re2e_gemm_workspace_bytes(0, 1, (t1 - t0) * L.B, N, L.Kd);
+  if (L.valid && L.Kd >= kRowMapsMinK) {
+    const int r0 = L.t_off[t0], r1 = L.t_off[t1];
+    if (r1 > r0) { const size_t b = re2e_gemm_workspace_bytes(0, 1, r1 - r0, N, L.Kd); if (b > need) need = b; }
+  }
+  return need;
+}
+
+int project(const Layer& L, int d, int t0, int t1, void* ws, size_t wsb, hipStream_t st) {
+  const int N = 4 * L.H;
+  long row0 = (long)t0 * L.B;
+  int M = (t1 - t0) * L.B;
+  if (L.valid && L.Kd >= kRowMapsMinK) {
+    const int r0 = L.t_off[t0], r1 = L.t_off[t1];
+    if (r1 == r0) return RE2E_OK;
+    if (r1 <= L.ident) { row0 = r0; M = r1 - r0; }
+    else {
+      const int rc = re2e_gemm_nt_rows(r1 - r0, N, L.Kd, L.x, L.ldx, L.wih[d], L.ldw, L.xg[d], N, L.bih[d], L.bhh[d], RE2E_ACT_NONE, 0.f, L.valid + r0,
+                                       r0 == 0 ? (L.ident < r1 ? L.ident : r1) : 0, L.T * L.B, ws, wsb, st);
+      if (rc != RE2E_EUNSUPPORTED) return rc;
+    }
+  }
+  return re2e_gemm(0, 1, M, N, L.Kd, L.x + row0 * L.ldx, L.ldx, L.wih[d], L.ldw, L.xg[d] + row0 * N, N, L.bih[d], L.bhh[d], RE2E_ACT_NONE, 0.f, nullptr, nullptr,
+                   nullptr, 0, ws, wsb, st);
+}
+
+size_t align256(size_t b) { return (b + 255) & ~(size_t)255; }
+
+}
+
+extern "C" int re2e_bilstm_pipe_plan(int T, int B, int H, long rows, int N, int K, int cus, int segments, int have_feed, char* out, size_t out_bytes) {
+  RE2E_CHECK_ARG(T > 0 && B > 0 && H > 0 && rows > 0 && N > 0 && K > 0 && cus >= 0 && segments >= 0 && out && out_bytes > 0, "bad argument");
+  if (H % 8 != 0) { re2e_set_error("re2e_bilstm_pipe_plan: hidden size must be a multiple of 8 (got %d)", H); return RE2E_EUNSUPPORTED; }
+  if (cus == 0) cus = re2e_cu_count();
+  const PipePlan p = plan_pipe(T, B, H, rows, N, K, cus, segments, have_feed != 0);
+  int n = snprintf(out, out_bytes, "segments=%d min_len=%d bounds=", p.K, p.min_len);
+  for (int k = 0; k <= p.K && n > 0 && (size_t)n < out_bytes; ++k) n += snprintf(out + n, out_bytes - n, k ? ",%d" : "%d", p.s[k]);
+  RE2E_CHECK_ARG(n > 0 && (size_t)n < out_bytes, "out_bytes too small");
+  return RE2E_OK;
+}
+
+extern "C" size_t re2e_bilstm_pipe_workspace_bytes(int T, int B, int H, int K, const int* t_off_host, int segments, int have_feed) {
+  if (T <= 0 || B <= 0 || H <= 0 || H % 8 || K <= 0) return 0;
+  const PipePlan p = plan_pipe(T, B, H, (long)T * B, 4 * H, K, re2e_cu_count(), segments, have_feed != 0);
+  Layer L;
+  memset(&L, 0, sizeof(L));
+  L.Kd = K; L.T = T; L.B = B; L.H = H; L.t_off = t_off_host; L.valid = t_off_host ? reinterpret_cast<const int*>(1) : nullptr;
+  size_t need = 0;
+  for (int k = 0; k < p.K; ++k)
+    for (int d = 0; d < 2; ++d) {
+      const size_t b = d ? project_ws(L, T - p.s[k + 1], T - p.s[k]) : project_ws(L, p.s[k], p.s[k + 1]);
+      if (b > need) need = b;
+    }
+  return 2 * align256(need);
+}
+
+extern "C" int re2e_bilstm_fwd_pipe(const float* x, long ldx, int K, const float* wih_f, const float* wih_r, long ldw, const float* bih_f, const float* bhh_f,
+                                    const float* bih_r, const float* bhh_r, float* xg_f, float* xg_r, const float* whh_f, const float* whh_r, float* ybuf,
+                                    float* cbuf, const int* lens_dev, int T, int B, int H, const int* valid_dev, int nvalid, int ident,
+                                    const int* t_off_host, int segments, void* lstm_ws, size_t lstm_ws_bytes, void* gemm_ws, size_t gemm_ws_bytes,
+                                    hipStream_t feed, hipStream_t stream) {
+  RE2E_CHECK_ARG(x && wih_f && wih_r && xg_f && xg_r && whh_f && whh_r && ybuf && cbuf && lens_dev && lstm_ws, "null arg");
+  RE2E_CHECK_ARG(T > 0 && B > 0 && H > 0 && K > 0 && ldx >= K && ldw >= K && segments >= 0, "bad shape");
+  RE2E_CHECK_ARG(!valid_dev || (t_off_host && nvalid > 0 && ident >= 0 && ident <= nvalid && t_off_host[0] == 0 && t_off_host[T] == nvalid), "bad row map");
+  RE2E_CHECK_ARG(feed != stream || feed == nullptr, "feed must be another stream than the caller's (or null)");
+  if (H % 8 != 0) { re2e_set_error("re2e_bilstm_fwd_pipe: hidden size must be a multiple of 8 (got %d)", H); return RE2E_EUNSUPPORTED; }
+  const bool have_feed = feed != nullptr;
+  const PipePlan p = plan_pipe(T, B, H, (long)T * B, 4 * H, K, re2e_cu_count(), segments, have_feed);
+  Layer L = {x, ldx, K, {wih_f, wih_r}, ldw, {bih_f, bih_r}, {bhh_f, bhh_r}, {xg_f, xg_r}, T, B, H, valid_dev, nvalid, ident, t_off_host};
+  size_t need = 0;
+  for (int k = 0; k < p.K; ++k)
+    for (int d = 0; d < 2; ++d) {
+      const size_t b = d ? project_ws(L, T - p.s[k + 1], T - p.s[k]) : project_ws(L, p.s[k], p.s[k + 1]);
+      if (b > need) need = b;
+    }
+  need = align256(need);
+  RE2E_CHECK_ARG(need == 0 || (gemm_ws && gemm_ws_bytes >= 2 * need), "product workspace too small (re2e_bilstm_pipe_workspace_bytes)");
+  void* ws_main = gemm_ws;
+  void* ws_feed = gemm_ws ? (char*)gemm_ws + need : nullptr;
+  for (int d = 0; d < 2; ++d)
+    if (const int rc = d ? project(L, 1, T - p.s[1], T, ws_main, need, stream) : project(L, 0, 0, p.s[1], ws_main, need, stream)) return rc;
+  hipEvent_t ready[kMaxSeg + 1] = {nullptr};
+  if (p.K > 1) {
+    if (!order_after(feed, stream)) { re2e_set_error("re2e_bilstm_fwd_pipe: no event to be had"); return RE2E_EHIP; }
+    for (int k = 1; k < p.K; ++k) {
+      for (int d = 0; d < 2; ++d)
+        if (const int rc = d ? project(L, 1, T - p.s[k + 1], T - p.s[k], ws_feed, need, feed) : project(L, 0, p.s[k], p.s[k + 1], ws_feed, need, feed)) {
+          (void)order_after(stream, feed);
+          return rc;
+        }
+      ready[k] = next_event();
+      if (!ready[k] || hipEventRecord(ready[k], feed) != hipSuccess) {
+        (void)hipStreamSynchronize(feed);
+        re2e_set_error("re2e_bilstm_fwd_pipe: no event to be had");
+        return RE2E_EHIP;
+      }
+    }
+  }
+  int rc = RE2E_OK;
+  for (int k = 0; k < p.K && rc == RE2E_OK; ++k) {
+    if (k > 0 && hipStreamWaitEvent(stream, ready[k], 0) != hipSuccess) { re2e_set_error("re2e_bilstm_fwd_pipe: hipStreamWaitEvent failed"); rc = RE2E_EHIP; break; }
+    rc = re2e_lstm_seq_fwd_range(xg_f, xg_r, whh_f, whh_r, ybuf, cbuf, lens_dev, T, B, H, p.s[k], p.s[k + 1], lstm_ws, lstm_ws_bytes, stream);
+  }
+  if (rc != RE2E_OK && p.K > 1) (void)order_after(stream, feed);
+  return rc;
+}
diff --git a/robust_e2e_gan_amd/csrc/lstm.hip b/robust_e2e_gan_amd/csrc/lstm.hip
--- a/robust_e2e_gan_amd/csrc/lstm.hip
+++ b/robust_e2e_gan_amd/csrc/lstm.hip
@@ -149,7 +149,7 @@
 template <int WAVES, int QN, int UW>
 __global__ __launch_bounds__(WAVES * 64) void lstm_fwd_persist(float* xg_f, float* xg_r, const float* __restrict__ wfrag, float* ybuf,
                                                                float* cbuf, u64* hx_, unsigned* err, const int* __restrict__ lens,
-                                                               int T, int B, int H) {
+                                                               int T, int B, int H, int s_begin, int s_end) {
   extern __shared__ __attribute__((aligned(16))) float red[];
   static_assert(WAVES >= 4 * UW, "256 threads per 8 units own the 32 x 8 cell updates");
   const int dir = blockIdx.z, mt = blockIdx.y, MT = gridDim.y, NX = gridDim.x * UW;
@@ -159,7 +159,7 @@
   float* xg = dir ? xg_r : xg_f;
   const int j0 = x * 8, b0 = mt * 32;
   constexpr int kAbort = UW * WAVES * 32 * 33;
-  if (tid == 0) red[kAbort] = 0.f;
+  if (tid == 0) red[kAbort] = (s_begin > 0 && *err != 0u) ? 1.f : 0.f;
   const long H2 = 2L * H;
   f32x4 w[UW][QN];
 #pragma unroll
@@ -180,13 +180,15 @@
   const int wr_off = grp + x * 256 + ((jj >> 2) * 32 + bm) * 4 + (jj & 3);
   float c = 0.f, pre[4] = {0.f, 0.f, 0.f, 0.f};
   if (ok) {
-    const float* gp = xg + ((long)(dir ? T - 1 : 0) * B + b) * 4 * H + j;
+    const int t0 = dir ? T - 1 - s_begin : s_begin;
+    const float* gp = xg + ((long)t0 * B + b) * 4 * H + j;
 #pragma unroll
     for (int g = 0; g < 4; ++g) pre[g] = gp[g * H];
+    if (s_begin > 0) c = cbuf[((long)(dir ? t0 + 2 : t0) * B + b) * H2 + dir * H + j];
   }
   LSTM_STAMP_DECL;
   __syncthreads();
-  for (int s = 0; s < T; ++s) {
+  for (int s = s_begin; s < s_end; ++s) {
     const int t = dir ? T - 1 - s : s;
     LSTM_STAMP(0); LSTM_STAMP(10);
     f32x16 acc[UW];
@@ -195,23 +197,31 @@
 #pragma unroll
       for (int r = 0; r < 16; ++r) acc[u][r] = 0.f;
     if (s > 0) {
-      const gu64* src = hx + ((s & 1) ^ 1) * par_sz + rd_off;
       float hv[QN][4];
-      const unsigned rd_b = (unsigned)((((s & 1) ^ 1) * par_sz + rd_off) * 8);
-      for (unsigned spins = 0;; ++spins) {
-        asm volatile("" ::: "memory");
-        bool good = true;
+      if (s == s_begin) {
+        const f32x4* hp = reinterpret_cast<const f32x4*>(ybuf + ((long)(dir ? t + 2 : t) * B + (b0 + lr < B ? b0 + lr : 0)) * H2 + dir * H + 8 * wid * QN + 4 * lh);
 #pragma unroll
         for (int q = 0; q < QN; ++q) {
-          const u32x4 lo = __builtin_amdgcn_raw_buffer_load_b128(hx_rs, rd_b + (unsigned)q * 2048u, 0, 16);
-          const u32x4 hi = __builtin_amdgcn_raw_buffer_load_b128(hx_rs, rd_b + (unsigned)q * 2048u + 16u, 0, 16);
-          hv[q][0] = __uint_as_float(lo[0]); hv[q][1] = __uint_as_float(lo[2]);
-          hv[q][2] = __uint_as_float(hi[0]); hv[q][3] = __uint_as_float(hi[2]);
-          good &= (lo[1] == (unsigned)s) & (lo[3] == (unsigned)s) & (hi[1] == (unsigned)s) & (hi[3] == (unsigned)s);
+          const f32x4 v = b0 + lr < B ? hp[2 * q] : f32x4{0.f, 0.f, 0.f, 0.f};
+          hv[q][0] = v[0]; hv[q][1] = v[1]; hv[q][2] = v[2]; hv[q][3] = v[3];
         }
-        if (__all(good)) break;
-        if (spins > kSpinLimit) { if (lane == 0) { red[kAbort] = 1.f; if (atomicExch(err, 1u) == 0u) atomicAdd(&g_persist_aborts, 1u); } break; }
-        __builtin_amdgcn_s_sleep(1);
+      } else {
+        const unsigned rd_b = (unsigned)((((s & 1) ^ 1) * par_sz + rd_off) * 8);
+        for (unsigned spins = 0;; ++spins) {
+          asm volatile("" ::: "memory");
+          bool good = true;
+#pragma unroll
+          for (int q = 0; q < QN; ++q) {
+            const u32x4 lo = __builtin_amdgcn_raw_buffer_load_b128(hx_rs, rd_b + (unsigned)q * 2048u, 0, 16);
+            const u32x4 hi = __builtin_amdgcn_raw_buffer_load_b128(hx_rs, rd_b + (unsigned)q * 2048u + 16u, 0, 16);
+            hv[q][0] = __uint_as_float(lo[0]); hv[q][1] = __uint_as_float(lo[2]);
+            hv[q][2] = __uint_as_float(hi[0]); hv[q][3] = __uint_as_float(hi[2]);
+            good &= (lo[1] == (unsigned)s) & (lo[3] == (unsigned)s) & (hi[1] == (unsigned)s) & (hi[3] == (unsigned)s);
+          }
+          if (__all(good)) break;
+          if (spins > kSpinLimit) { if (lane == 0) { red[kAbort] = 1.f; if (atomicExch(err, 1u) == 0u) atomicAdd(&g_persist_aborts, 1u); } break; }
+          __builtin_amdgcn_s_sleep(1);
+        }
       }
       LSTM_STAMP(1);
 #pragma unroll
@@ -241,7 +251,7 @@
       float h = go * tanhf_(cn);
       if (t >= ln) { cn = 0.f; h = 0.f; }
       c = cn;
-      if (ok && s + 1 < T) {
+      if (ok && s + 1 < s_end) {
         const float* gp = xg + ((long)(dir ? t - 1 : t + 1) * B + b) * 4 * H + j;
 #pragma unroll
         for (int g = 0; g < 4; ++g) pre[g] = gp[g * H];
@@ -277,7 +287,7 @@
 template <int TILES, int NJ, bool PERSIST>
 __global__ __launch_bounds__(256) void lstm_fwd2(float* xg_f, float* xg_r, const float* __restrict__ whh_f, const float* __restrict__ whh_r,
                                                  float* ybuf, float* cbuf, unsigned* hx_, unsigned* err, const int* __restrict__ lens, int T,
-                                                 int B, int H, int s_arg) {
+                                                 int B, int H, int s_arg, int s_end) {
   constexpr int KS = 4;
   extern __shared__ __attribute__((aligned(16))) float lds2[];
   f32x4* part = reinterpret_cast<f32x4*>(lds2);
@@ -288,7 +298,7 @@
   float* xg = dir ? xg_r : xg_f;
   const float* whh = dir ? whh_r : whh_f;
   const long H2 = 2L * H;
-  if (PERSIST && tid == 0) *abortw = 0;
+  if (PERSIST && tid == 0) *abortw = (s_arg > 0 && *err != 0u) ? 1 : 0;
   f32x4 w[TILES][NJ];
 #pragma unroll
   for (int t = 0; t < TILES; ++t) {
@@ -300,7 +310,7 @@
   const __amdgpu_buffer_rsrc_t hx_rs = __builtin_amdgcn_make_buffer_rsrc(hx_, 0, (int)(2 * par_w * 4), 0x00020000);
   const bool fin = ft >= 0;
   const int j = 4 * TILES * x + 4 * (fin ? ft : 0) + kk;
-  const int s0 = PERSIST ? 0 : s_arg, s1 = PERSIST ? T : s_arg + 1;
+  const int s0 = s_arg, s1 = PERSIST ? s_end : s_arg + 1;
   const int grp = (dir * MT + mt) * H * 16;
   const int b = 16 * mt + n;
   const unsigned rd_w = (unsigned)(grp + ((4 * ks * NJ + kk) * 16 + n) * 4);
@@ -314,7 +324,7 @@
     const float* gp = xg + ((long)t0 * B + b) * 4 * H + j;
 #pragma unroll
     for (int g = 0; g < 4; ++g) pre[g] = gp[g * H];
-    if (!PERSIST) c = cbuf[((long)(dir ? t0 + 2 : t0) * B + b) * H2 + dir * H + j];
+    if (!PERSIST || s0 > 0) c = cbuf[((long)(dir ? t0 + 2 : t0) * B + b) * H2 + dir * H + j];
   }
   u32x4 ld[NJ];
 #pragma unroll
@@ -324,9 +334,15 @@
 #pragma unroll
     for (int jj = 0; jj < NJ; ++jj) ld[jj] = src[jj * 64];
   }
+  if (PERSIST && s0 > 0 && b < B) {
+    const u32x4* src = reinterpret_cast<const u32x4*>(ybuf + ((long)(dir ? T + 1 - s0 : s0) * B + b) * H2 + dir * H + 16 * ks * NJ + 4 * kk);
+#pragma unroll
+    for (int jj = 0; jj < NJ; ++jj) ld[jj] = src[jj * 4];
+  }
   LSTM_STAMP_DECL;
   if (PERSIST) __syncthreads();
   for (int s = s0; s < s1; ++s) {
+    const bool hand = PERSIST && s > s0;
     const int t = dir ? T - 1 - s : s;
     LSTM_STAMP(0); LSTM_STAMP(10);
     constexpr int NACC = TILES == 1 ? 2 : TILES;
@@ -346,7 +362,7 @@
         }
         asm volatile("" ::: "memory");
       };
-      if (PERSIST) {
+      if (hand) {
         wait_producers();
 #pragma unroll
         for (int jj = 0; jj < NJ; ++jj) ld[jj] = __builtin_amdgcn_raw_buffer_load_b128(hx_rs, rd_b + (unsigned)jj * 1024u, 0, 16);
@@ -355,7 +371,7 @@
 #pragma unroll
       for (int jj = 0; jj < NJ; ++jj) {
         u32x4 v = ld[jj];
-        if (PERSIST) {
+        if (hand) {
           if (!__all(tags_are(v, want))) {
             wait_producers();
 #pragma unroll
@@ -371,8 +387,8 @@
         float hv[4];
 #pragma unroll
         for (int i = 0; i < 4; ++i) {
-          unsigned uu = PERSIST ? (v[i] & ~kTagBit) : v[i];
-          if (PERSIST) uu = uu == kNanPub ? 0x7fc00000u : uu;
+          unsigned uu = hand ? (v[i] & ~kTagBit) : v[i];
+          if (hand) uu = uu == kNanPub ? 0x7fc00000u : uu;
           hv[i] = __uint_as_float(uu);
         }
 #pragma unroll
@@ -407,7 +423,7 @@
       float h = go * tanhf_(cn);
       if (t >= ln) { cn = 0.f; h = 0.f; }
       c = cn;
-      if (PERSIST && ok && s + 1 < T) {
+      if (PERSIST && ok && s + 1 < s1) {
         const float* gp = xg + ((long)(dir ? t - 1 : t + 1) * B + b) * 4 * H + j;
 #pragma unroll
         for (int g = 0; g < 4; ++g) pre[g] = gp[g * H];
@@ -1108,6 +1124,7 @@
   float *wfrag, *hfrag;
   void* hxmem;
   size_t hxbytes;
+  int s0, s1;
 };
 struct BwdArgs {
   float *g_f, *g_r;
@@ -1124,32 +1141,32 @@
 void launch_fwd_step(const SeqPlan& p, const FwdArgs& a, hipStream_t st) {
   ensure_lds<&lstm_fwd_step<W>>(p.lds);
   const long hn = (long)2 * 2 * p.grid.y * a.H * 32;
-  hipLaunchKernelGGL(zero_kernel, dim3(cdiv(hn, 256) > 1024 ? 1024 : cdiv(hn, 256)), dim3(256), 0, st, a.hfrag, hn);
-  for (int s = 0; s < a.T; ++s)
+  if (a.s0 == 0) hipLaunchKernelGGL(zero_kernel, dim3(cdiv(hn, 256) > 1024 ? 1024 : cdiv(hn, 256)), dim3(256), 0, st, a.hfrag, hn);
+  for (int s = a.s0; s < a.s1; ++s)
     hipLaunchKernelGGL((lstm_fwd_step<W>), p.grid, dim3(W * 64), p.lds, st, a.xg_f, a.xg_r, a.wfrag, a.ybuf, a.cbuf, a.hfrag, a.lens, a.T, a.B, a.H, s);
 }
 template <int W, int QN>
 void launch_fwd_persist(const SeqPlan& p, const FwdArgs& a, hipStream_t st) {
   ensure_lds<&lstm_fwd_persist<W, QN, 1>>(p.lds);
   lstm_stamps_arm();
-  (void)hipMemsetAsync(a.hxmem, 0, a.hxbytes, st);
+  if (a.s0 == 0) (void)hipMemsetAsync(a.hxmem, 0, a.hxbytes, st);
   hipLaunchKernelGGL((lstm_fwd_persist<W, QN, 1>), p.grid, dim3(W * 64), p.lds, st, a.xg_f, a.xg_r, a.wfrag, a.ybuf, a.cbuf, (u64*)((char*)a.hxmem + 16),
-                     (unsigned*)a.hxmem, a.lens, a.T, a.B, a.H);
+                     (unsigned*)a.hxmem, a.lens, a.T, a.B, a.H, a.s0, a.s1);
 }
 template <int TILES, int NJ>
 void launch_fwd2_persist(const SeqPlan& p, const FwdArgs& a, hipStream_t st) {
   ensure_lds<&lstm_fwd2<TILES, NJ, true>>(p.lds);
   lstm_stamps_arm();
-  (void)hipMemsetAsync(a.hxmem, 0, a.hxbytes, st);
+  if (a.s0 == 0) (void)hipMemsetAsync(a.hxmem, 0, a.hxbytes, st);
   hipLaunchKernelGGL((lstm_fwd2<TILES, NJ, true>), p.grid, dim3(256), p.lds, st, a.xg_f, a.xg_r, a.whh_f, a.whh_r, a.ybuf, a.cbuf,
-                     (unsigned*)((char*)a.hxmem + 16), (unsigned*)a.hxmem, a.lens, a.T, a.B, a.H, 0);
+                     (unsigned*)((char*)a.hxmem + 16), (unsigned*)a.hxmem, a.lens, a.T, a.B, a.H, a.s0, a.s1);
 }
 template <int TILES, int NJ>
 void launch_fwd2_step(const SeqPlan& p, const FwdArgs& a, hipStream_t st) {
   ensure_lds<&lstm_fwd2<TILES, NJ, false>>(p.lds);
-  for (int s = 0; s < a.T; ++s)
+  for (int s = a.s0; s < a.s1; ++s)
     hipLaunchKernelGGL((lstm_fwd2<TILES, NJ, false>), p.grid, dim3(256), p.lds, st, a.xg_f, a.xg_r, a.whh_f, a.whh_r, a.ybuf, a.cbuf,
-                       (unsigned*)((char*)a.hxmem + 16), (unsigned*)a.hxmem, a.lens, a.T, a.B, a.H, s);
+                       (unsigned*)((char*)a.hxmem + 16), (unsigned*)a.hxmem, a.lens, a.T, a.B, a.H, s, s + 1);
 }
 template <int JT>
 void launch_bwd_step(const SeqPlan& p, const BwdArgs& a, hipStream_t st) {
@@ -1217,17 +1234,17 @@
   static const bool on = [] { const char* e = getenv("RE2E_DEBUG_HOOKS"); return e && atoi(e) == 1; }();
   return on;
 }
-__global__ void forced_abort_kernel(float* ybuf, long n) {
+__global__ void forced_abort_kernel(float* ybuf, long n, unsigned* err) {
   for (long i = (long)blockIdx.x * blockDim.x + threadIdx.x; i < n; i += (long)gridDim.x * blockDim.x) ybuf[i] = __uint_as_float(0x7fc00000u);
-  if (blockIdx.x == 0 && threadIdx.x == 0) atomicAdd(&g_persist_aborts, 1u);
-}
-bool forced_abort(hipStream_t st, float* ybuf, int T, int B, int H) {
+  if (blockIdx.x == 0 && threadIdx.x == 0) { atomicAdd(&g_persist_aborts, 1u); if (err) *err = 1u; }
+}
+bool forced_abort(hipStream_t st, float* ybuf, int T, int B, int H, unsigned* err = nullptr) {
   int left = g_force_abort.load(std::memory_order_relaxed);
   do {
     if (left <= 0) return false;
   } while (!g_force_abort.compare_exchange_weak(left, left - 1, std::memory_order_relaxed));
   const long n = (long)T * B * 2 * H;
-  hipLaunchKernelGGL(forced_abort_kernel, dim3(1024), dim3(256), 0, st, ybuf + (long)B * 2 * H, n);
+  hipLaunchKernelGGL(forced_abort_kernel, dim3(1024), dim3(256), 0, st, ybuf + (long)B * 2 * H, n, err);
   return true;
 }
 __global__ __launch_bounds__(256) void occupy_kernel(unsigned long long ticks, float* sink) {
@@ -1313,6 +1330,11 @@
   return d < 0 ? -1 : (int)n + d;
 }
 
+int re2e_lstm_fwd_resident_(int T, int B, int H, int cus) {
+  SeqPlan p;
+  return plan_fwd(T, B, H, true, cus, p) && (p.family == kFwdPersist || p.family == kFwd2Persist);
+}
+
 extern "C" int re2e_lstm_plan(int T, int B, int H, int backward, int cus, char* out, size_t out_bytes) {
   RE2E_CHECK_ARG(T > 0 && B > 0 && H > 0 && cus >= 0 && out && out_bytes > 0, "bad argument");
   if (cus == 0) cus = cu_count();
@@ -1329,28 +1351,47 @@
   return RE2E_OK;
 }
 
+static int seq_fwd_range(const char* who, float* xg_f, float* xg_r, const float* whh_f, const float* whh_r, float* ybuf, float* cbuf, const int* lens_dev,
+                         int T, int B, int H, int s_begin, int s_end, void* workspace, size_t workspace_bytes, hipStream_t stream) {
+  if (!(xg_f && xg_r && whh_f && whh_r && ybuf && cbuf && lens_dev && workspace)) { re2e_set_error("%s: null arg", who); return RE2E_EINVAL; }
+  if (!(T > 0 && B > 0 && H > 0 && 0 <= s_begin && s_begin < s_end && s_end <= T)) { re2e_set_error("%s: bad shape or range", who); return RE2E_EINVAL; }
+  if (H % 8 != 0) { re2e_set_error("%s: hidden size must be a multiple of 8 (got %d)", who, H); return RE2E_EUNSUPPORTED; }
+  if (workspace_bytes < fwd_ws_floats(B, H) * sizeof(float) + fwd_hx_bytes(B, H)) { re2e_set_error("%s: workspace too small", who); return RE2E_EINVAL; }
+  if (s_begin > 0 && (reinterpret_cast<uintptr_t>(ybuf) & 15)) { re2e_set_error("%s: a range with s_begin > 0 needs a 16-byte aligned ybuf", who); return RE2E_EINVAL; }
+  SeqPlan p;
+  const bool aligned = ((reinterpret_cast<uintptr_t>(whh_f) | reinterpret_cast<uintptr_t>(whh_r)) & 15) == 0;
+  if (!plan_fwd(T, B, H, aligned, cu_count(), p)) { re2e_set_error("%s: no kernel is built for hidden size %d", who, H); return RE2E_EUNSUPPORTED; }
+  const long wn = (long)4 * H * H;
+  float* wfrag = (float*)workspace;
+  const FwdArgs args = {xg_f, xg_r, whh_f, whh_r, ybuf, cbuf, lens_dev, T, B, H, wfrag, wfrag + 2 * wn,
+                        (char*)workspace + fwd_ws_floats(B, H) * sizeof(float), fwd_hx_bytes(B, H), s_begin, s_end};
+  const bool resident = p.family == kFwdPersist || p.family == kFwd2Persist;
+  if (s_begin == 0) {
+    const bool whole = s_end == T;
+    if (!env_off("RE2E_LSTM_PERSIST") && T >= 2 && (whole || resident)) {
+      if (!whole) (void)hipMemsetAsync(args.hxmem, 0, args.hxbytes, stream);
+      if (forced_abort(stream, ybuf, T, B, H, whole ? nullptr : (unsigned*)args.hxmem)) { RE2E_LAUNCH_CHECK(); return RE2E_OK; }
+    }
+    if (p.family == kFwdPersist || p.family == kFwdStep) {
+      hipLaunchKernelGGL(pack_w_fwd_kernel, dim3(cdiv(wn, 256) > 2048 ? 2048 : cdiv(wn, 256)), dim3(256), 0, stream, whh_f, wfrag, H);
+      hipLaunchKernelGGL(pack_w_fwd_kernel, dim3(cdiv(wn, 256) > 2048 ? 2048 : cdiv(wn, 256)), dim3(256), 0, stream, whh_r, wfrag + wn, H);
+    }
+  }
+  if (const int rc = run_fwd(p, args, stream)) return rc;
+  RE2E_LAUNCH_CHECK();
+  return RE2E_OK;
+}
+
 extern "C" int re2e_lstm_seq_fwd(float* xg_f, float* xg_r, const float* whh_f, const float* whh_r, float* ybuf, float* cbuf,
                                  const int* lens_dev, int T, int B, int H, void* workspace, size_t workspace_bytes,
                                  hipStream_t stream) {
-  RE2E_CHECK_ARG(xg_f && xg_r && whh_f && whh_r && ybuf && cbuf && lens_dev && workspace, "null arg");
-  RE2E_CHECK_ARG(T > 0 && B > 0 && H > 0, "bad shape");
-  if (H % 8 != 0) { re2e_set_error("re2e_lstm_seq_fwd: hidden size must be a multiple of 8 (got %d)", H); return RE2E_EUNSUPPORTED; }
-  RE2E_CHECK_ARG(workspace_bytes >= fwd_ws_floats(B, H) * sizeof(float) + fwd_hx_bytes(B, H), "workspace too small");
-  SeqPlan p;
-  const bool aligned = ((reinterpret_cast<uintptr_t>(whh_f) | reinterpret_cast<uintptr_t>(whh_r)) & 15) == 0;
-  if (!plan_fwd(T, B, H, aligned, cu_count(), p)) { re2e_set_error("re2e_lstm_seq_fwd: no kernel is built for hidden size %d", H); return RE2E_EUNSUPPORTED; }
-  if (!env_off("RE2E_LSTM_PERSIST") && T >= 2 && forced_abort(stream, ybuf, T, B, H)) { RE2E_LAUNCH_CHECK(); return RE2E_OK; }
-  const long wn = (long)4 * H * H;
-  float* wfrag = (float*)workspace;
-  const FwdArgs args = {xg_f, xg_r, whh_f, whh_r, ybuf, cbuf, lens_dev, T, B, H, wfrag, wfrag + 2 * wn,
-                        (char*)workspace + fwd_ws_floats(B, H) * sizeof(float), fwd_hx_bytes(B, H)};
-  if (p.family == kFwdPersist || p.family == kFwdStep) {
-    hipLaunchKernelGGL(pack_w_fwd_kernel, dim3(cdiv(wn, 256) > 2048 ? 2048 : cdiv(wn, 256)), dim3(256), 0, stream, whh_f, wfrag, H);
-    hipLaunchKernelGGL(pack_w_fwd_kernel, dim3(cdiv(wn, 256) > 2048 ? 2048 : cdiv(wn, 256)), dim3(256), 0, stream, whh_r, wfrag + wn, H);
-  }
-  if (const int rc = run_fwd(p, args, stream)) return rc;
-  RE2E_LAUNCH_CHECK();
-  return RE2E_OK;
+  return seq_fwd_range("re2e_lstm_seq_fwd", xg_f, xg_r, whh_f, whh_r, ybuf, cbuf, lens_dev, T, B, H, 0, T, workspace, workspace_bytes, stream);
+}
+
+extern "C" int re2e_lstm_seq_fwd_range(float* xg_f, float* xg_r, const float* whh_f, const float* whh_r, float* ybuf, float* cbuf,
+                                       const int* lens_dev, int T, int B, int H, int s_begin, int s_end, void* workspace, size_t workspace_bytes,
+                                       hipStream_t stream) {
+  return seq_fwd_range("re2e_lstm_seq_fwd_range", xg_f, xg_r, whh_f, whh_r, ybuf, cbuf, lens_dev, T, B, H, s_begin, s_end, workspace, workspace_bytes, stream);
 }
 
 extern "C" int re2e_lstm_seq_bwd(float* g_f, float* g_r, const float* whh_f, const float* whh_r, const float* dy, const float* ybuf,
diff --git a/robust_e2e_gan_amd/flops.py b/robust_e2e_gan_amd/flops.py
--- a/robust_e2e_gan_amd/flops.py
+++ b/robust_e2e_gan_amd/flops.py
@@ -48,6 +48,9 @@
     're2e_conv_wgrad': lambda *a: 2.0 * a[1] * a[9] * a[10] * a[6] * a[7] * a[8] * a[4],
     're2e_conv_dgrad_s2': lambda *a: 2.0 * a[1] * a[9] * a[10] * a[6] * a[4] * (a[7] * a[8] / 4.0),
     're2e_lstm_seq_fwd': lambda *a: 2.0 * 2 * a[7] * a[8] * a[9] * 4 * a[9],
+    're2e_lstm_seq_fwd_range': lambda *a: 2.0 * 2 * (a[11] - a[10]) * a[8] * a[9] * 4 * a[9],
+    're2e_bilstm_fwd_pipe': lambda *a: (2.0 * 2 * (a[21] if _ptr(a[20]) and a[2] >= 384 else a[17] * a[18]) * 4 * a[19] * a[2]
+                                        + 2.0 * 2 * a[17] * a[18] * a[19] * 4 * a[19]),
     're2e_lstm_seq_bwd': lambda *a: 2.0 * 2 * a[9] * a[10] * a[11] * 4 * a[11],
     're2e_fbank_fwd': lambda *a: 2.0 * a[1] * a[2] * a[3],
     're2e_fbank_bwd': lambda *a: 2.0 * a[1] * a[2] * a[3],
diff --git a/robust_e2e_gan_amd/joint_train.py b/robust_e2e_gan_amd/joint_train.py
--- a/robust_e2e_gan_amd/joint_train.py
+++ b/robust_e2e_gan_amd/joint_train.py
@@ -90,13 +90,14 @@
             ops.dropout_seed(self._dropout_stream_seed(int(getattr(opt, 'seed', 1234))))
         self.overlap_dstep = os.environ.get('RE2E_NO_OVERLAP', '0') != '1'
         self.marks = [] if os.environ.get('RE2E_TIMELINE') else None
-        self.main_stream = self.side_stream = self.wgrad_stream = None
+        self.main_stream = self.side_stream = self.wgrad_stream = self.feed_stream = None
         if torch.cuda.is_available():
-            self.main_stream, self.side_stream, self.wgrad_stream = lib.step_streams(next(enhance_model.parameters()).device)
+            self.main_stream, self.side_stream, self.wgrad_stream, self.feed_stream = lib.step_streams(next(enhance_model.parameters()).device)
 
     def step(self, data, sche_samp_rate, enhance_cmvn):
         overlap = self.overlap_dstep
-        with ops.routing(wgrad=self.wgrad_stream if overlap else None, aux=self.side_stream if overlap else None, marks=self.marks, multi=overlap,
+        with ops.routing(wgrad=self.wgrad_stream if overlap else None, aux=self.side_stream if overlap else None,
+                         feed=self.feed_stream if overlap and self.main_stream is not None else None, marks=self.marks, multi=overlap,
                          sync_bn=bool(getattr(self.opt, 'sync_bn', False)) and rdist.world_size() > 1):
             if not (overlap and self.main_stream is not None):
                 return self._step(data, sche_samp_rate, enhance_cmvn)
diff --git a/robust_e2e_gan_amd/lib.py b/robust_e2e_gan_amd/lib.py
--- a/robust_e2e_gan_amd/lib.py
+++ b/robust_e2e_gan_amd/lib.py
@@ -7,7 +7,7 @@
 
 _HERE = os.path.dirname(os.path.abspath(__file__))
 LIB_PATH = os.environ.get('RE2E_LIB') or os.path.join(_HERE, 'libre2e_hip.so')
-ABI_VERSION = 322
+ABI_VERSION = 323
 
 ACT_NONE, ACT_TANH, ACT_RELU, ACT_LRELU, ACT_SIGMOID, ACT_SIGMOID_MASK_MUL = range(6)
 LOSS_L2, LOSS_L1, LOSS_SMOOTH_L1, LOSS_BCE = range(4)
@@ -90,6 +90,10 @@
     're2e_debug_occupy': (I, [I, I, I, P]),
     're2e_step_gate': (I, [P, I, P, P, P, P, P, P, P]),
     're2e_lstm_seq_fwd': (I, [P, P, P, P, P, P, P, I, I, I, P, Z, P]),
+    're2e_lstm_seq_fwd_range': (I, [P, P, P, P, P, P, P, I, I, I, I, I, P, Z, P]),
+    're2e_bilstm_fwd_pipe': (I, [P, L, I, P, P, L, P, P, P, P, P, P, P, P, P, P, P, I, I, I, P, I, I, P, I, P, Z, P, Z, P, P]),
+    're2e_bilstm_pipe_workspace_bytes': (Z, [I, I, I, I, P, I, I]),
+    're2e_bilstm_pipe_plan': (I, [I, I, I, L, I, I, I, I, I, P, Z]),
     're2e_lstm_seq_bwd': (I, [P, P, P, P, P, P, P, P, P, I, I, I, P, P, Z, P]),
     're2e_lstm_plan': (I, [I, I, I, I, I, P, Z]),
     're2e_lstm_cell_fwd': (I, [P, P, P, P, I, I, P]),
@@ -232,6 +236,16 @@
     return dict(kv.split('=') for kv in buf.value.decode().split())
 
 
+def bilstm_pipe_plan(T, B, H, rows, N, K, cus=0, segments=0, have_feed=True):
+    buf = ctypes.create_string_buffer(1024)
+    lib = load()
+    rc = lib.re2e_bilstm_pipe_plan(T, B, H, rows, N, K, cus, segments, int(bool(have_feed)), buf, len(buf))
+    if rc != 0:
+        raise Re2eError('re2e_bilstm_pipe_plan failed (%d): %s' % (rc, lib.re2e_last_error().decode()))
+    kv = dict(x.split('=') for x in buf.value.decode().split())
+    return {'segments': int(kv['segments']), 'min_len': int(kv['min_len']), 'bounds': [int(v) for v in kv['bounds'].split(',')]}
+
+
 def gemm_plan(transa, transb, M, N, K, act=ACT_NONE, aligned=(True, True, True), rowmap=False, filler=False, cus=0):
     buf = ctypes.create_string_buffer(256)
     lib = load()
@@ -251,11 +265,13 @@
     got = _STEP_STREAMS.get(key)
     if got is None:
         with torch.cuda.device(idx):
+            wgrad = torch.cuda.Stream()
             main = torch.cuda.Stream(priority=int(main_priority))
-            side, wgrad = torch.cuda.Stream(), torch.cuda.Stream()
+            feed = torch.cuda.Stream(priority=int(main_priority))
+            side = torch.cuda.Stream()
         set_stream_role(side, True)
         set_stream_role(wgrad, True)
-        got = _STEP_STREAMS[key] = (main, side, wgrad)
+        got = _STEP_STREAMS[key] = (main, side, wgrad, feed)
     return got
 
 
diff --git a/robust_e2e_gan_amd/ops.py b/robust_e2e_gan_amd/ops.py
--- a/robust_e2e_gan_amd/ops.py
+++ b/robust_e2e_gan_amd/ops.py
@@ -62,10 +62,10 @@
 
 
 class RowMaps(object):
-    __slots__ = ('valid', 'invalid', 'nv', 'ni', 'rows', 'ident')
-
-    def __init__(self, valid, invalid, nv, ni, rows, ident):
-        self.valid, self.invalid, self.nv, self.ni, self.rows, self.ident = valid, invalid, nv, ni, rows, ident
+    __slots__ = ('valid', 'invalid', 'nv', 'ni', 'rows', 'ident', 't_off')
+
+    def __init__(self, valid, invalid, nv, ni, rows, ident, t_off=None):
+        self.valid, self.invalid, self.nv, self.ni, self.rows, self.ident, self.t_off = valid, invalid, nv, ni, rows, ident, t_off
 
 
 _ROW_MAPS = {}
@@ -87,16 +87,18 @@
         idx = np.arange(T * B, dtype=np.int32)
         v_ = idx[ok]
         neq = np.nonzero(v_ != idx[:v_.size])[0]
-        hit = (v_, idx[~ok], int(neq[0]) if neq.size else int(v_.size))
+        t_off = np.zeros(T + 1, np.int32)
+        np.cumsum(ok.reshape(T, B).sum(1), out=t_off[1:])
+        hit = (v_, idx[~ok], int(neq[0]) if neq.size else int(v_.size), t_off)
         while len(_ROW_MAPS) >= 64:
             _ROW_MAPS.pop(next(iter(_ROW_MAPS)))
         _ROW_MAPS[key] = hit
-    v, iv, ident = hit
+    v, iv, ident, t_off = hit
     if v.size < 256 or iv.size < ROW_MAPS_MIN_PAD * T * B:
         return None
     dev = lens_d.device
     return RowMaps(ec.dev_cached(('rows_v',) + key, lambda: v, dev), ec.dev_cached(('rows_i',) + key, lambda: iv, dev), int(v.size), int(iv.size), T * B,
-                   ident if ROW_IDENT else 0)
+                   ident if ROW_IDENT else 0, t_off)
 
 
 def gemm_rows(A, B, C, N, K, maps, lda=None, ldb=None, ldc=None, bias=None, bias2=None, act=lib.ACT_NONE, beta=0.0, fill=False):
@@ -151,6 +153,8 @@
 MULTI_STREAM = False
 WGRAD_STREAM = None
 AUX_STREAM = None
+FEED_STREAM = None
+PIPE_SEGMENTS = 0
 FROZEN_PARAMS = frozenset()
 MARKS = None
 SYNC_BN = False
@@ -169,9 +173,13 @@
         g.update(prev)
 
 
-def routing(wgrad=None, aux=None, marks=None, sync_bn=False, multi=None):
+def routing(wgrad=None, aux=None, marks=None, sync_bn=False, multi=None, feed=None):
     multi = (wgrad is not None or aux is not None) if multi is None else bool(multi)
-    return _ambient(MULTI_STREAM=multi, WGRAD_STREAM=wgrad, AUX_STREAM=aux, MARKS=marks, SYNC_BN=bool(sync_bn))
+    return _ambient(MULTI_STREAM=multi, WGRAD_STREAM=wgrad, AUX_STREAM=aux, FEED_STREAM=feed, MARKS=marks, SYNC_BN=bool(sync_bn))
+
+
+def pipe_segments(n):
+    return _ambient(PIPE_SEGMENTS=int(n))
 
 
 def inline_weight_grads():
@@ -1165,23 +1173,15 @@
         ctx.maps = maps
         xg = [empty((T * B, 4 * H), x), empty((T * B, 4 * H), x)]
         Ip = (I + 3) & ~3
+        wih = [w[0], w[4]]
         if Ip != I and T * B >= 1024 and lib.exp_env('RE2E_NO_PAD_INPUT') != '1':
             x2p = zeros((T * B, Ip), x)
             x2p[:, :I].copy_(x2)
             for d in range(2):
-                wp = zeros((4 * H, Ip), x)
-                wp[:, :I].copy_(w[4 * d].detach())
-                if maps is not None:
-                    gemm_rows(x2p, wp, xg[d], 4 * H, Ip, maps, bias=w[4 * d + 2], bias2=w[4 * d + 3])
-                else:
-                    gemm(x2p, wp, xg[d], T * B, 4 * H, Ip, transb=True, bias=w[4 * d + 2], bias2=w[4 * d + 3])
+                wih[d] = zeros((4 * H, Ip), x)
+                wih[d][:, :I].copy_(w[4 * d].detach())
             x2 = x2p
-        else:
-            for d in range(2):
-                if maps is not None and w[4 * d].is_contiguous():
-                    gemm_rows(x2, w[4 * d], xg[d], 4 * H, I, maps, bias=w[4 * d + 2], bias2=w[4 * d + 3])
-                else:
-                    gemm(x2, w[4 * d], xg[d], T * B, 4 * H, I, transb=True, bias=w[4 * d + 2], bias2=w[4 * d + 3])
+        Kd = x2.shape[1]
         ybuf = empty((T + 2, B, 2 * H), x)
         cbuf = empty((T + 2, B, 2 * H), x)
         for buf in (ybuf, cbuf):
@@ -1189,8 +1189,23 @@
             buf[T + 1].zero_()
         wsb = query('re2e_lstm_workspace_bytes', B, H)
         ws = workspace(wsb, x.device, 'lstm')
-        call('re2e_lstm_seq_fwd', xg[0].data_ptr(), xg[1].data_ptr(), w[1].data_ptr(), w[5].data_ptr(), ybuf.data_ptr(), cbuf.data_ptr(),
-             lens_dev.data_ptr(), T, B, H, ws.data_ptr(), wsb)
+        feed = FEED_STREAM if MULTI_STREAM else None
+        if feed is not None and feed.cuda_stream != lib.stream() and all(m.is_contiguous() for m in wih) and x2.is_contiguous():
+            t_off = maps.t_off.ctypes.data if maps is not None else None
+            gwsb = query('re2e_bilstm_pipe_workspace_bytes', T, B, H, Kd, t_off, PIPE_SEGMENTS, 1)
+            gws = workspace(gwsb, x.device, 'bilstm_pipe') if gwsb else None
+            call('re2e_bilstm_fwd_pipe', x2.data_ptr(), Kd, Kd, wih[0].data_ptr(), wih[1].data_ptr(), Kd, ptr(w[2]), ptr(w[3]), ptr(w[6]), ptr(w[7]),
+                 xg[0].data_ptr(), xg[1].data_ptr(), w[1].data_ptr(), w[5].data_ptr(), ybuf.data_ptr(), cbuf.data_ptr(), lens_dev.data_ptr(), T, B, H,
+                 maps.valid.data_ptr() if maps is not None else None, maps.nv if maps is not None else 0, maps.ident if maps is not None else 0, t_off,
+                 PIPE_SEGMENTS, ws.data_ptr(), wsb, ptr(gws), gwsb, feed.cuda_stream)
+        else:
+            for d in range(2):
+                if maps is not None and wih[d].is_contiguous():
+                    gemm_rows(x2, wih[d], xg[d], 4 * H, Kd, maps, bias=w[4 * d + 2], bias2=w[4 * d + 3])
+                else:
+                    gemm(x2, wih[d], xg[d], T * B, 4 * H, Kd, transb=True, bias=w[4 * d + 2], bias2=w[4 * d + 3])
+            call('re2e_lstm_seq_fwd', xg[0].data_ptr(), xg[1].data_ptr(), w[1].data_ptr(), w[5].data_ptr(), ybuf.data_ptr(), cbuf.data_ptr(),
+                 lens_dev.data_ptr(), T, B, H, ws.data_ptr(), wsb)
         ctx.w, ctx.lens = w, lens_dev
         ctx.save_for_backward(x2, xg[0], xg[1], ybuf, cbuf)
         ctx.dims = (T, B, I, H)
diff --git a/robust_e2e_gan_amd/trainers.py b/robust_e2e_gan_amd/trainers.py
--- a/robust_e2e_gan_amd/trainers.py
+++ b/robust_e2e_gan_amd/trainers.py
@@ -29,9 +29,9 @@
 
     def __init__(self):
         self.on = torch.cuda.is_available() and os.environ.get('RE2E_NO_OVERLAP', '0') != '1'
-        self.main = self.side = self.wgrad = None
+        self.main = self.side = self.wgrad = self.feed = None
         if self.on:
-            self.main, self.side, self.wgrad = lib.step_streams()
+            self.main, self.side, self.wgrad, self.feed = lib.step_streams()
 
     @contextlib.contextmanager
     def step(self):
@@ -41,7 +41,7 @@
         caller = torch.cuda.current_stream()
         self.main.wait_stream(caller)
         try:
-            with ops.routing(wgrad=self.wgrad, aux=self.side, multi=True), torch.cuda.stream(self.main):
+            with ops.routing(wgrad=self.wgrad, aux=self.side, feed=self.feed, multi=True), torch.cuda.stream(self.main):
                 yield self
                 torch.cuda.current_stream().wait_stream(self.wgrad)
                 torch.cuda.current_stream().wait_stream(self.side)
```
